# xingchensong/TouchNet

Measured on AMD Instinct MI355X. Metric: audio+text tokens/sec/node (packed seq, full train step) + step MFU, higher is better.
Workload: dtype bf16

## Files before the change

### include/touchnet_amd.h

```cpp
#ifndef TOUCHNET_AMD_H_
#define TOUCHNET_AMD_H_

#ifdef __cplusplus
extern "C" {
#endif

const char* tn_version(void);

int tn_norm_bwd_workspace_floats(int rows, int H);
int tn_rmsnorm_fwd(const void* x, const void* res_in, const void* w, void* y, void* res_out, float* rstd,
                   int rows, int H, float eps, int dtype, void* stream);
int tn_rmsnorm_bwd(const void* dy, const void* h, const void* w, const float* rstd, const void* dres, void* dh,
                   void* dw, float* workspace, int rows, int H, int dtype, void* stream);

int tn_layernorm_fwd(const void* x, const void* res_in, const void* w, const void* b, void* y, void* res_out,
                     float* mean, float* rstd, int rows, int H, float eps, int dtype, void* stream);
int tn_layernorm_bwd(const void* dy, const void* h, const void* w, const float* mean, const float* rstd,
                     const void* dres, void* dh, void* dw, void* db, float* workspace, int rows, int H, int dtype,
                     void* stream);

int tn_swiglu_fwd(const void* gate, const void* up, void* out, long long n, int dtype, void* stream);
int tn_swiglu_bwd(const void* dout, const void* gate, const void* up, void* dgate, void* dup, long long n,
                  int dtype, void* stream);
int tn_swiglu_fwd_t(const void* gate, const void* up, void* out, void* out_t, int rows, int cols, void* stream);
int tn_swiglu_bwd_t(const void* dout, const void* gate, const void* up, void* dgate, void* dup, void* dgu_t, int rows,
                    int cols, void* stream);
int tn_gelu_fwd(const void* x, void* out, long long n, int dtype, void* stream);
int tn_gelu_bwd(const void* dout, const void* x, void* dx, long long n, int dtype, void* stream);

int tn_rope_table(const long long* position_ids, const float* inv_freq, void* cos_t, void* sin_t, int n, int half,
                  float attention_scaling, int dtype, void* stream);
int tn_rope_apply(const void* q, const void* k, void* q_out, void* k_out, const void* cos_t, const void* sin_t,
                  int n, int hq, int hk, int D, int backward, int dtype, void* stream);

int tn_ce_forward(const void* logits, const long long* labels, const long long* sentence_lens,
                  const float* num_sentence, float* nll, float* lse, int* hit, float* out, int n, int V,
                  long long ignore_index, int dtype, void* stream);
int tn_ce_reduce(const float* nll, const int* hit, const long long* labels, const long long* sentence_lens,
                 const float* num_sentence, float* out, int n, long long ignore_index, void* stream);
int tn_ce_backward(const void* logits, void* dlogits, const long long* labels, const long long* sentence_lens,
                   const float* lse, const float* num_sentence, const float* grad_out, int n, int V,
                   long long ignore_index, int dtype, void* stream);

int tn_attn_meta_ints(int B, int T);
int tn_attn_build_meta(const int* doc, int* meta, int B, int T, void* stream);
int tn_attn_fwd(const void* q, const void* k, const void* v, void* o, float* lse2, const int* doc, const int* meta,
                int B, int T, int Nh, int Nkv, int D, float scale, void* stream);
int tn_attn_bwd(const void* q, const void* k, const void* v, const void* o, const void* dout, const float* lse2,
                float* delta, void* dq, void* dk, void* dv, const int* doc, const int* meta, int B, int T, int Nh,
                int Nkv, int D, float scale, void* stream);
int tn_attn_bwd_rope(const void* q, const void* k, const void* v, const void* o, const void* dout, const float* lse2,
                     float* delta, void* dq, void* dk, void* dv, const int* doc, const int* meta, int B, int T, int Nh,
                     int Nkv, int D, float scale, const void* cos_t, const void* sin_t, void* stream);
int tn_attn_fwd_bidir(const void* q, const void* k, const void* v, void* o, float* lse2, const int* doc, const int* meta,
                      int B, int T, int Nh, int Nkv, int D, float scale, void* stream);
int tn_attn_bwd_bidir(const void* q, const void* k, const void* v, const void* o, const void* dout, const float* lse2,
                      float* delta, void* dq, void* dk, void* dv, const int* doc, const int* meta, int B, int T, int Nh,
                      int Nkv, int D, float scale, void* stream);

int tn_attn_fwd_seg(const void* q, const void* k, const void* v, void* o, float* lse2, const int* doc,
                    const int* meta, int B, int T, int Nh, int Nkv, int D, float scale, int nseg,
                    const int* host_segs, int rows_per_batch, void* stream);
int tn_attn_fwd_seg_chunks(const void* q, const void* k, const void* v, void* o, float* lse2, const int* doc,
                           const int* meta, int B, int T, int Nh, int Nkv, int D, float scale, int nseg, const int* segs,
                           int rows_per_batch, int chunk_len, unsigned long long chunk_mask, void* stream);
int tn_attn_merge(const void* o_a, const float* lse2_a, const void* o_b, const float* lse2_b, void* o, float* lse2,
                  int B, int rows, int Nh, int D, void* stream);
int tn_attn_bwd_seg(const void* q, const void* k, const void* v, const void* o, const void* dout,
                    const float* lse2, float* delta, void* dq, void* dk, void* dv, const int* doc, const int* meta,
                    int B, int T, int Nh, int Nkv, int D, float scale, int nseg, const int* host_segs,
                    int rows_per_batch, void* stream);

int tn_fbank_frames(int n_samples);
int tn_kaldi_fbank(const float* wav, float* feat, int n_samples, int n_mels, void* stream);
int tn_log_mel(const float* wav, const float* mel_fb, float* feat, float* scratch_max, int n_samples, int n_mels,
               void* stream);
int tn_audiofeat_stack(const float* feat, float* out, int T, int F, int stack, int stride, int normalize,
                       void* stream);
int tn_feat_augment(const float* x, float* y, int T, int F, int out_rows, const int* t_masks, int n_t,
                    const int* f_masks, int n_f, const int* subs, int n_sub, void* stream);
int tn_resample_polyphase(const float* x, float* y, const float* tab, long long n_in, long long n_out, int p, int q,
                          int ntap, void* stream);
int tn_resample_sinc(const void* x, int x_is_pcm16, float* y, const float* tab, long long n_in, long long n_out,
                     int orig, int new_, int ntap, void* stream);

int tn_sumsq_scratch_floats(void);
int tn_sumsq(const void* g, float* scratch, float* norm_sq, long long n, int dtype, void* stream);
long long tn_sumsq_multi_chunk(void);
int tn_sumsq_multi(const void* const* ptrs, const long long* sizes, const long long* first_chunk, int ntensors,
                   long long nchunks, float* partial, float* norm_sq, int dtype, void* stream);
int tn_adamw_step(float* p, float* m, float* v, const void* g, void* p_shadow_bf16, const float* norm_sq,
                  long long n, float lr, float beta1, float beta2, float eps, float weight_decay, float max_norm,
                  float bias_corr1, float bias_corr2, int g_dtype, void* stream);

long long tn_adamw_multi_chunk(void);
int tn_adamw_prepare(const float* norm_sq, float* state, float beta1, float beta2, float max_norm, void* stream);
int tn_adamw_multi(void* const* ps, void* const* ms, void* const* vs, const void* const* gs, void* const* shadows,
                   const long long* sizes, const long long* first_chunk, int ntensors, long long nchunks,
                   const float* state, float lr, float beta1, float beta2, float eps, float weight_decay, int g_dtype,
                   void* stream);
int tn_adamw_multi_bounded(void* const* ps, void* const* ms, void* const* vs, const void* const* gs, void* const* shadows,
                           const long long* sizes, const long long* first_chunk, int ntensors, long long nchunks,
                           const float* state, float lr, float beta1, float beta2, float eps, float weight_decay,
                           int g_dtype, int max_workgroups, void* stream);

int tn_transpose_bf16(const void* src, void* dst, int rows, int cols, long long src_ld, long long dst_ld,
                      void* stream);

long long tn_colsum_workspace_floats(int rows, int cols);
int tn_colsum_bf16(const void* x, void* out, float* ws, int rows, int cols, long long ld, void* stream);

int tn_pcm16_to_f32(const void* pcm_int16, float* out, long long n, void* stream);

int tn_bestrq_tokenize(const float* feat, const float* quantizer, const float* codebook, long long* codes, int T,
                       int F, int E, int V, void* stream);

int tn_pack_plan(const int* lens, int n, int B, int T, int skip_too_long, int* row, int* col, int* sent, int* batch,
                 int* counts, void* stream);
int tn_pack_fill(const int* row, const int* col, const int* sent, const int* batch, int which_batch, int n,
                 const int* ntok, const long long* tok_off, const long long* tokens, const int* alen,
                 const long long* feat_off, const float* feat_src, int F, int B, int T, long long bos, long long eos,
                 long long pad, long long* input_ids, long long* labels, long long* position_ids, long long* doc,
                 long long* sentence_lens, float* feats, int* nsent, void* stream);

int tn_gemm_bf16(const void* const* A, const void* const* B, const long long* lda, const long long* ldb, const int* K,
                 int nseg, int a_kmaj, int b_kmaj, void* C, void* Ct, const void* bias, int M, int N, long long ldc,
                 long long ldct, int accumulate, void* stream);
int tn_gemm_bf16_addend(const void* A, const void* B, long long lda, long long ldb, int K, int a_kmaj, int b_kmaj, void* C,
                        const void* bias, const void* addend, long long ldadd, int M, int N, long long ldc, void* stream);
int tn_gemm_bf16_splitk(const void* A, const void* B, long long lda, long long ldb, int K, int a_kmaj, int b_kmaj,
                        void* C, const void* bias, int M, int N, long long ldc, int accumulate, int splitk, int tail_only,
                        void* workspace, long long workspace_bytes, void* stream);
int tn_gemm_bf16_wgrad_f32(const void* A, const void* B, long long lda, long long ldb, int K, float* C, int M, int N,
                           long long ldc, int accumulate, int splitk, void* workspace, long long workspace_bytes,
                           void* stream);
int tn_gemm_bf16_wgrad_bias(const void* A, const void* B, long long lda, long long ldb, int K, void* C, void* bias_grad,
                            int M, int N, long long ldc, int accumulate, int c_f32, int splitk, void* workspace,
                            long long workspace_bytes, void* stream);
long long tn_gemm_splitk_workspace_bytes(int M, int N, int splitk, int with_bias_grad, int tail_only);
long long tn_gemm_grouped_workspace_bytes(const int* M, const int* N, const int* K, int ngrp);
int tn_gemm_bf16_grouped(const void* const* A, const void* const* B, const long long* lda, const long long* ldb,
                         const int* K, void* const* C, const long long* ldc, const int* M, const int* N, int ngrp,
                         int a_kmaj, int b_kmaj, int accumulate, int c_f32, void* workspace, long long workspace_bytes,
                         void* stream);
long long tn_gemm_grouped_table_bytes(int n);
int tn_gemm_bf16_grouped_table(const void* const* A, const void* const* B, const long long* lda, const long long* ldb,
                               const int* K, void* const* C, const long long* ldc, const int* M, const int* N,
                               void* const* bias_grad, int n, int accumulate, int c_f32, void* table,
                               long long table_bytes, void* stream);
int tn_gemm_bf16_swiglu_fwd(const void* x, const void* wg, const void* wu, void* gate, void* up, void* act, int M, int I,
                            int K, long long ldx, long long ldw, long long ldc, void* stream);
int tn_gemm_bf16_swiglu_bwd(const void* dy, const void* wd, const void* gate, const void* up, void* dgate, void* dup,
                            int M, int I, int H, long long lddy, long long ldw, long long ld, void* stream);
int tn_gemm_bf16_gelu_fwd(const void* x, const void* w, const void* bias, void* pre, void* act, int M, int N, int K,
                          long long ldx, long long ldw, long long ldc, void* stream);
int tn_gemm_bf16_gelu_bwd(const void* dy, const void* w2, const void* pre, void* dpre, int M, int I, int H, long long lddy,
                          long long ldw, long long ld, void* stream);
int tn_gemm_bf16_rope(const void* x, const void* w, const void* bias, const void* cos_t, const void* sin_t, void* out, int M,
                      int N, int K, long long ldx, long long ldw, long long ldc, int head_dim, void* stream);
int tn_gemm_bf16_tn(const void* A, const void* B, void* C, void* Ct, const void* bias, int M, int N, int K,
                    long long lda, long long ldb, long long ldc, long long ldct, int accumulate, void* stream);

void tn_gemm_set_persistent(int on);
int tn_gemm_get_persistent(void);

long long tn_attn_decode_workspace_bytes(int B, int Nh, int Nkv, int D, int S_max);
int tn_attn_decode(const void* q, const void* k_new, const void* v_new, void* k_cache, void* v_cache, const int* cache_len,
                   void* o, void* workspace, int B, int Nh, int Nkv, int D, int S_max, float scale, void* stream);
int tn_greedy_step(const void* logits, int* hist, int* hist_len, int* cache_len, int* finished, int* n_unfinished, int B,
                   int V, int S_hist, float penalty, int ngram, int eos, int pad, int dtype, void* stream);
int tn_sample_step(const void* logits, int* hist, int* hist_len, int* cache_len, int* finished, int* n_unfinished,
                   const long long* row_key, const float* uniforms, int* n_kept, int B, int V, int S_hist, float penalty,
                   int do_sample, float temperature, int top_k, float top_p, unsigned long long seed, const int* eos_ids,
                   int n_eos, int pad, int dtype, void* stream);
int tn_kimi_text_step(const void* logits, int* hist, int* hist_len, int* cache_len, int* finished, int* n_unfinished,
                      const int* prompt_len, const void* embed, void* x_next, const long long* row_key,
                      const float* uniforms, int B, int V, int S_hist, int H, float penalty, int window, float temperature,
                      int top_k, unsigned long long seed, int eos, int blank, int audio_token, int dtype, void* stream);

int tn_attn_decode_beam(const void* q, const void* k_new, const void* v_new, void* k_cache, void* v_cache,
                        const int* cache_len, const int* src, void* o, void* workspace, int R, int Nh, int Nkv, int D,
                        int S_max, float scale, void* stream);
long long tn_beam_step_workspace_bytes(int B, int K);
int tn_beam_step(const void* logits, int* hist, int* hist_len, int* cache_len, int* src, float* run_score, int* fin_ids,
                 int* fin_len, float* fin_score, int* fin_flag, int* gen, int* unsat, int* done, int* n_unfinished,
                 int* out_ids, int* out_parent, void* workspace, int B, int K, int K_in, int V, int S_hist, float penalty,
                 int ngram, const int* eos_ids, int n_eos, int n_new, float length_penalty, int early_stopping, int dtype,
                 void* stream);

int tn_attn_block_causal_fwd(const void* q, const void* k, const void* v, void* o, const int* seg_start, const int* key_end,
                             int B, int T, int Nh, int D, int block, float scale, void* stream);
int tn_vq_nearest(const void* x, const void* codebook, const float* cnorm, long long* ids, int M, int V, int d, void* stream);

#ifdef __cplusplus
}
#endif
#endif
```

### touchnet_amd/_C.py

```python
from __future__ import annotations

import ctypes as C
import os

import torch

_HERE = os.path.dirname(os.path.abspath(__file__))
LIB_PATH = os.environ.get("TN_AMD_LIB") or os.path.join(_HERE, "_lib", "libtouchnet_amd.so")

_vp, _i, _f, _ll, _ull = C.c_void_p, C.c_int, C.c_float, C.c_longlong, C.c_ulonglong

PROTOTYPES = {
    "tn_version": [],
    "tn_norm_bwd_workspace_floats": [_i, _i],
    "tn_rmsnorm_fwd": [_vp, _vp, _vp, _vp, _vp, _vp, _i, _i, _f, _i, _vp],
    "tn_rmsnorm_bwd": [_vp, _vp, _vp, _vp, _vp, _vp, _vp, _vp, _i, _i, _i, _vp],
    "tn_layernorm_fwd": [_vp, _vp, _vp, _vp, _vp, _vp, _vp, _vp, _i, _i, _f, _i, _vp],
    "tn_layernorm_bwd": [_vp, _vp, _vp, _vp, _vp, _vp, _vp, _vp, _vp, _vp, _i, _i, _i, _vp],
    "tn_swiglu_fwd": [_vp, _vp, _vp, _ll, _i, _vp],
    "tn_swiglu_bwd": [_vp, _vp, _vp, _vp, _vp, _ll, _i, _vp],
    "tn_gelu_fwd": [_vp, _vp, _ll, _i, _vp],
    "tn_gelu_bwd": [_vp, _vp, _vp, _ll, _i, _vp],
    "tn_rope_table": [_vp, _vp, _vp, _vp, _i, _i, _f, _i, _vp],
    "tn_rope_apply": [_vp, _vp, _vp, _vp, _vp, _vp, _i, _i, _i, _i, _i, _i, _vp],
    "tn_ce_forward": [_vp, _vp, _vp, _vp, _vp, _vp, _vp, _vp, _i, _i, _ll, _i, _vp],
    "tn_ce_reduce": [_vp, _vp, _vp, _vp, _vp, _vp, _i, _ll, _vp],
    "tn_ce_backward": [_vp, _vp, _vp, _vp, _vp, _vp, _vp, _i, _i, _ll, _i, _vp],
    "tn_attn_meta_ints": [_i, _i],
    "tn_attn_build_meta": [_vp, _vp, _i, _i, _vp],
    "tn_attn_fwd": [_vp, _vp, _vp, _vp, _vp, _vp, _vp, _i, _i, _i, _i, _i, _f, _vp],
    "tn_attn_bwd": [_vp, _vp, _vp, _vp, _vp, _vp, _vp, _vp, _vp, _vp, _vp, _vp, _i, _i, _i, _i, _i, _f, _vp],
    "tn_attn_bwd_rope": [_vp, _vp, _vp, _vp, _vp, _vp, _vp, _vp, _vp, _vp, _vp, _vp, _i, _i, _i, _i, _i, _f, _vp, _vp, _vp],
    "tn_attn_fwd_bidir": [_vp, _vp, _vp, _vp, _vp, _vp, _vp, _i, _i, _i, _i, _i, _f, _vp],
    "tn_attn_bwd_bidir": [_vp, _vp, _vp, _vp, _vp, _vp, _vp, _vp, _vp, _vp, _vp, _vp, _i, _i, _i, _i, _i, _f, _vp],
    "tn_attn_fwd_seg": [_vp, _vp, _vp, _vp, _vp, _vp, _vp, _i, _i, _i, _i, _i, _f, _i, _vp, _i, _vp],
    "tn_attn_fwd_seg_chunks": [_vp, _vp, _vp, _vp, _vp, _vp, _vp, _i, _i, _i, _i, _i, _f, _i, _vp, _i, _i, C.c_ulonglong, _vp],
    "tn_attn_merge": [_vp, _vp, _vp, _vp, _vp, _vp, _i, _i, _i, _i, _vp],
    "tn_attn_bwd_seg": [_vp, _vp, _vp, _vp, _vp, _vp, _vp, _vp, _vp, _vp, _vp, _vp, _i, _i, _i, _i, _i, _f, _i, _vp,
                        _i, _vp],
    "tn_fbank_frames": [_i],
    "tn_kaldi_fbank": [_vp, _vp, _i, _i, _vp],
    "tn_log_mel": [_vp, _vp, _vp, _vp, _i, _i, _vp],
    "tn_audiofeat_stack": [_vp, _vp, _i, _i, _i, _i, _i, _vp],
    "tn_resample_polyphase": [_vp, _vp, _vp, _ll, _ll, _i, _i, _i, _vp],
    "tn_resample_sinc": [_vp, _i, _vp, _vp, _ll, _ll, _i, _i, _i, _vp],
    "tn_feat_augment": [_vp, _vp, _i, _i, _i, _vp, _i, _vp, _i, _vp, _i, _vp],
    "tn_sumsq_scratch_floats": [],
    "tn_sumsq": [_vp, _vp, _vp, _ll, _i, _vp],
    "tn_adamw_step": [_vp, _vp, _vp, _vp, _vp, _vp, _ll, _f, _f, _f, _f, _f, _f, _f, _f, _i, _vp],
    "tn_transpose_bf16": [_vp, _vp, _i, _i, _ll, _ll, _vp],
    "tn_swiglu_fwd_t": [_vp, _vp, _vp, _vp, _i, _i, _vp],
    "tn_swiglu_bwd_t": [_vp, _vp, _vp, _vp, _vp, _vp, _i, _i, _vp],
    "tn_colsum_workspace_floats": [_i, _i],
    "tn_colsum_bf16": [_vp, _vp, _vp, _i, _i, _ll, _vp],
    "tn_pcm16_to_f32": [_vp, _vp, _ll, _vp],
    "tn_bestrq_tokenize": [_vp, _vp, _vp, _vp, _i, _i, _i, _i, _vp],
    "tn_sumsq_multi_chunk": [],
    "tn_sumsq_multi": [_vp, _vp, _vp, _i, _ll, _vp, _vp, _i, _vp],
    "tn_adamw_multi_chunk": [],
    "tn_adamw_prepare": [_vp, _vp, _f, _f, _f, _vp],
    "tn_adamw_multi": [_vp, _vp, _vp, _vp, _vp, _vp, _vp, _i, _ll, _vp, _f, _f, _f, _f, _f, _i, _vp],
    "tn_adamw_multi_bounded": [_vp, _vp, _vp, _vp, _vp, _vp, _vp, _i, _ll, _vp, _f, _f, _f, _f, _f, _i, _i, _vp],
    "tn_pack_plan": [_vp, _i, _i, _i, _i, _vp, _vp, _vp, _vp, _vp, _vp],
    "tn_pack_fill": [_vp, _vp, _vp, _vp, _i, _i, _vp, _vp, _vp, _vp, _vp, _vp, _i, _i, _i, _ll, _ll, _ll, _vp, _vp, _vp,
                     _vp, _vp, _vp, _vp, _vp],
    "tn_gemm_bf16_tn": [_vp, _vp, _vp, _vp, _vp, _i, _i, _i, _ll, _ll, _ll, _ll, _i, _vp],
    "tn_gemm_bf16_addend": [_vp, _vp, _ll, _ll, _i, _i, _i, _vp, _vp, _vp, _ll, _i, _i, _ll, _vp],
    "tn_gemm_bf16_splitk": [_vp, _vp, _ll, _ll, _i, _i, _i, _vp, _vp, _i, _i, _ll, _i, _i, _i, _vp, _ll, _vp],
    "tn_gemm_bf16_wgrad_f32": [_vp, _vp, _ll, _ll, _i, _vp, _i, _i, _ll, _i, _i, _vp, _ll, _vp],
    "tn_gemm_bf16": [C.POINTER(_vp), C.POINTER(_vp), C.POINTER(_ll), C.POINTER(_ll), C.POINTER(_i), _i, _i, _i, _vp, _vp,
                     _vp, _i, _i, _ll, _ll, _i, _vp],
    "tn_gemm_splitk_workspace_bytes": [_i, _i, _i, _i, _i],
    "tn_gemm_grouped_workspace_bytes": [C.POINTER(_i), C.POINTER(_i), C.POINTER(_i), _i],
    "tn_gemm_bf16_grouped": [C.POINTER(_vp), C.POINTER(_vp), C.POINTER(_ll), C.POINTER(_ll), C.POINTER(_i), C.POINTER(_vp),
                             C.POINTER(_ll), C.POINTER(_i), C.POINTER(_i), _i, _i, _i, _i, _i, _vp, _ll, _vp],
    "tn_gemm_grouped_table_bytes": [_i],
    "tn_gemm_bf16_grouped_table": [C.POINTER(_vp), C.POINTER(_vp), C.POINTER(_ll), C.POINTER(_ll), C.POINTER(_i),
                                   C.POINTER(_vp), C.POINTER(_ll), C.POINTER(_i), C.POINTER(_i), C.POINTER(_vp), _i, _i, _i,
                                   _vp, _ll, _vp],
    "tn_gemm_bf16_wgrad_bias": [_vp, _vp, _ll, _ll, _i, _vp, _vp, _i, _i, _ll, _i, _i, _i, _vp, _ll, _vp],
    "tn_gemm_bf16_rope": [_vp, _vp, _vp, _vp, _vp, _vp, _i, _i, _i, _ll, _ll, _ll, _i, _vp],
    "tn_gemm_bf16_gelu_fwd": [_vp, _vp, _vp, _vp, _vp, _i, _i, _i, _ll, _ll, _ll, _vp],
    "tn_gemm_bf16_gelu_bwd": [_vp, _vp, _vp, _vp, _i, _i, _i, _ll, _ll, _ll, _vp],
    "tn_gemm_bf16_swiglu_fwd": [_vp, _vp, _vp, _vp, _vp, _vp, _i, _i, _i, _ll, _ll, _ll, _vp],
    "tn_gemm_bf16_swiglu_bwd": [_vp, _vp, _vp, _vp, _vp, _vp, _i, _i, _i, _ll, _ll, _ll, _vp],
    "tn_gemm_set_persistent": [_i],
    "tn_gemm_get_persistent": [],
    "tn_attn_decode_workspace_bytes": [_i, _i, _i, _i, _i],
    "tn_attn_decode": [_vp, _vp, _vp, _vp, _vp, _vp, _vp, _vp, _i, _i, _i, _i, _i, _f, _vp],
    "tn_greedy_step": [_vp, _vp, _vp, _vp, _vp, _vp, _i, _i, _i, _f, _i, _i, _i, _i, _vp],
    "tn_sample_step": [_vp, _vp, _vp, _vp, _vp, _vp, _vp, _vp, _vp, _i, _i, _i, _f, _i, _f, _i, _f, _ull, _vp, _i, _i, _i,
                       _vp],
    "tn_kimi_text_step": [_vp] * 11 + [_i, _i, _i, _i, _f, _i, _f, _i, _ull, _i, _i, _i, _i, _vp],
    "tn_attn_decode_beam": [_vp, _vp, _vp, _vp, _vp, _vp, _vp, _vp, _vp, _i, _i, _i, _i, _i, _f, _vp],
    "tn_beam_step_workspace_bytes": [_i, _i],
    "tn_beam_step": [_vp] * 17 + [_i, _i, _i, _i, _i, _f, _i, _vp, _i, _i, _f, _i, _i, _vp],
    "tn_attn_block_causal_fwd": [_vp, _vp, _vp, _vp, _vp, _vp, _i, _i, _i, _i, _i, _f, _vp],
    "tn_vq_nearest": [_vp, _vp, _vp, _vp, _i, _i, _i, _vp],
}
_RESTYPE = {"tn_gemm_set_persistent": None, "tn_version": C.c_char_p, "tn_sumsq_multi_chunk": C.c_longlong, "tn_adamw_multi_chunk": C.c_longlong,
            "tn_colsum_workspace_floats": C.c_longlong, "tn_gemm_splitk_workspace_bytes": C.c_longlong,
            "tn_gemm_grouped_workspace_bytes": C.c_longlong, "tn_gemm_grouped_table_bytes": C.c_longlong,
            "tn_attn_decode_workspace_bytes": C.c_longlong, "tn_beam_step_workspace_bytes": C.c_longlong,
            "tn_philox4x32_10": None}

DEV_PROTOTYPES = {
    "tn_philox4x32_10": [_vp, _ull],
}

_lib = None


class KernelError(RuntimeError):
    pass


def lib() -> C.CDLL:
    global _lib
    if _lib is None:
        if not os.path.exists(LIB_PATH):
            raise ImportError(
                f"{LIB_PATH} not found: build it with `python -m touchnet_amd.build` "
                "(touchnet_amd has no fallback path; the HIP extension is mandatory)")
        handle = C.CDLL(LIB_PATH)
        for name, argtypes in {**PROTOTYPES, **DEV_PROTOTYPES}.items():
            fn = getattr(handle, name)
            fn.argtypes = argtypes
            fn.restype = _RESTYPE.get(name, C.c_int)
        _lib = handle
    return _lib


def check(code: int, what: str) -> None:
    if code != 0:
        raise KernelError(f"{what} failed with code {code} "
                          f"({'EINVAL: unsupported shape/dtype' if code == -22 else 'hipError_t'})")


DTYPE_CODE = {torch.float32: 0, torch.bfloat16: 1}


def dcode(t: torch.Tensor) -> int:
    try:
        return DTYPE_CODE[t.dtype]
    except KeyError:
        raise KernelError(f"unsupported dtype {t.dtype} (float32 / bfloat16 only)") from None


def ptr(t):
    if t is None:
        return None
    if not t.is_cuda:
        raise KernelError("touchnet_amd kernels need device (HIP) tensors; got a CPU tensor")
    return C.c_void_p(t.data_ptr())


def stream():
    return C.c_void_p(torch.cuda.current_stream().cuda_stream)


def version() -> str:
    return lib().tn_version().decode()
```

### touchnet_amd/csrc/gemm.hip

```cpp
#include "gemm_host.h"

namespace tn {
namespace gemm {

typedef f32x4_t Acc16[8][4];

template <bool AK, bool BK, int EPI = EPI_PLAIN>
struct Kernel16 {
  static_assert(EPI == EPI_PLAIN || EPI == EPI_SWIGLU_FWD || EPI == EPI_SWIGLU_BWD || EPI == EPI_ROPE ||
                    EPI == EPI_GELU_FWD || EPI == EPI_GELU_BWD,
                "Kernel16: plain / SwiGLU / RoPE / GELU epilogues (the weight-gradient modes stay on Kernel)");
  static_assert(EPI != EPI_GELU_FWD || !BK, "GELU forward: x W^T layout");
  static_assert(EPI != EPI_GELU_BWD || BK, "GELU backward: dY W layout");
  static_assert(!AK, "Kernel16: row-stored A (forward and input-gradient products)");
  static_assert(EPI != EPI_SWIGLU_FWD || !BK, "SwiGLU forward: x W^T layout");
  static_assert(EPI != EPI_SWIGLU_BWD || BK, "SwiGLU backward: dY W layout");
  static_assert(EPI != EPI_ROPE || !BK, "RoPE epilogue: x W^T layout");
  static constexpr int BN_EFF = EPI == EPI_SWIGLU_FWD ? 128 : BN;
  static __device__ __forceinline__ float sigm(float x) { return sigmoid_fast(x); }
  static __device__ __forceinline__ float lo16(uint32_t w) { return __uint_as_float(w << 16); }
  static __device__ __forceinline__ float hi16(uint32_t w) { return __uint_as_float(w & 0xffff0000u); }
  static __device__ __forceinline__ float rbf(float v) { return __uint_as_float(((uint32_t)f2bf(v)) << 16); }
  template <bool KMAJ>
  struct F4 {
// ... 438 lines not shown
      for (int bi = 0; bi < 4; ++bi) {
        const int m = min(wm0 + (half * 4 + bi) * 16 + l15, p.M - 1);
#pragma unroll
        for (int bj = 0; bj < 2; ++bj) {
          const long long o = (long long)m * hd + c0 + 16 * bj + 4 * g4;
          cw[bi][bj] = *reinterpret_cast<const uint2*>(p.rope_cos + o);
          sw[bi][bj] = *reinterpret_cast<const uint2*>(p.rope_sin + o);
        }
      }
#pragma unroll
      for (int bi = 0; bi < 4; ++bi)
#pragma unroll
        for (int bj = 0; bj < 2; ++bj) {
          const float ba[4] = {lo16(bwa[bj].x), hi16(bwa[bj].x), lo16(bwa[bj].y), hi16(bwa[bj].y)};
          const float bb[4] = {lo16(bwb[bj].x), hi16(bwb[bj].x), lo16(bwb[bj].y), hi16(bwb[bj].y)};
          const float cf[4] = {lo16(cw[bi][bj].x), hi16(cw[bi][bj].x), lo16(cw[bi][bj].y), hi16(cw[bi][bj].y)};
          const float sf[4] = {lo16(sw[bi][bj].x), hi16(sw[bi][bj].x), lo16(sw[bi][bj].y), hi16(sw[bi][bj].y)};
          float ya[4], yb[4];
#pragma unroll
          for (int e = 0; e < 4; ++e)
            rope_rotate(rbf(acc[half * 4 + bi][bj][e] + ba[e]), rbf(acc[half * 4 + bi][bj + 2][e] + bb[e]), cf[e], sf[e],
                        ya[e], yb[e]);
          *reinterpret_cast<u32x2_t*>(park_at(park, bi, bj, l15, g4)) = u32x2_t{pack2bf(ya[0], ya[1]), pack2bf(ya[2], ya[3])};
          *reinterpret_cast<u32x2_t*>(park_at(park, bi, bj + 2, l15, g4)) = u32x2_t{pack2bf(yb[0], yb[1]), pack2bf(yb[2], yb[3])};
        }
      asm volatile("s_waitcnt lgkmcnt(0)" ::: "memory");
#pragma unroll 4
      for (int it = 0; it < 8; ++it) {
        const int row = it * 8 + (lane >> 3), c = lane & 7;
        const u32x4_t pv = *reinterpret_cast<const u32x4_t*>(park + row * 128 + ((c ^ (row & 7)) << 4));
        const int m = wm0 + half * 64 + row, n = (c < 4 ? col_a : col_b) + (c & 3) * 8;
        if (m < p.M && n < p.N)
          *reinterpret_cast<uint4*>(p.C + (long long)m * p.ldc + n) = make_uint4(pv.x, pv.y, pv.z, pv.w);
      }
    }
  }

  static __device__ __forceinline__ void epilogue16(const Params& p, Acc16& acc, char* park, int wm0, int wn0, int lane) {
    const int l15 = lane & 15, g4 = lane >> 4;
    float bias_v[4][4];
    if (p.bias != nullptr) {
#pragma unroll
      for (int bj = 0; bj < 4; ++bj) {
        const int n = min(wn0 + bj * 16 + 4 * g4, p.N - 4);
        const uint2 w = *reinterpret_cast<const uint2*>(p.bias + n);
        bias_v[bj][0] = __uint_as_float(w.x << 16);
        bias_v[bj][1] = __uint_as_float(w.x & 0xffff0000u);
        bias_v[bj][2] = __uint_as_float(w.y << 16);
        bias_v[bj][3] = __uint_as_float(w.y & 0xffff0000u);
      }
    }
    const bool acc_c = p.accumulate != 0 || p.addend != nullptr;
#pragma unroll
    for (int half = 0; half < 2; ++half) {
      uint4 xpre[8];
      if constexpr (EPI == EPI_GELU_BWD) {
#pragma unroll
        for (int it = 0; it < 8; ++it) {
          const int m = wm0 + half * 64 + it * 8 + (lane >> 3), n = wn0 + (lane & 7) * 8;
          xpre[it] = (m < p.M && n < p.N) ? *reinterpret_cast<const uint4*>(p.E1 + (long long)m * p.lde + n)
                                          : make_uint4(0, 0, 0, 0);
        }
      }
#pragma unroll
      for (int bi = 0; bi < 4; ++bi) {
        const int row = bi * 16 + l15;
#pragma unroll
        for (int bj = 0; bj < 4; ++bj) {
          float v[4];
#pragma unroll
          for (int e = 0; e < 4; ++e) v[e] = acc[half * 4 + bi][bj][e] + (p.bias != nullptr ? bias_v[bj][e] : 0.f);
          const int chunk = (bj * 2 + (g4 >> 1)) ^ (row & 7);
          const u32x2_t pk = {pack2bf(v[0], v[1]), pack2bf(v[2], v[3])};
          *reinterpret_cast<u32x2_t*>(park + row * 128 + chunk * 16 + (g4 & 1) * 8) = pk;
        }
      }
      asm volatile("s_waitcnt lgkmcnt(0)" ::: "memory");
      constexpr int kReadOutUnroll = EPI == EPI_GELU_BWD ? 8 : 4;
#pragma unroll kReadOutUnroll
      for (int it = 0; it < 8; ++it) {
        const int row = it * 8 + (lane >> 3), c = lane & 7;
        const u32x4_t pv = *reinterpret_cast<const u32x4_t*>(park + row * 128 + ((c ^ (row & 7)) << 4));
        uint4 v = make_uint4(pv.x, pv.y, pv.z, pv.w);
        const int m = wm0 + half * 64 + row, n = wn0 + c * 8;
        if (m < p.M && n < p.N) {
          bf16_t* dst = p.C + (long long)m * p.ldc + n;
          if constexpr (EPI == EPI_GELU_FWD) {
            *reinterpret_cast<uint4*>(dst) = v;
            Vec16<bf16_t> x;
            x.raw = v;
            float f[8];
            x.unpack(f);
#pragma unroll
            for (int e = 0; e < 8; e += 2) {
              const gelu_f32x2 r = gelu_f2(gelu_f32x2{f[e], f[e + 1]});
              f[e] = r.x;
              f[e + 1] = r.y;
            }
            x.pack(f);
            *reinterpret_cast<uint4*>(p.C2 + (long long)m * p.ldc + n) = x.raw;
            continue;
          }
          if constexpr (EPI == EPI_GELU_BWD) {
            Vec16<bf16_t> x, d;
            x.raw = xpre[it];
            d.raw = v;
            float f[8], df[8];
            x.unpack(f);
            d.unpack(df);
#pragma unroll
            for (int e = 0; e < 8; e += 2) {
              const gelu_f32x2 r = gelu_grad_f2(gelu_f32x2{f[e], f[e + 1]}, gelu_f32x2{df[e], df[e + 1]});
              df[e] = r.x;
              df[e + 1] = r.y;
            }
            d.pack(df);
            *reinterpret_cast<uint4*>(dst) = d.raw;
            continue;
          }
          if (acc_c) {
            Vec16<bf16_t> o, nw;
            o.load(p.addend != nullptr ? p.addend + (long long)m * p.ldadd + n : dst);
            nw.raw = v;
            float fo[8], fn[8];
            o.unpack(fo);
            nw.unpack(fn);
#pragma unroll
            for (int e = 0; e < 8; ++e) fn[e] += fo[e];
            nw.pack(fn);
            v = nw.raw;
          }
          *reinterpret_cast<uint4*>(dst) = v;
        }
      }
    }
  }
};

template <bool AK, bool BK, int EPI = EPI_PLAIN>
__global__ __launch_bounds__(NT, 2) void gemm16_kernel(const Params p) {
  __shared__ __attribute__((aligned(1024))) char smem[LDS_BYTES];
  Kernel16<AK, BK, EPI>::run(p, smem);
}

__global__ __launch_bounds__(256) void splitk_reduce_kernel(const float* __restrict__ ws, int S, int M, int N, int nbm,
                                                            int nbn, int tile0, int ntiles, bf16_t* __restrict__ C,
                                                            long long ldc, const bf16_t* __restrict__ bias,
                                                            int accumulate, int out_f32,
                                                            const float* __restrict__ bias_ws,
                                                            bf16_t* __restrict__ bias_out) {
  const int t = blockIdx.x >> 5, part = blockIdx.x & 31;
  int tm, tn;
  tile_of_block(tile0 + t, nbm, nbn, tm, tn);
  const int idx = part * 256 + threadIdx.x;
  const int lm = idx >> 5, ln = (idx & 31) * 8;
  const int m = tm * BM + lm, n = tn * BN + ln;
  if (m >= M || n >= N) return;
  if (bias_out != nullptr && tn == 0 && ln == 0) {
    float b = 0.f;
    for (int sp = 0; sp < S; ++sp) b += bias_ws[(long long)sp * (nbm * BM) + m];
    bias_out[m] = f2bf(b);
  }
  float a[8] = {0.f, 0.f, 0.f, 0.f, 0.f, 0.f, 0.f, 0.f};
  const float* src = ws + (long long)t * (BM * BN) + lm * BN + ln;
  const long long slab = (long long)ntiles * (BM * BN);
  for (int sp = 0; sp < S; ++sp) {
    const float4 x = *reinterpret_cast<const float4*>(src + sp * slab);
    const float4 y = *reinterpret_cast<const float4*>(src + sp * slab + 4);
    a[0] += x.x; a[1] += x.y; a[2] += x.z; a[3] += x.w;
    a[4] += y.x; a[5] += y.y; a[6] += y.z; a[7] += y.w;
  }
  if (out_f32) {
    float* d = reinterpret_cast<float*>(C) + (long long)m * ldc + n;
    float4 x = make_float4(a[0], a[1], a[2], a[3]), y = make_float4(a[4], a[5], a[6], a[7]);
    if (accumulate) {
      const float4 ox = *reinterpret_cast<const float4*>(d), oy = *reinterpret_cast<const float4*>(d + 4);
      x.x += ox.x; x.y += ox.y; x.z += ox.z; x.w += ox.w;
      y.x += oy.x; y.y += oy.y; y.z += oy.z; y.w += oy.w;
    }
    *reinterpret_cast<float4*>(d) = x;
    *reinterpret_cast<float4*>(d + 4) = y;
    return;
  }
  bf16_t* dst = C + (long long)m * ldc + n;
  if (bias != nullptr) {
    Vec16<bf16_t> b;
    float fb[8];
    b.load(bias + n);
    b.unpack(fb);
#pragma unroll
    for (int e = 0; e < 8; ++e) a[e] += fb[e];
  }
  if (accumulate) {
    Vec16<bf16_t> o;
    float fo[8];
    o.load(dst);
    o.unpack(fo);
#pragma unroll
    for (int e = 0; e < 8; ++e) a[e] += fo[e];
  }
  Vec16<bf16_t> out;
  out.pack(a);
  out.store(dst);
}

template <bool AK, bool BK, bool HAS_CT>
static int launch(dim3 grid, hipStream_t st, const Params& p) {
  constexpr bool WGRAD = AK && BK && !HAS_CT;
  auto reduce = [&](const float* bias_ws, bf16_t* bias_out) {
    hipLaunchKernelGGL(splitk_reduce_kernel, dim3((unsigned)p.ntiles * 32u), dim3(256), 0, st, p.ws, p.splitk, p.M, p.N,
                       p.nbm, p.nbn, p.tile0, p.ntiles, p.C, p.ldc, p.bias, p.accumulate, p.c_f32, bias_ws, bias_out);
  };
  if (p.bias_out != nullptr) {
    if constexpr (WGRAD) {
      if (p.splitk > 1) {
        hipLaunchKernelGGL((gemm_kernel<true, true, false, true, false, EPI_BIASG>), grid, dim3(NT), 0, st, p);
        reduce(p.bias_ws, p.bias_out);
      } else if (p.c_f32) {
        hipLaunchKernelGGL((gemm_kernel<true, true, false, false, true, EPI_BIASG>), grid, dim3(NT), 0, st, p);
      } else {
        hipLaunchKernelGGL((gemm_kernel<true, true, false, false, false, EPI_BIASG>), grid, dim3(NT), 0, st, p);
      }
    } else {
      return -1;
    }
  } else if (p.splitk > 1) {
    if constexpr (!HAS_CT) {
      hipLaunchKernelGGL((gemm_kernel<AK, BK, false, true>), grid, dim3(NT), 0, st, p);
      reduce(nullptr, nullptr);
    } else {
      return -1;
    }
  } else if (p.c_f32) {
    if constexpr (WGRAD) {
      hipLaunchKernelGGL((gemm_kernel<true, true, false, false, true>), grid, dim3(NT), 0, st, p);
    } else {
      return -1;
    }
  } else if constexpr (!AK && !HAS_CT) {
    hipLaunchKernelGGL((gemm16_kernel<AK, BK>), grid, dim3(NT), 0, st, p);
  } else {
    hipLaunchKernelGGL((gemm_kernel<AK, BK, HAS_CT>), grid, dim3(NT), 0, st, p);
  }
  return 0;
}

}
}


extern "C" long long tn_gemm_splitk_workspace_bytes(int M, int N, int splitk, int with_bias_grad, int tail_only);

namespace {

int g_persistent = 1;

long long slab_floats(int parts, long long tiles) { return parts * tiles * BM * BN; }

int grouped_split(long long total, int min_stages, int& r) {
  const int ncu = num_cus();
  r = (int)(total % ncu);
  if (total <= ncu || r == 0 || r * 2 > ncu || min_stages < 16) return 1;
  return min(ncu / r, min_stages / 8);
}

struct GemmCall {
  const void* const* A;
  const void* const* B;
  const long long* lda;
  const long long* ldb;
  const int* K;
  int nseg, a_kmaj, b_kmaj;
  void* C;
  long long ldc;
  int M, N;
  void* stream;
  const void* bias = nullptr;
  int accumulate = 0;
  void* Ct = nullptr;
  long long ldct = 0;
  int splitk = 1, tail_only = 0;
  void* workspace = nullptr;
  long long workspace_bytes = 0;
  int c_f32 = 0;
  void* bias_grad = nullptr;
  const void* addend = nullptr;
  long long ldadd = 0;
};

int launch_mode(bool a_kmaj, bool b_kmaj, bool ct, dim3 grid, hipStream_t st, const Params& p) {
  if (!a_kmaj && !b_kmaj) return ct ? launch<false, false, true>(grid, st, p) : launch<false, false, false>(grid, st, p);
  if (!a_kmaj) return ct ? launch<false, true, true>(grid, st, p) : launch<false, true, false>(grid, st, p);
  return ct ? launch<true, true, true>(grid, st, p) : launch<true, true, false>(grid, st, p);
}

int gemm_launch(const GemmCall& c) {
  const int M = c.M, N = c.N;
  const bool wgrad_mode = c.a_kmaj && c.b_kmaj && c.nseg == 1 && c.Ct == nullptr && c.bias == nullptr;
  if (c.a_kmaj && !c.b_kmaj) return TN_EINVAL;
  if (c.addend != nullptr && (c.accumulate || c.splitk > 1 || c.tail_only || c.Ct != nullptr || c.c_f32 ||
                              c.bias_grad != nullptr || !out_ok(c.addend, c.ldadd, N, 8)))
    return TN_EINVAL;
  if ((c.bias_grad != nullptr || c.c_f32) && (!wgrad_mode || c.tail_only)) return TN_EINVAL;
  if (!aligned(1, c.bias_grad)) return TN_EINVAL;
  if (M <= 0 || N <= 0 || c.nseg < 1 || c.nseg > MAXSEG || (N % 8) != 0 || (c.a_kmaj && (M % 8))) return TN_EINVAL;
  if (!out_ok(c.C, c.ldc, N, 8)) return TN_EINVAL;
  if (c.Ct != nullptr && ((M % 8) || c.accumulate || !out_ok(c.Ct, c.ldct, M, 8))) return TN_EINVAL;
  Params p;
  clear_params(p);
  for (int s = 0; s < c.nseg; ++s) {
    const int k = c.K[s];
    if (!(c.a_kmaj ? kmaj_operand_ok(c.A[s], c.lda[s], k, M, M) : row_operand_ok(c.A[s], c.lda[s], k, 1))) return TN_EINVAL;
    if (!(c.b_kmaj ? kmaj_operand_ok(c.B[s], c.ldb[s], k, N, 1) : row_operand_ok(c.B[s], c.ldb[s], k, 1))) return TN_EINVAL;
    set_seg(p.seg[s], c.A[s], c.B[s], c.lda[s], c.ldb[s], k);
    p.stages += (k + 63) / 64;
  }
  for (int s = c.nseg; s < MAXSEG; ++s) p.seg[s] = p.seg[0];
  p.nseg = c.nseg;
  p.M = M;
  p.N = N;
  p.C = (bf16_t*)c.C;
  p.Ct = (bf16_t*)c.Ct;
  p.bias = (const bf16_t*)c.bias;
  p.ldc = c.ldc;
  p.ldct = c.ldct;
  p.accumulate = c.accumulate;
  p.addend = (const bf16_t*)c.addend;
  p.ldadd = c.ldadd;
  p.nbm = (M + BM - 1) / BM;
  p.nbn = (N + BN - 1) / BN;
  p.ntiles = p.nbm * p.nbn;
  p.c_f32 = c.c_f32;
  p.bias_out = (bf16_t*)c.bias_grad;
  const int ncu = num_cus();
  int main_tiles = 0;
  if (c.splitk > 1) {
    if (c.nseg != 1 || c.Ct != nullptr) return TN_EINVAL;
    if (!(c.a_kmaj && c.b_kmaj) && (p.stages % c.splitk) != 0) return TN_EINVAL;
    const long long need = tn_gemm_splitk_workspace_bytes(M, N, c.splitk, c.bias_grad != nullptr, c.tail_only);
    if (need < 0 || c.workspace == nullptr || !aligned(15, c.workspace) || c.workspace_bytes < need) return TN_EINVAL;
    if (c.tail_only) main_tiles = p.ntiles / ncu * ncu;
    p.splitk = c.splitk;
    p.kchunk = (p.stages + c.splitk - 1) / c.splitk;
    p.ws = (float*)c.workspace;
    if (c.bias_grad != nullptr) p.bias_ws = p.ws + slab_floats(c.splitk, p.ntiles);
  }
  hipStream_t st = (hipStream_t)c.stream;
  int rc = 0;
  if (main_tiles > 0) {
    Params pm = p;
    pm.splitk = 1;
    pm.ntiles = main_tiles;
    rc |= launch_mode(c.a_kmaj, c.b_kmaj, c.Ct != nullptr, dim3(ncu), st, pm);
    p.tile0 = main_tiles;
    p.ntiles -= main_tiles;
  }
  rc |= launch_mode(c.a_kmaj, c.b_kmaj, c.Ct != nullptr, grid_for(p.ntiles * p.splitk), st, p);
  if (rc != 0) return TN_EINVAL;
  TN_LAUNCH_CHECK();
  return TN_OK;
}

template <int EPI, bool B_KMAJ>
int launch_fused(Params& p, int M, int N, long long ldc, int col_tile, void* stream) {
  for (int s = 1; s < MAXSEG; ++s)
    if (p.seg[s].K == 0) p.seg[s] = p.seg[0];
  p.stages = p.seg[0].K / 64;
  p.M = M;
  p.N = N;
  p.ldc = ldc;
  p.nbm = (M + BM - 1) / BM;
  p.nbn = (N + col_tile - 1) / col_tile;
  p.ntiles = p.nbm * p.nbn;
  hipLaunchKernelGGL((gemm16_kernel<false, B_KMAJ, EPI>), grid_for(p.ntiles), dim3(NT), 0, (hipStream_t)stream, p);
  TN_LAUNCH_CHECK();
  return TN_OK;
}

}

extern "C" {

void tn_gemm_set_persistent(int on) { g_persistent = on ? 1 : 0; }
int tn_gemm_get_persistent(void) { return g_persistent; }

long long tn_gemm_splitk_workspace_bytes(int M, int N, int splitk, int with_bias_grad, int tail_only) {
  if (splitk <= 1) return 0;
  if (M <= 0 || N <= 0) return -1;
  const long long nbm = (M + BM - 1) / BM;
  long long tiles = nbm * ((N + BN - 1) / BN);
  if (tail_only) {
    const int ncu = num_cus();
    if (tiles < ncu || tiles % ncu == 0) return -1;
    tiles %= ncu;
  }
  return (slab_floats(splitk, tiles) + (with_bias_grad ? splitk * nbm * BM : 0)) * (long long)sizeof(float);
}

int tn_gemm_bf16(const void* const* A, const void* const* B, const long long* lda, const long long* ldb, const int* K,
                 int nseg, int a_kmaj, int b_kmaj, void* C, void* Ct, const void* bias, int M, int N, long long ldc,
                 long long ldct, int accumulate, void* stream) {
  GemmCall c{A, B, lda, ldb, K, nseg, a_kmaj, b_kmaj, C, ldc, M, N, stream};
  c.bias = bias;
  c.accumulate = accumulate;
  c.Ct = Ct;
  c.ldct = ldct;
  return gemm_launch(c);
}

int tn_gemm_bf16_addend(const void* A, const void* B, long long lda, long long ldb, int K, int a_kmaj, int b_kmaj, void* C,
                        const void* bias, const void* addend, long long ldadd, int M, int N, long long ldc, void* stream) {
  if (addend == nullptr || addend == C) return TN_EINVAL;
  GemmCall c{&A, &B, &lda, &ldb, &K, 1, a_kmaj, b_kmaj, C, ldc, M, N, stream};
  c.bias = bias;
  c.addend = addend;
  c.ldadd = ldadd;
  return gemm_launch(c);
}

int tn_gemm_bf16_splitk(const void* A, const void* B, long long lda, long long ldb, int K, int a_kmaj, int b_kmaj,
                        void* C, const void* bias, int M, int N, long long ldc, int accumulate, int splitk, int tail_only,
                        void* workspace, long long workspace_bytes, void* stream) {
  if (splitk < 2) return TN_EINVAL;
  GemmCall c{&A, &B, &lda, &ldb, &K, 1, a_kmaj, b_kmaj, C, ldc, M, N, stream};
  c.bias = bias;
  c.accumulate = accumulate;
  c.splitk = splitk;
  c.tail_only = tail_only;
  c.workspace = workspace;
  c.workspace_bytes = workspace_bytes;
  return gemm_launch(c);
}

static int wgrad(const void* A, const void* B, long long lda, long long ldb, int K, void* C, void* bias_grad, int M, int N,
                 long long ldc, int accumulate, int c_f32, int splitk, void* workspace, long long workspace_bytes,
                 void* stream) {
  GemmCall c{&A, &B, &lda, &ldb, &K, 1, 1, 1, C, ldc, M, N, stream};
  c.accumulate = accumulate;
  c.c_f32 = c_f32;
  c.bias_grad = bias_grad;
  c.splitk = splitk > 1 ? splitk : 1;
  c.workspace = workspace;
  c.workspace_bytes = workspace_bytes;
  return gemm_launch(c);
}

int tn_gemm_bf16_wgrad_f32(const void* A, const void* B, long long lda, long long ldb, int K, float* C, int M, int N,
                           long long ldc, int accumulate, int splitk, void* workspace, long long workspace_bytes,
                           void* stream) {
  return wgrad(A, B, lda, ldb, K, C, nullptr, M, N, ldc, accumulate, 1, splitk, workspace, workspace_bytes, stream);
}

int tn_gemm_bf16_wgrad_bias(const void* A, const void* B, long long lda, long long ldb, int K, void* C, void* bias_grad,
                            int M, int N, long long ldc, int accumulate, int c_f32, int splitk, void* workspace,
                            long long workspace_bytes, void* stream) {
  if (bias_grad == nullptr) return TN_EINVAL;
  return wgrad(A, B, lda, ldb, K, C, bias_grad, M, N, ldc, accumulate, c_f32, splitk, workspace, workspace_bytes, stream);
}

long long tn_gemm_grouped_workspace_bytes(const int* M, const int* N, const int* K, int ngrp) {
  if (ngrp < 1 || ngrp > MAXSEG) return -1;
  long long tiles = 0;
  int min_stages = 0x7fffffff, r;
  for (int g = 0; g < ngrp; ++g) {
    tiles += (long long)((M[g] + BM - 1) / BM) * ((N[g] + BN - 1) / BN);
    min_stages = min(min_stages, (K[g] + 63) / 64);
  }
  const int S = grouped_split(tiles, min_stages, r);
  return S > 1 ? slab_floats(S, r) * (long long)sizeof(float) : 0;
}

int tn_gemm_bf16_grouped(const void* const* A, const void* const* B, const long long* lda, const long long* ldb,
                         const int* K, void* const* C, const long long* ldc, const int* M, const int* N, int ngrp,
                         int a_kmaj, int b_kmaj, int accumulate, int c_f32, void* workspace, long long workspace_bytes,
                         void* stream) {
  if (ngrp < 1 || ngrp > MAXSEG) return TN_EINVAL;
  if (!(a_kmaj && b_kmaj)) return TN_EINVAL;
  Params p;
  clear_params(p);
  int total = 0, min_stages = 0x7fffffff;
  for (int g = 0; g < ngrp; ++g) {
    if (!grouped_product(A[g], B[g], lda[g], ldb[g], K[g], C[g], ldc[g], M[g], N[g], c_f32, total, p.seg[g], p.grp[g]))
      return TN_EINVAL;
    min_stages = min(min_stages, p.grp[g].stages);
    total += p.grp[g].nbm * p.grp[g].nbn;
  }
  for (int g = ngrp; g < MAXSEG; ++g) {
    p.seg[g] = p.seg[0];
    p.grp[g] = p.grp[0];
    p.grp[g].start = 0x7fffffff;
  }
  p.ngrp = ngrp;
  p.accumulate = accumulate;
  p.c_f32 = c_f32;
  hipStream_t st = (hipStream_t)stream;
  int r, S = grouped_split(total, min_stages, r);
  if (S > 1 && (workspace == nullptr || !aligned(15, workspace) ||
                workspace_bytes < slab_floats(S, r) * (long long)sizeof(float)))
    S = 1;
  const int main_tiles = S > 1 ? total - r : total;
  p.tile0 = 0;
  p.ntiles = main_tiles;
  if (c_f32)
    hipLaunchKernelGGL((gemm_kernel<true, true, false, false, true, EPI_GROUPED>), grid_for(main_tiles), dim3(NT), 0, st, p);
  else
    hipLaunchKernelGGL((gemm_kernel<true, true, false, false, false, EPI_GROUPED>), grid_for(main_tiles), dim3(NT), 0, st, p);
  if (S > 1) {
    float* ws = (float*)workspace;
    for (int g = 0; g < ngrp; ++g) {
      const int end = p.grp[g].start + p.grp[g].nbm * p.grp[g].nbn;
      const int lo = max(main_tiles, p.grp[g].start), hi = end;
      if (lo >= hi) continue;
      Params q;
      clear_params(q);
      q.seg[0] = p.seg[g];
      q.seg[1] = q.seg[2] = q.seg[0];
      q.M = p.grp[g].M;
      q.N = p.grp[g].N;
      q.C = p.grp[g].C;
      q.ldc = p.grp[g].ldc;
      q.accumulate = accumulate;
      q.nbm = p.grp[g].nbm;
      q.nbn = p.grp[g].nbn;
      q.stages = p.grp[g].stages;
      q.splitk = S;
      q.kchunk = (q.stages + S - 1) / S;
      q.ws = ws;
      q.tile0 = lo - p.grp[g].start;
      q.ntiles = hi - lo;
      q.c_f32 = c_f32;
      hipLaunchKernelGGL((gemm_kernel<true, true, false, true>), grid_for(q.ntiles * S), dim3(NT), 0, st, q);
      hipLaunchKernelGGL(splitk_reduce_kernel, dim3((unsigned)q.ntiles * 32u), dim3(256), 0, st, q.ws, q.splitk, q.M, q.N,
                         q.nbm, q.nbn, q.tile0, q.ntiles, q.C, q.ldc, (const bf16_t*)nullptr, q.accumulate, q.c_f32,
                         (const float*)nullptr, (bf16_t*)nullptr);
      ws += slab_floats(S, q.ntiles);
    }
  }
  TN_LAUNCH_CHECK();
  return TN_OK;
}
int tn_gemm_bf16_swiglu_fwd(const void* x, const void* wg, const void* wu, void* gate, void* up, void* act, int M, int I,
                            int K, long long ldx, long long ldw, long long ldc, void* stream) {
  if (M <= 0 || I <= 0 || (I % 8) || !row_operand_ok(x, ldx, K, K) || !row_operand_ok(wg, ldw, K, K) ||
      !row_operand_ok(wu, ldw, K, K) || !out_ok(gate, ldc, I, 8) || !aligned(15, up, act))
    return TN_EINVAL;
  Params p;
  clear_params(p);
  set_seg(p.seg[0], x, wg, ldx, ldw, K);
  set_seg(p.seg[1], x, wu, ldx, ldw, K);
  p.C = (bf16_t*)gate;
  p.C2 = (bf16_t*)up;
  p.C3 = (bf16_t*)act;
  return launch_fused<EPI_SWIGLU_FWD, false>(p, M, I, ldc, 128, stream);
}

int tn_gemm_bf16_swiglu_bwd(const void* dy, const void* wd, const void* gate, const void* up, void* dgate, void* dup,
                            int M, int I, int H, long long lddy, long long ldw, long long ld, void* stream) {
  if (M <= 0 || I <= 0 || (I % 8) || !row_operand_ok(dy, lddy, H, H) || !kmaj_operand_ok(wd, ldw, H, I, I) ||
      !out_ok(dgate, ld, I, 8) || !aligned(15, dup, gate, up))
    return TN_EINVAL;
  Params p;
  clear_params(p);
  set_seg(p.seg[0], dy, wd, lddy, ldw, H);
  p.C = (bf16_t*)dgate;
  p.C2 = (bf16_t*)dup;
  p.E1 = (const bf16_t*)gate;
  p.E2 = (const bf16_t*)up;
  p.lde = ld;
  return launch_fused<EPI_SWIGLU_BWD, true>(p, M, I, ld, BN, stream);
}

int tn_gemm_bf16_rope(const void* x, const void* w, const void* bias, const void* cos_t, const void* sin_t, void* out, int M,
                      int N, int K, long long ldx, long long ldw, long long ldc, int head_dim, void* stream) {
  if (M <= 0 || N <= 0 || !row_operand_ok(x, ldx, K, K) || !row_operand_ok(w, ldw, K, K) || !out_ok(out, ldc, N, 8))
    return TN_EINVAL;
  if (!((head_dim == 128 && N % 256 == 0) || (head_dim == 64 && N % 64 == 0))) return TN_EINVAL;
  if (cos_t == nullptr || sin_t == nullptr || !aligned(7, cos_t, sin_t, bias)) return TN_EINVAL;
  Params p;
  clear_params(p);
  set_seg(p.seg[0], x, w, ldx, ldw, K);
  p.C = (bf16_t*)out;
  p.bias = (const bf16_t*)bias;
  p.rope_cos = (const bf16_t*)cos_t;
  p.rope_sin = (const bf16_t*)sin_t;
  p.rope_d = head_dim;
  return launch_fused<EPI_ROPE, false>(p, M, N, ldc, BN, stream);
}

int tn_gemm_bf16_gelu_fwd(const void* x, const void* w, const void* bias, void* pre, void* act, int M, int N, int K,
                          long long ldx, long long ldw, long long ldc, void* stream) {
  if (M <= 0 || N <= 0 || (N % 8) || !row_operand_ok(x, ldx, K, K) || !row_operand_ok(w, ldw, K, K) ||
      !out_ok(pre, ldc, N, 8) || !aligned(15, act) || !aligned(7, bias))
    return TN_EINVAL;
  if (pre == act) return TN_EINVAL;
  Params p;
  clear_params(p);
  set_seg(p.seg[0], x, w, ldx, ldw, K);
  p.C = (bf16_t*)pre;
  p.C2 = (bf16_t*)act;
  p.bias = (const bf16_t*)bias;
  return launch_fused<EPI_GELU_FWD, false>(p, M, N, ldc, BN, stream);
}

int tn_gemm_bf16_gelu_bwd(const void* dy, const void* w2, const void* pre, void* dpre, int M, int I, int H, long long lddy,
                          long long ldw, long long ld, void* stream) {
  if (M <= 0 || I <= 0 || (I % 8) || !row_operand_ok(dy, lddy, H, H) || !kmaj_operand_ok(w2, ldw, H, I, I) ||
      !out_ok(dpre, ld, I, 8) || !aligned(15, pre))
    return TN_EINVAL;
  Params p;
  clear_params(p);
  set_seg(p.seg[0], dy, w2, lddy, ldw, H);
  p.C = (bf16_t*)dpre;
  p.E1 = (const bf16_t*)pre;
  p.lde = ld;
  return launch_fused<EPI_GELU_BWD, true>(p, M, I, ld, BN, stream);
}

int tn_gemm_bf16_tn(const void* A, const void* B, void* C, void* Ct, const void* bias, int M, int N, int K,
                    long long lda, long long ldb, long long ldc, long long ldct, int accumulate, void* stream) {
  return tn_gemm_bf16(&A, &B, &lda, &ldb, &K, 1, 0, 0, C, Ct, bias, M, N, ldc, ldct, accumulate, stream);
}

}
```

### touchnet_amd/csrc/gemm_host.h

```cpp
#pragma once

#include "gemm_kernel.h"

using namespace tn::gemm;
using tn::bf16_t;

extern "C" int tn_gemm_get_persistent(void);

namespace {

int num_cus() {
  static const int ncu = [] {
    int dev = 0, n = 256;
    if (hipGetDevice(&dev) == hipSuccess) (void)hipDeviceGetAttribute(&n, hipDeviceAttributeMultiprocessorCount, dev);
    return n >= 8 ? n / 8 * 8 : 8;
  }();
  return ncu;
}

bool persistent_now() {
  const char* pe = getenv("TN_GEMM_PERSIST");
  return pe ? atoi(pe) != 0 : tn_gemm_get_persistent() != 0;
}

dim3 grid_for(int units) {
  const int ncu = num_cus();
  return dim3(persistent_now() && units > ncu ? ncu : units);
}

void clear_params(Params& p) {
  p = Params{};
  p.splitk = 1;
  p.nseg = 1;
}

void set_seg(Seg& s, const void* A, const void* B, long long lda, long long ldb, int K) {
  s.A = (const bf16_t*)A;
  s.B = (const bf16_t*)B;
  s.lda = lda;
  s.ldb = ldb;
  s.K = K;
  s.pad_ = 0;
}

template <typename... P>
bool aligned(uintptr_t mask, P... ps) {
  return ((... | (uintptr_t)ps) & mask) == 0;
}

constexpr long long DMA_SPAN = 0x7fffffffLL;

bool row_operand_ok(const void* X, long long ld, int K, long long min_ld) {
  return K > 0 && (K % 64) == 0 && aligned(15, X) && (ld % 8) == 0 && ld >= min_ld && 288 * ld * 2 < DMA_SPAN;
}

bool kmaj_operand_ok(const void* X, long long ld, int K, int rows, long long min_ld) {
  return K > 0 && aligned(15, X) && (ld % 8) == 0 && ld >= min_ld && ((long long)(K - 1) * ld + rows) * 2 < DMA_SPAN;
}

bool out_ok(const void* C, long long ld, int cols, int ld_mult) { return aligned(15, C) && (ld % ld_mult) == 0 && ld >= cols; }

bool grouped_product(const void* A, const void* B, long long lda, long long ldb, int k, void* C, long long ldc, int m, int n,
                     int c_f32, int start, Seg& s, Grp& g) {
  if (m <= 0 || n <= 0 || (m % 8) || (n % 8) || !kmaj_operand_ok(A, lda, k, m, m) || !kmaj_operand_ok(B, ldb, k, n, 1) ||
      !out_ok(C, ldc, n, c_f32 ? 4 : 8))
    return false;
  set_seg(s, A, B, lda, ldb, k);
  g.C = (bf16_t*)C;
  g.ldc = ldc;
  g.M = m;
  g.N = n;
  g.nbm = (m + BM - 1) / BM;
  g.nbn = (n + BN - 1) / BN;
  g.start = start;
  g.stages = (k + 63) / 64;
  return true;
}

}
```

### touchnet_amd/csrc/gemm_kernel.h

```cpp
#pragma once

#include <stdlib.h>

#include <type_traits>
#include <utility>
#include <vector>

#include "common.h"

namespace tn {
namespace gemm {

constexpr int BM = 256, BN = 256;
constexpr int SLOT = 32768;
constexpr int LDS_BYTES = 5 * SLOT;
constexpr int NT = 512;
constexpr int MAXSEG = 3;

typedef __attribute__((address_space(3))) void* lds_ptr_t;
typedef __attribute__((ext_vector_type(2))) uint32_t u32x2_t;
typedef __attribute__((ext_vector_type(4))) uint32_t u32x4_t;

struct Seg {
  const bf16_t* A;
  const bf16_t* B;
  long long lda, ldb;
  int K;
  int pad_;
};

struct Grp {
  bf16_t* C;
  long long ldc;
  int M, N, nbm, nbn;
  int start;
  int stages;
};

struct Rec {
  Seg seg;
  Grp grp;
  bf16_t* bias_out;
};
typedef const __attribute__((address_space(4))) Rec* rec_ptr_t;
constexpr int MAXTAB = 1024;
constexpr int TABCHUNK = 32;

constexpr int EPI_PLAIN = 0, EPI_GROUPED = 1, EPI_SWIGLU_FWD = 2, EPI_SWIGLU_BWD = 3, EPI_BIASG = 4, EPI_ROPE = 5;
constexpr int EPI_GELU_FWD = 6, EPI_GELU_BWD = 7, EPI_TABLE = 8;

struct Params {
  Seg seg[MAXSEG];
  int nseg;
  int M, N;
  bf16_t* C;
  bf16_t* Ct;
  const bf16_t* bias;
  long long ldc, ldct;
  int accumulate;
  const bf16_t* addend;
  long long ldadd;
  int nbm, nbn;
  int stages;
  int splitk, kchunk;
  float* ws;
  int tile0, ntiles;
  int c_f32;
  Grp grp[MAXSEG];
  int ngrp;
  bf16_t* C2;
  bf16_t* C3;
  const bf16_t* E1;
  const bf16_t* E2;
  long long lde;
  bf16_t* bias_out;
  float* bias_ws;
  const bf16_t* rope_cos;
  const bf16_t* rope_sin;
  int rope_d;
  const Rec* table;
};

__device__ __forceinline__ int xcd_chunk(int bid, int total) {
  const int xcd = bid & 7, local = bid >> 3;
  const int q = total >> 3, r = total & 7;
  return (xcd < r ? xcd * (q + 1) : r * (q + 1) + (xcd - r) * q) + local;
}

__device__ __forceinline__ void panel_group(int vid, int nbm, int nbn, int& tm, int& tn) {
  constexpr int GM = 8;
  const int per_group = GM * nbn;
  const int g = vid / per_group, w = vid - g * per_group;
  const int gm = min(GM, nbm - g * GM);
  tm = g * GM + w % gm;
  tn = w / gm;
}

__device__ __forceinline__ void tile_of_block(int bid, int nbm, int nbn, int& tm, int& tn) {
  panel_group(xcd_chunk(bid, nbm * nbn), nbm, nbn, tm, tn);
}

typedef f32x16_t Acc[4][2];

constexpr int kPieceB[4] = {0, 2, 4, 6}, kPieceA[4] = {14, 18, 22, 26};
static_assert(kPieceB[3] < kPieceA[0], "every B piece is issued before the first A piece");

template <bool IS_A> constexpr int piece_at(int pos) {
  for (int i = 0; i < 4; ++i)
    if ((IS_A ? kPieceA[i] : kPieceB[i]) == pos) return i;
  return -1;
}
constexpr int early_piece_count() {
  int n = 0;
  for (int i = 0; i < 4; ++i) n += (kPieceB[i] < 8) + (kPieceA[i] < 8);
  return n;
}

template <bool KMAJ, bool M16 = false>
struct Stream {
  __amdgpu_buffer_rsrc_t rs;
  int soff;
  int step;
  int left;
  int seg;
  int ld2;
  int voff[4];

  __device__ __forceinline__ void set_voff(int wave, int lane) {
    if constexpr (!KMAJ) {
#pragma unroll
      for (int q = 0; q < 4; ++q) {
        const int row = wave * 32 + q * 8 + (lane >> 3);
        voff[q] = row * ld2 + (((lane & 7) ^ ((row >> 1) & 7)) << 4);
      }
    } else {
#pragma unroll
      for (int q = 0; q < 4; ++q) {
        const int k = wave * 8 + q * 2 + (lane >> 5);
        const int u = lane & 31;
        const int ch = M16 ? ((u & 3) ^ (((k >> 3) & 1) << 1)) : (u & 3);
        voff[q] = k * ld2 + ((((u >> 2) ^ (k & 3)) << 6) | (ch << 4));
      }
    }
  }

  __device__ __forceinline__ void open(const bf16_t* X, long long ld, int K, int R, int origin, int wave, int lane) {
    ld2 = (int)(ld * 2);
    if constexpr (!KMAJ) {
      const long long bytes = max((long long)(R - origin) * ld2, 0LL);
      rs = __builtin_amdgcn_make_buffer_rsrc((void*)(X + (long long)origin * ld), 0, (int)min(bytes, 0x7fffffffLL),
                                             0x00020000);
      step = 128;
    } else {
      const long long bytes = ((long long)(K - 1) * ld + (R - origin)) * 2;
      rs = __builtin_amdgcn_make_buffer_rsrc((void*)(X + origin), 0, (int)min(bytes, 0x7fffffffLL), 0x00020000);
      step = 64 * ld2;
    }
    set_voff(wave, lane);
    soff = 0;
    left = (K + 63) >> 6;
  }
  __device__ __forceinline__ void kill(const void* any) {
    rs = __builtin_amdgcn_make_buffer_rsrc((void*)any, 0, 0, 0x00020000);
    soff = 0;
    step = 0;
    left = 0x7fffffff;
  }
};

template <bool KMAJ, int NB>
struct Frags {
  bf16x8_t v[NB];
  u32x2_t h[KMAJ ? NB : 1][2];
};

template <int OFF>
__device__ __forceinline__ u32x2_t ds_tr16(uint32_t addr) {
  u32x2_t r;
  asm volatile("ds_read_b64_tr_b16 %0, %1 offset:%2" : "=v"(r) : "v"(addr), "n"(OFF));
  return r;
}

template <bool AK, bool BK, bool HAS_CT, bool SPLITK = false, bool OUT_F32 = false, int EPI = EPI_PLAIN>
struct Kernel {
  static_assert(EPI == EPI_PLAIN || EPI == EPI_GROUPED || EPI == EPI_BIASG || EPI == EPI_TABLE,
                "Kernel: plain / grouped / bias-gradient epilogues (the fused ones are Kernel16's)");
  static constexpr bool MULTI = EPI == EPI_GROUPED || EPI == EPI_TABLE;
  static constexpr bool BIASG = EPI == EPI_BIASG || EPI == EPI_TABLE;
  static_assert(!MULTI || (!HAS_CT && !SPLITK), "grouped launch: whole tiles, no transposed copy");
  static_assert(!BIASG || (AK && BK && !HAS_CT), "bias gradient: weight-gradient mode");
  struct Out {
    bf16_t* C;
    long long ldc;
    int M, N;
  };
  template <bool KMAJ, int NB>
  struct Reader {
    int x[4];
    __device__ __forceinline__ Reader(int lane, int row0 ) {
      const int l31 = lane & 31, hi = lane >> 5;
      if constexpr (!KMAJ) {
        const int f = (l31 >> 1) & 7;
#pragma unroll
        for (int q = 0; q < 4; ++q) x[q] = (row0 + l31) * 128 + (((2 * q + hi) ^ f) << 4);
      } else {
        const int s4 = lane & 15, j = s4 >> 2, w = s4 & 3, half = (lane >> 4) & 1;
#pragma unroll
        for (int b = 0; b < 4; ++b)
          x[b] = (8 * hi + j) * 512 + half * 32 + w * 8 + ((((row0 >> 5) + (b < NB ? b : 0)) ^ j) << 6);
      }
    }
    template <int Q, int B>
    __device__ __forceinline__ void read(const char* smem, int sbase, Frags<KMAJ, NB>& f) const {
      if constexpr (!KMAJ) {
        f.v[B] = __builtin_bit_cast(bf16x8_t, *reinterpret_cast<const u32x4_t*>(smem + sbase + x[Q] + B * 4096));
      } else {
        const uint32_t a = (uint32_t)(size_t)(lds_ptr_t)smem + (uint32_t)(sbase + x[B]);
        f.h[B][0] = ds_tr16<(16 * Q) * 512>(a);
        f.h[B][1] = ds_tr16<(16 * Q + 4) * 512>(a);
      }
    }
  };

  static __device__ __forceinline__ void wait_frags(Frags<AK, 4>& a, Frags<BK, 2>& b) {
    if constexpr (AK && BK) {
      asm volatile("s_waitcnt lgkmcnt(0)"
                   : "+v"(a.h[0][0]), "+v"(a.h[0][1]), "+v"(a.h[1][0]), "+v"(a.h[1][1]), "+v"(a.h[2][0]), "+v"(a.h[2][1]),
                     "+v"(a.h[3][0]), "+v"(a.h[3][1]), "+v"(b.h[0][0]), "+v"(b.h[0][1]), "+v"(b.h[1][0]), "+v"(b.h[1][1]));
    } else if constexpr (AK) {
      asm volatile("s_waitcnt lgkmcnt(0)"
                   : "+v"(a.h[0][0]), "+v"(a.h[0][1]), "+v"(a.h[1][0]), "+v"(a.h[1][1]), "+v"(a.h[2][0]), "+v"(a.h[2][1]),
                     "+v"(a.h[3][0]), "+v"(a.h[3][1]));
    } else if constexpr (BK) {
      asm volatile("s_waitcnt lgkmcnt(0)" : "+v"(b.h[0][0]), "+v"(b.h[0][1]), "+v"(b.h[1][0]), "+v"(b.h[1][1]));
    }
    if constexpr (AK) {
#pragma unroll
      for (int i = 0; i < 4; ++i) {
        const u32x4_t t = {a.h[i][0].x, a.h[i][0].y, a.h[i][1].x, a.h[i][1].y};
        a.v[i] = __builtin_bit_cast(bf16x8_t, t);
      }
    }
    if constexpr (BK) {
#pragma unroll
      for (int j = 0; j < 2; ++j) {
        const u32x4_t t = {b.h[j][0].x, b.h[j][0].y, b.h[j][1].x, b.h[j][1].y};
        b.v[j] = __builtin_bit_cast(bf16x8_t, t);
      }
    }
  }

  static __device__ __forceinline__ void run(const Params& p, char* smem) { body(p, smem); }

  static __device__ __forceinline__ void body(const Params& p, char* smem) {
    const int tid = threadIdx.x;
    int lane = tid & 63;
    const int wave = __builtin_amdgcn_readfirstlane(tid >> 6);
    const int wr = wave >> 2, wc = wave & 3;

    const int bid = blockIdx.x, G = gridDim.x;
    const int tiles = p.ntiles;
    const int mine = ((SPLITK ? tiles * p.splitk : tiles) - bid + G - 1) / G;
    const rec_ptr_t tab = (rec_ptr_t)p.table;
    auto seg_of = [&](int g) {
      if constexpr (EPI == EPI_TABLE) {
        Seg s;
        s.A = tab[g].seg.A;
        s.B = tab[g].seg.B;
        s.lda = tab[g].seg.lda;
        s.ldb = tab[g].seg.ldb;
        s.K = tab[g].seg.K;
        s.pad_ = 0;
        return s;
      } else {
        return p.seg[g];
      }
    };
    auto grp_of = [&](int g) {
      if constexpr (EPI == EPI_TABLE) {
        Grp r;
        r.C = tab[g].grp.C;
        r.ldc = tab[g].grp.ldc;
        r.M = tab[g].grp.M;
        r.N = tab[g].grp.N;
        r.nbm = tab[g].grp.nbm;
        r.nbn = tab[g].grp.nbn;
        r.start = tab[g].grp.start;
        r.stages = tab[g].grp.stages;
        return r;
      } else {
        return p.grp[g];
      }
    };
    auto origin_g = [&](int k, int& m0, int& n0, int& g) {
      int tm, tn, u = bid + k * G;
      if constexpr (SPLITK) u -= (u / tiles) * tiles;
      u += p.tile0;
      g = 0;
      if constexpr (EPI == EPI_TABLE) {
        u = xcd_chunk(u, tiles);
        int hi = p.ngrp - 1;
        while (g < hi) {
          const int mid = (g + hi + 1) >> 1;
          if (tab[mid].grp.start <= u) g = mid;
          else hi = mid - 1;
        }
      } else if constexpr (EPI == EPI_GROUPED) {
        if (p.ngrp > 1 && u >= p.grp[1].start) g = 1;
        if (p.ngrp > 2 && u >= p.grp[2].start) g = 2;
      }
      if constexpr (EPI == EPI_TABLE) {
        const Grp r = grp_of(g);
        panel_group(u - r.start, r.nbm, r.nbn, tm, tn);
      } else if constexpr (EPI == EPI_GROUPED) {
        const Grp r = grp_of(g);
        tile_of_block(u - r.start, r.nbm, r.nbn, tm, tn);
      } else {
        tile_of_block(u, p.nbm, p.nbn, tm, tn);
      }
      m0 = tm * BM;
      n0 = tn * BN;
    };
    auto origin = [&](int k, int& m0, int& n0) {
      int g;
      origin_g(k, m0, n0, g);
    };
    auto split_of = [&](int k) { return (bid + k * G) / tiles; };

    Stream<AK> sA;
    Stream<BK> sB;
    int ka = 0, kb = 0;
    auto open_a = [&](int s) {
      int m0, n0;
      origin(ka, m0, n0);
      if constexpr (SPLITK) {
        const int k0 = split_of(ka) * p.kchunk * 64, klen = min(p.seg[0].K - k0, p.kchunk * 64);
        if (klen > 0) sA.open(p.seg[0].A + (AK ? (long long)k0 * p.seg[0].lda : (long long)k0), p.seg[0].lda, klen, p.M,
                              m0, wave, lane);
        else sA.kill(p.C);
        sA.left = p.kchunk;
      } else if constexpr (MULTI) {
        int g;
        origin_g(ka, m0, n0, g);
// ... 120 lines not shown
        constexpr int pa = P0 < 0 ? -1 : piece_at<true>(P0 + m);
        if constexpr (pb >= 0) {
          piece_b(dst_b, pb);
          if constexpr (pb == 3) adv_b();
          TN_PIN();
        }
        if constexpr (pa >= 0) {
          piece_a(dst_a, pa);
          if constexpr (pa == 3) adv_a();
          TN_PIN();
        }
      };
      step(std::integral_constant<int, 0>{});
      step(std::integral_constant<int, 1>{});
      step(std::integral_constant<int, 2>{});
      step(std::integral_constant<int, 3>{});
      step(std::integral_constant<int, 4>{});
      step(std::integral_constant<int, 5>{});
      step(std::integral_constant<int, 6>{});
      step(std::integral_constant<int, 7>{});
    };
    auto early_pieces = [&](int dst_b, int dst_a) {
      auto one = [&](auto MC) {
        constexpr int m = decltype(MC)::value;
        constexpr int pb = piece_at<false>(m), pa = piece_at<true>(m);
        if constexpr (pb >= 0) {
          piece_b(dst_b, pb);
          if constexpr (pb == 3) adv_b();
        }
        if constexpr (pa >= 0) {
          piece_a(dst_a, pa);
          if constexpr (pa == 3) adv_a();
        }
      };
      one(std::integral_constant<int, 0>{});
      one(std::integral_constant<int, 1>{});
      one(std::integral_constant<int, 2>{});
      one(std::integral_constant<int, 3>{});
      one(std::integral_constant<int, 4>{});
      one(std::integral_constant<int, 5>{});
      one(std::integral_constant<int, 6>{});
      one(std::integral_constant<int, 7>{});
    };
    auto next = [](int s, int d) { s += d; return s >= 5 ? s - 5 : s; };
    using I0 = std::integral_constant<int, 0>;
    using I1 = std::integral_constant<int, 1>;
    using I2 = std::integral_constant<int, 2>;
    using I3 = std::integral_constant<int, 3>;
    using NONE = std::integral_constant<int, -1>;

#pragma unroll
    for (int q = 0; q < 4; ++q) piece_a(0, q);
    adv_a();
#pragma unroll
    for (int q = 0; q < 4; ++q) piece_b(1, q);
    adv_b();
#pragma unroll
    for (int q = 0; q < 4; ++q) piece_a(2, q);
    adv_a();
    early_pieces(3, 4);
    asm volatile("s_waitcnt vmcnt(%0)" ::"n"(4 + early_piece_count()) : "memory");
    __builtin_amdgcn_s_barrier();
    int sa = 0, sb = 1;
    int pa = 4, pb = 3;

    auto trip = [&](auto LASTC) {
      constexpr bool LAST = decltype(LASTC)::value;
      const int sa1 = next(sa, 2), sb1 = next(sb, 2);
      __builtin_amdgcn_s_setprio(1);
      quarter(I1{}, std::integral_constant<int, 8>{}, ae, be, ao, bo, sa, sb, pb, pa);
      wait_frags(ao, bo);
      TN_PIN();
      quarter(I2{}, std::integral_constant<int, 16>{}, ao, bo, ae, be, sa, sb, pb, pa);
      wait_frags(ae, be);
      TN_PIN();
      quarter(I3{}, std::integral_constant<int, 24>{}, ae, be, ao, bo, sa, sb, pb, pa);
      __builtin_amdgcn_s_setprio(0);
      wait_frags(ao, bo);
      __builtin_amdgcn_s_waitcnt(0xc07f);
      asm volatile("s_waitcnt vmcnt(4)" ::: "memory");
      __builtin_amdgcn_s_barrier();
      __builtin_amdgcn_s_setprio(1);
      if constexpr (!LAST) {
        quarter(I0{}, I0{}, ao, bo, ae, be, sa1, sb1, sa, sb);
        __builtin_amdgcn_s_setprio(0);
        wait_frags(ae, be);
        TN_PIN();
      } else {
        if constexpr (BIASG) {
          if (bias_on) bias_accum(ao);
        }
#pragma unroll
        for (int m = 0; m < 8; ++m) mma(ao, bo, m >> 1, m & 1);
        __builtin_amdgcn_s_setprio(0);
      }
      pb = sa;
      pa = sb;
      sa = sa1;
      sb = sb1;
    };

    const int np_all = SPLITK ? p.kchunk : p.stages;
    for (int kc = 0; kc < mine; ++kc) {
      int np = np_all;
      if constexpr (BIASG) {
        int m0_, n0_, g_;
        origin_g(kc, m0_, n0_, g_);
        bias_on = n0_ == 0;
        if constexpr (EPI == EPI_TABLE) bias_on = bias_on && tab[g_].bias_out != nullptr;
        bsum = 0.f;
      }
      if constexpr (MULTI) {
        int m0_, n0_, g_;
        origin_g(kc, m0_, n0_, g_);
        np = grp_of(g_).stages;
      }
      read_all(I0{}, sa, sb, ae, be);
      wait_frags(ae, be);
      TN_PIN();
      for (int t = 1; t < np; ++t) trip(std::false_type{});
      trip(std::true_type{});
      int m0, n0, grp;
      origin_g(kc, m0, n0, grp);
      if constexpr (BIASG) {
        if (bias_on) {
          const float tot = bsum + __shfl_xor(bsum, 32, 64);
          const int m = m0 + wr * 128 + wc * 32 + (lane & 31);
          if (lane < 32) {
            if constexpr (SPLITK) {
              p.bias_ws[(long long)split_of(kc) * (p.nbm * BM) + m] = tot;
            } else if constexpr (EPI == EPI_TABLE) {
              if (m < tab[grp].grp.M) tab[grp].bias_out[m] = f2bf(tot);
            } else if (m < p.M) {
              p.bias_out[m] = f2bf(tot);
            }
          }
        }
      }
      if constexpr (SPLITK) {
        const int u = bid + kc * G, sp = u / tiles;
        epilogue_ws(p, acc, sp * tiles + (u - sp * tiles), wr * 128, wc * 64, lane);
      } else if constexpr (OUT_F32) {
        if constexpr (MULTI) {
          const Grp r = grp_of(grp);
          const Out o = {r.C, r.ldc, r.M, r.N};
          epilogue_f32(p, o, acc, m0 + wr * 128, n0 + wc * 64, lane);
        } else {
          const Out o = {p.C, p.ldc, p.M, p.N};
          epilogue_f32(p, o, acc, m0 + wr * 128, n0 + wc * 64, lane);
        }
      } else if constexpr (MULTI) {
        const Grp r = grp_of(grp);
        const Out o = {r.C, r.ldc, r.M, r.N};
        epilogue(p, o, acc, smem + (wave < 4 ? pb : pa) * SLOT + (wave & 3) * 8192, m0 + wr * 128, n0 + wc * 64, lane);
      } else {
        const Out o = {p.C, p.ldc, p.M, p.N};
        epilogue(p, o, acc, smem + (wave < 4 ? pb : pa) * SLOT + (wave & 3) * 8192, m0 + wr * 128, n0 + wc * 64, lane);
      }
      zero_acc();
      __builtin_amdgcn_s_waitcnt(0xc07f);
      __builtin_amdgcn_s_barrier();
      asm volatile("" : "+v"(lane));
      ra = Reader<AK, 4>(lane, wr * 128);
      rb = Reader<BK, 2>(lane, wc * 64);
      sA.set_voff(wave, lane);
      sB.set_voff(wave, lane);
      early_pieces(pb, pa);
    }
  }

  static __device__ __forceinline__ void epilogue_f32(const Params& p, const Out& o, Acc& acc, int wm0, int wn0, int lane) {
    const int l31 = lane & 31, hi = lane >> 5;
    float* C = reinterpret_cast<float*>(o.C);
    const bool add = p.accumulate != 0;
#pragma unroll
    for (int i = 0; i < 4; ++i) {
      const int m = wm0 + i * 32 + l31;
#pragma unroll
      for (int j = 0; j < 2; ++j)
#pragma unroll
        for (int g = 0; g < 4; ++g) {
          const int n = wn0 + j * 32 + 8 * g + 4 * hi;
          if (m < o.M && n < o.N) {
            f32x4_t* dst = reinterpret_cast<f32x4_t*>(C + (long long)m * o.ldc + n);
            f32x4_t v = {acc[i][j][4 * g], acc[i][j][4 * g + 1], acc[i][j][4 * g + 2], acc[i][j][4 * g + 3]};
            if (add) v += *dst;
            *dst = v;
          }
        }
    }
  }

  static __device__ __forceinline__ void epilogue_ws(const Params& p, Acc& acc, int slab, int lm0, int ln0, int lane) {
    const int l31 = lane & 31, hi = lane >> 5;
    float* base = p.ws + (long long)slab * (BM * BN);
#pragma unroll
    for (int i = 0; i < 4; ++i) {
      const int m = lm0 + i * 32 + l31;
#pragma unroll
      for (int j = 0; j < 2; ++j)
#pragma unroll
        for (int g = 0; g < 4; ++g) {
          const int n = ln0 + j * 32 + 8 * g + 4 * hi;
          const f32x4_t v = {acc[i][j][4 * g], acc[i][j][4 * g + 1], acc[i][j][4 * g + 2], acc[i][j][4 * g + 3]};
          *reinterpret_cast<f32x4_t*>(base + m * BN + n) = v;
        }
    }
  }

  static __device__ __forceinline__ void epilogue(const Params& p, const Out& o, Acc& acc, char* park, int wm0, int wn0,
                                                  int lane) {
    const int l31 = lane & 31, hi = lane >> 5;
    float bias_v[2][4][4];
    if (p.bias != nullptr) {
#pragma unroll
      for (int j = 0; j < 2; ++j)
#pragma unroll
        for (int g = 0; g < 4; ++g) {
          const int n = min(wn0 + j * 32 + 8 * g + 4 * hi, o.N - 4);
          const uint2 w = *reinterpret_cast<const uint2*>(p.bias + n);
          bias_v[j][g][0] = __uint_as_float(w.x << 16);
          bias_v[j][g][1] = __uint_as_float(w.x & 0xffff0000u);
          bias_v[j][g][2] = __uint_as_float(w.y << 16);
          bias_v[j][g][3] = __uint_as_float(w.y & 0xffff0000u);
        }
    }
    const bool acc_c = p.accumulate != 0 || p.addend != nullptr;
#pragma unroll
    for (int half = 0; half < 2; ++half) {
#pragma unroll
      for (int ii = 0; ii < 2; ++ii) {
        const int i = half * 2 + ii;
        const int row = ii * 32 + l31;
#pragma unroll
        for (int j = 0; j < 2; ++j)
#pragma unroll
          for (int g = 0; g < 4; ++g) {
            float v[4];
#pragma unroll
            for (int e = 0; e < 4; ++e) v[e] = acc[i][j][4 * g + e] + (p.bias != nullptr ? bias_v[j][g][e] : 0.f);
            const int chunk = (j * 4 + g) ^ (row & 7);
            const u32x2_t pk = {pack2bf(v[0], v[1]), pack2bf(v[2], v[3])};
            *reinterpret_cast<u32x2_t*>(park + row * 128 + chunk * 16 + hi * 8) = pk;
          }
      }
      asm volatile("s_waitcnt lgkmcnt(0)" ::: "memory");
#pragma unroll 4
      for (int it = 0; it < 8; ++it) {
        const int row = it * 8 + (lane >> 3), c = lane & 7;
        const u32x4_t pv = *reinterpret_cast<const u32x4_t*>(park + row * 128 + ((c ^ (row & 7)) << 4));
        uint4 v = make_uint4(pv.x, pv.y, pv.z, pv.w);
        const int m = wm0 + half * 64 + row, n = wn0 + c * 8;
        if (m < o.M && n < o.N) {
          bf16_t* dst = o.C + (long long)m * o.ldc + n;
          if (acc_c) {
            Vec16<bf16_t> o, nw;
            o.load(p.addend != nullptr ? p.addend + (long long)m * p.ldadd + n : dst);
            nw.raw = v;
            float fo[8], fn[8];
            o.unpack(fo);
            nw.unpack(fn);
#pragma unroll
            for (int e = 0; e < 8; ++e) fn[e] += fo[e];
            nw.pack(fn);
            v = nw.raw;
          }
          *reinterpret_cast<uint4*>(dst) = v;
        }
      }
      if constexpr (HAS_CT) {
#pragma unroll 2
        for (int it = 0; it < 8; ++it) {
          const int n_l = it * 8 + (lane >> 3), mg = lane & 7;
          uint32_t w[4];
#pragma unroll
          for (int e2 = 0; e2 < 4; ++e2) {
            uint32_t lo, hi16;
            {
              const int row = mg * 8 + 2 * e2;
              lo = *reinterpret_cast<const uint16_t*>(park + row * 128 + ((((n_l >> 3) ^ (row & 7))) << 4) + (n_l & 7) * 2);
            }
            {
              const int row = mg * 8 + 2 * e2 + 1;
              hi16 = *reinterpret_cast<const uint16_t*>(park + row * 128 + ((((n_l >> 3) ^ (row & 7))) << 4) + (n_l & 7) * 2);
            }
            w[e2] = lo | (hi16 << 16);
          }
          const int n = wn0 + n_l, m = wm0 + half * 64 + mg * 8;
          if (n < o.N && m < o.M)
            *reinterpret_cast<uint4*>(p.Ct + (long long)n * p.ldct + m) = make_uint4(w[0], w[1], w[2], w[3]);
        }
      }
    }
  }
};

template <bool AK, bool BK, bool HAS_CT, bool SPLITK = false, bool OUT_F32 = false, int EPI = EPI_PLAIN>
__global__ __launch_bounds__(NT, 2) void gemm_kernel(const Params p) {
  __shared__ __attribute__((aligned(1024))) char smem[LDS_BYTES];
  Kernel<AK, BK, HAS_CT, SPLITK, OUT_F32, EPI>::run(p, smem);
}

}
}
```

### touchnet_amd/csrc/gemm_table.hip

```cpp
#include "gemm_host.h"

namespace tn {
namespace gemm {

struct RecChunk {
  Rec r[TABCHUNK];
};
static_assert(sizeof(Rec) % 8 == 0 && sizeof(RecChunk) <= 3072, "a chunk of records fits the kernel-argument segment");
constexpr int REC_WORDS = (int)(sizeof(Rec) / 8);

__global__ __launch_bounds__(TABCHUNK * REC_WORDS) void table_upload_kernel(const RecChunk c, Rec* dst, int n) {
  const int t = threadIdx.x;
  if (t < n * REC_WORDS)
    reinterpret_cast<unsigned long long*>(dst)[t] = reinterpret_cast<const unsigned long long*>(&c)[t];
}

}
}

extern "C" {

long long tn_gemm_grouped_table_bytes(int n) { return n < 1 || n > MAXTAB ? -1 : (long long)n * (long long)sizeof(Rec); }

int tn_gemm_bf16_grouped_table(const void* const* A, const void* const* B, const long long* lda, const long long* ldb,
                               const int* K, void* const* C, const long long* ldc, const int* M, const int* N,
                               void* const* bias_grad, int n, int accumulate, int c_f32, void* table, long long table_bytes,
                               void* stream) {
  if (n < 1 || n > MAXTAB) return TN_EINVAL;
  if (table == nullptr || !aligned(15, table) || table_bytes < tn_gemm_grouped_table_bytes(n)) return TN_EINVAL;
  std::vector<RecChunk> chunks((n + TABCHUNK - 1) / TABCHUNK);
  long long total = 0;
  for (int g = 0; g < n; ++g) {
    Rec& r = chunks[g / TABCHUNK].r[g % TABCHUNK];
    if (total > 0x7fffffff) return TN_EINVAL;
    if (!grouped_product(A[g], B[g], lda[g], ldb[g], K[g], C[g], ldc[g], M[g], N[g], c_f32, (int)total, r.seg, r.grp))
      return TN_EINVAL;
    r.bias_out = bias_grad != nullptr ? (bf16_t*)bias_grad[g] : nullptr;
    if (!aligned(1, r.bias_out)) return TN_EINVAL;
    total += (long long)r.grp.nbm * r.grp.nbn;
  }
  if (total > 0x7fffffff) return TN_EINVAL;
  hipStream_t st = (hipStream_t)stream;
  for (int c = 0; c * TABCHUNK < n; ++c)
    hipLaunchKernelGGL(table_upload_kernel, dim3(1), dim3(TABCHUNK * REC_WORDS), 0, st, chunks[c],
                       (Rec*)table + c * TABCHUNK, min(TABCHUNK, n - c * TABCHUNK));
  Params p;
  clear_params(p);
  p.table = (const Rec*)table;
  p.ngrp = n;
  p.accumulate = accumulate;
  p.c_f32 = c_f32;
  p.ntiles = (int)total;
  if (c_f32)
    hipLaunchKernelGGL((gemm_kernel<true, true, false, false, true, EPI_TABLE>), grid_for(p.ntiles), dim3(NT), 0, st, p);
  else
    hipLaunchKernelGGL((gemm_kernel<true, true, false, false, false, EPI_TABLE>), grid_for(p.ntiles), dim3(NT), 0, st, p);
  TN_LAUNCH_CHECK();
  return TN_OK;
}

}
```

### touchnet_amd/csrc/optim.hip

```cpp
#include "common.h"

namespace tn {

constexpr int kSumsqBlocks = 1024;

template <typename T>
__global__ __launch_bounds__(256) void sumsq_partial_kernel(const T* __restrict__ g, float* __restrict__ partial,
                                                            size_t n) {
  constexpr int N = Vec16<T>::N;
  __shared__ float sm[4];
  float acc = 0.f;
  const size_t nvec = n / N;
  for (size_t v = (size_t)blockIdx.x * blockDim.x + threadIdx.x; v < nvec; v += (size_t)gridDim.x * blockDim.x) {
    Vec16<T> a;
    float f[N];
    a.load(g + v * N);
    a.unpack(f);
#pragma unroll
    for (int j = 0; j < N; ++j) acc += f[j] * f[j];
  }
  if (blockIdx.x == 0)
    for (size_t i = nvec * N + threadIdx.x; i < n; i += blockDim.x) {
      const float f = Elem<T>::ld(g + i);
      acc += f * f;
    }
  acc = block_sum(acc, sm);
  if (threadIdx.x == 0) partial[blockIdx.x] = acc;
}

__global__ __launch_bounds__(1024) void sumsq_final_kernel(const float* __restrict__ partial,
                                                           float* __restrict__ norm_sq, int nb) {
  __shared__ float sm[16];
  float acc = 0.f;
  for (int i = threadIdx.x; i < nb; i += blockDim.x) acc += partial[i];
  acc = block_sum(acc, sm);
  if (threadIdx.x == 0) norm_sq[0] += acc;
}

constexpr long long kSumsqChunk = 32768;

template <typename T>
__global__ __launch_bounds__(256) void sumsq_multi_kernel(const void* const* __restrict__ ptrs,
                                                          const long long* __restrict__ sizes,
                                                          const long long* __restrict__ first_chunk, int ntensors,
                                                          float* __restrict__ partial) {
  constexpr int N = Vec16<T>::N;
  __shared__ float sm[4];
  const long long c = blockIdx.x;
  int lo = 0, hi = ntensors - 1;
  while (lo < hi) {
    const int mid = (lo + hi + 1) >> 1;
    if (first_chunk[mid] <= c) lo = mid; else hi = mid - 1;
  }
  const T* g = static_cast<const T*>(ptrs[lo]);
  const long long beg = (c - first_chunk[lo]) * kSumsqChunk;
  const long long end = min(beg + kSumsqChunk, sizes[lo]);
  float acc = 0.f;
  if ((reinterpret_cast<uintptr_t>(g) & 15) == 0) {
    const long long nvec = (end - beg) / N;
    for (long long v = threadIdx.x; v < nvec; v += 256) {
      Vec16<T> a;
      float f[N];
      a.load(g + beg + v * N);
      a.unpack(f);
#pragma unroll
      for (int j = 0; j < N; ++j) acc += f[j] * f[j];
    }
    for (long long i = beg + nvec * N + threadIdx.x; i < end; i += 256) {
      const float f = Elem<T>::ld(g + i);
      acc += f * f;
    }
  } else {
    for (long long i = beg + threadIdx.x; i < end; i += 256) {
      const float f = Elem<T>::ld(g + i);
      acc += f * f;
    }
  }
  acc = block_sum(acc, sm);
  if (threadIdx.x == 0) partial[c] = acc;
}

template <typename G> __device__ __forceinline__ void load4(const G* g, size_t i, float (&f)[4]);
template <> __device__ __forceinline__ void load4<float>(const float* g, size_t i, float (&f)[4]) {
  const float4 t = reinterpret_cast<const float4*>(g)[i];
  f[0] = t.x; f[1] = t.y; f[2] = t.z; f[3] = t.w;
}
template <> __device__ __forceinline__ void load4<bf16_t>(const bf16_t* g, size_t i, float (&f)[4]) {
  const uint2 t = reinterpret_cast<const uint2*>(g)[i];
  f[0] = __uint_as_float(t.x << 16); f[1] = __uint_as_float(t.x & 0xffff0000u);
  f[2] = __uint_as_float(t.y << 16); f[3] = __uint_as_float(t.y & 0xffff0000u);
}

template <typename G>
__global__ __launch_bounds__(256) void adamw_kernel(float* __restrict__ p, float* __restrict__ m,
                                                    float* __restrict__ v, const G* __restrict__ g,
                                                    bf16_t* __restrict__ shadow, const float* __restrict__ norm_sq,
                                                    size_t n, float lr, float b1, float b2, float eps, float wd,
                                                    float max_norm, float bc1, float bc2) {
  const float nsq = norm_sq ? norm_sq[0] : 0.f;
  if (!(nsq == nsq) || nsq > 3.0e38f) return;
  float clip = 1.f;
  if (norm_sq && max_norm > 0.f) clip = fminf(1.f, max_norm / (sqrtf(nsq) + 1e-6f));
  const float step = lr / bc1, rs_bc2 = rsqrtf(bc2), decay = 1.f - lr * wd;
  const size_t n4 = n / 4;
  for (size_t i = (size_t)blockIdx.x * blockDim.x + threadIdx.x; i < n4; i += (size_t)gridDim.x * blockDim.x) {
    float4 pv = reinterpret_cast<float4*>(p)[i];
    float4 mv = reinterpret_cast<float4*>(m)[i];
    float4 vv = reinterpret_cast<float4*>(v)[i];
    float gf[4];
    load4<G>(g, i, gf);
#pragma unroll
    for (int j = 0; j < 4; ++j) gf[j] *= clip;
    float* pp = &pv.x;
    float* mp = &mv.x;
    float* vp = &vv.x;
#pragma unroll
    for (int j = 0; j < 4; ++j) {
      pp[j] *= decay;
      mp[j] = b1 * mp[j] + (1.f - b1) * gf[j];
      vp[j] = b2 * vp[j] + (1.f - b2) * gf[j] * gf[j];
      pp[j] -= step * mp[j] / (sqrtf(vp[j]) * rs_bc2 + eps);
    }
    reinterpret_cast<float4*>(p)[i] = pv;
    reinterpret_cast<float4*>(m)[i] = mv;
    reinterpret_cast<float4*>(v)[i] = vv;
    if (shadow) {
      uint2 s;
      s.x = pack2bf(pp[0], pp[1]);
      s.y = pack2bf(pp[2], pp[3]);
      reinterpret_cast<uint2*>(shadow)[i] = s;
    }
  }
  if (blockIdx.x == 0)
    for (size_t i = n4 * 4 + threadIdx.x; i < n; i += blockDim.x) {
      const float gi = Elem<G>::ld(g + i) * clip;
      float pi = p[i] * decay;
      const float mi = b1 * m[i] + (1.f - b1) * gi;
      const float vi = b2 * v[i] + (1.f - b2) * gi * gi;
      pi -= step * mi / (sqrtf(vi) * rs_bc2 + eps);
      p[i] = pi;
      m[i] = mi;
      v[i] = vi;
      if (shadow) shadow[i] = f2bf(pi);
    }
}

constexpr long long kAdamChunk = 16384;

__global__ void adamw_prepare_kernel(const float* __restrict__ norm_sq, float* __restrict__ state, float b1, float b2,
                                     float max_norm) {
  const float nsq = norm_sq ? norm_sq[0] : 0.f;
  const bool bad = !(nsq == nsq) || nsq > 3.0e38f;
  int step = __float_as_int(state[0]);
  if (!bad) ++step;
  state[0] = __int_as_float(step);
  const float fs = (float)(step < 1 ? 1 : step);
  state[1] = 1.f - powf(b1, fs);
  state[2] = 1.f - powf(b2, fs);
  state[3] = (norm_sq && max_norm > 0.f && !bad) ? fminf(1.f, max_norm / (sqrtf(nsq) + 1e-6f)) : 1.f;
  state[4] = bad ? 1.f : 0.f;
}

__device__ __forceinline__ void adamw_element(float& p, float& m, float& v, float g, float clip, float decay, float step,
                                              float rs_bc2, float b1, float b2, float omb1, float omb2, float eps) {
#pragma clang fp contract(off)
  const float gj = g * clip;
  m = __builtin_fmaf(omb1, gj, b1 * m);
  v = __builtin_fmaf(gj, omb2 * gj, b2 * v);
  const float upd = (step * m) / __builtin_fmaf(sqrtf(v), rs_bc2, eps);
  p = __builtin_fmaf(decay, p, -upd);
}

template <typename G>
__global__ __launch_bounds__(256) void adamw_multi_kernel(float* const* __restrict__ ps, float* const* __restrict__ ms,
                                                          float* const* __restrict__ vs,
                                                          const void* const* __restrict__ gs,
                                                          bf16_t* const* __restrict__ shadows,
                                                          const long long* __restrict__ sizes,
                                                          const long long* __restrict__ first_chunk, int ntensors,
                                                          long long nchunks,
                                                          const float* __restrict__ state, float lr, float b1, float b2,
                                                          float eps, float wd) {
  if (state[4] != 0.f) return;
  for (long long c = blockIdx.x; c < nchunks; c += gridDim.x) {
  int lo = 0, hi = ntensors - 1;
  while (lo < hi) {
    const int mid = (lo + hi + 1) >> 1;
    if (first_chunk[mid] <= c) lo = mid; else hi = mid - 1;
  }
  float* p = ps[lo];
  float* m = ms[lo];
  float* v = vs[lo];
  const G* g = static_cast<const G*>(gs[lo]);
  bf16_t* shadow = shadows[lo];
  const long long beg = (c - first_chunk[lo]) * kAdamChunk;
  const long long end = min(beg + kAdamChunk, sizes[lo]);
  const float clip = state[3];
  const float step = lr / state[1], rs_bc2 = rsqrtf(state[2]), decay = 1.f - lr * wd;
  const float omb1 = 1.f - b1, omb2 = 1.f - b2;
  const bool aligned = ((reinterpret_cast<uintptr_t>(p) | reinterpret_cast<uintptr_t>(m) |
                         reinterpret_cast<uintptr_t>(v) | reinterpret_cast<uintptr_t>(g) |
                         reinterpret_cast<uintptr_t>(shadow)) & 15) == 0;
  long long done = beg;
  if (aligned) {
    const long long n4 = (end - beg) / 4;
    const size_t base4 = (size_t)(beg / 4);
    for (long long i = threadIdx.x; i < n4; i += 256) {
      float4 pv = reinterpret_cast<float4*>(p)[base4 + i];
      float4 mv = reinterpret_cast<float4*>(m)[base4 + i];
      float4 vv = reinterpret_cast<float4*>(v)[base4 + i];
      float gf[4];
      load4<G>(g, base4 + i, gf);
      float* pp = &pv.x;
      float* mp = &mv.x;
      float* vp = &vv.x;
#pragma unroll
      for (int j = 0; j < 4; ++j)
        adamw_element(pp[j], mp[j], vp[j], gf[j], clip, decay, step, rs_bc2, b1, b2, omb1, omb2, eps);
      reinterpret_cast<float4*>(p)[base4 + i] = pv;
      reinterpret_cast<float4*>(m)[base4 + i] = mv;
      reinterpret_cast<float4*>(v)[base4 + i] = vv;
      if (shadow) reinterpret_cast<uint2*>(shadow)[base4 + i] = make_uint2(pack2bf(pp[0], pp[1]), pack2bf(pp[2], pp[3]));
    }
    done = beg + n4 * 4;
  }
  for (long long i = done + threadIdx.x; i < end; i += 256) {
    float pi = p[i], mi = m[i], vi = v[i];
    adamw_element(pi, mi, vi, Elem<G>::ld(g + i), clip, decay, step, rs_bc2, b1, b2, omb1, omb2, eps);
    p[i] = pi;
    m[i] = mi;
    v[i] = vi;
    if (shadow) shadow[i] = f2bf(pi);
  }
  }
}

}

using namespace tn;

extern "C" {

int tn_sumsq_scratch_floats(void) { return kSumsqBlocks; }

int tn_sumsq(const void* g, float* scratch, float* norm_sq, long long n, int dtype, void* stream) {
  if (n <= 0) return TN_EINVAL;
  hipStream_t st = (hipStream_t)stream;
  int nb = (int)((n / 8 + 255) / 256);
  nb = nb < 1 ? 1 : (nb > kSumsqBlocks ? kSumsqBlocks : nb);
  if (dtype == 0)
    hipLaunchKernelGGL((sumsq_partial_kernel<float>), dim3(nb), dim3(256), 0, st, (const float*)g, scratch,
                       (size_t)n);
  else if (dtype == 1)
    hipLaunchKernelGGL((sumsq_partial_kernel<bf16_t>), dim3(nb), dim3(256), 0, st, (const bf16_t*)g, scratch,
                       (size_t)n);
  else
    return TN_EINVAL;
  TN_LAUNCH_CHECK();
  hipLaunchKernelGGL(sumsq_final_kernel, dim3(1), dim3(1024), 0, st, scratch, norm_sq, nb);
  TN_LAUNCH_CHECK();
  return TN_OK;
}

long long tn_sumsq_multi_chunk(void) { return kSumsqChunk; }

int tn_sumsq_multi(const void* const* ptrs, const long long* sizes, const long long* first_chunk, int ntensors,
                   long long nchunks, float* partial, float* norm_sq, int dtype, void* stream) {
  if (ntensors <= 0 || nchunks <= 0 || nchunks > 0x7fffffffLL) return TN_EINVAL;
  hipStream_t st = (hipStream_t)stream;
  if (dtype == 0)
    hipLaunchKernelGGL((sumsq_multi_kernel<float>), dim3((unsigned)nchunks), dim3(256), 0, st, ptrs, sizes, first_chunk,
                       ntensors, partial);
  else if (dtype == 1)
    hipLaunchKernelGGL((sumsq_multi_kernel<bf16_t>), dim3((unsigned)nchunks), dim3(256), 0, st, ptrs, sizes,
                       first_chunk, ntensors, partial);
  else
    return TN_EINVAL;
  TN_LAUNCH_CHECK();
  hipLaunchKernelGGL(sumsq_final_kernel, dim3(1), dim3(1024), 0, st, partial, norm_sq, (int)nchunks);
  TN_LAUNCH_CHECK();
  return TN_OK;
}

int tn_adamw_step(float* p, float* m, float* v, const void* g, void* p_shadow_bf16, const float* norm_sq,
                  long long n, float lr, float beta1, float beta2, float eps, float weight_decay, float max_norm,
                  float bias_corr1, float bias_corr2, int g_dtype, void* stream) {
  if (n <= 0) return TN_EINVAL;
  hipStream_t st = (hipStream_t)stream;
  size_t nb = ((size_t)n / 4 + 255) / 256;
  nb = nb < 1 ? 1 : (nb > 8192 ? 8192 : nb);
  if (g_dtype == 0)
    hipLaunchKernelGGL((adamw_kernel<float>), dim3((int)nb), dim3(256), 0, st, p, m, v, (const float*)g,
                       (bf16_t*)p_shadow_bf16, norm_sq, (size_t)n, lr, beta1, beta2, eps, weight_decay, max_norm,
                       bias_corr1, bias_corr2);
  else if (g_dtype == 1)
    hipLaunchKernelGGL((adamw_kernel<bf16_t>), dim3((int)nb), dim3(256), 0, st, p, m, v, (const bf16_t*)g,
                       (bf16_t*)p_shadow_bf16, norm_sq, (size_t)n, lr, beta1, beta2, eps, weight_decay, max_norm,
                       bias_corr1, bias_corr2);
  else
    return TN_EINVAL;
  TN_LAUNCH_CHECK();
  return TN_OK;
}

long long tn_adamw_multi_chunk(void) { return kAdamChunk; }

int tn_adamw_prepare(const float* norm_sq, float* state, float beta1, float beta2, float max_norm, void* stream) {
  if (state == nullptr) return TN_EINVAL;
  hipLaunchKernelGGL(adamw_prepare_kernel, dim3(1), dim3(1), 0, (hipStream_t)stream, norm_sq, state, beta1, beta2,
                     max_norm);
  TN_LAUNCH_CHECK();
  return TN_OK;
}

int tn_adamw_multi_bounded(void* const* ps, void* const* ms, void* const* vs, const void* const* gs,
                           void* const* shadows, const long long* sizes, const long long* first_chunk, int ntensors,
                           long long nchunks, const float* state, float lr, float beta1, float beta2, float eps,
                           float weight_decay, int g_dtype, int max_workgroups, void* stream) {
  if (ntensors <= 0 || nchunks <= 0 || nchunks > 0x7fffffffLL || state == nullptr || max_workgroups < 0) return TN_EINVAL;
  hipStream_t st = (hipStream_t)stream;
  const unsigned grid = (unsigned)((max_workgroups > 0 && max_workgroups < nchunks) ? max_workgroups : nchunks);
  if (g_dtype == 0)
    hipLaunchKernelGGL((adamw_multi_kernel<float>), dim3(grid), dim3(256), 0, st, (float* const*)ps,
                       (float* const*)ms, (float* const*)vs, gs, (bf16_t* const*)shadows, sizes, first_chunk, ntensors,
                       nchunks, state, lr, beta1, beta2, eps, weight_decay);
  else if (g_dtype == 1)
    hipLaunchKernelGGL((adamw_multi_kernel<bf16_t>), dim3(grid), dim3(256), 0, st, (float* const*)ps,
                       (float* const*)ms, (float* const*)vs, gs, (bf16_t* const*)shadows, sizes, first_chunk, ntensors,
                       nchunks, state, lr, beta1, beta2, eps, weight_decay);
  else
    return TN_EINVAL;
  TN_LAUNCH_CHECK();
  return TN_OK;
}

int tn_adamw_multi(void* const* ps, void* const* ms, void* const* vs, const void* const* gs, void* const* shadows,
                   const long long* sizes, const long long* first_chunk, int ntensors, long long nchunks,
                   const float* state, float lr, float beta1, float beta2, float eps, float weight_decay, int g_dtype,
                   void* stream) {
  return tn_adamw_multi_bounded(ps, ms, vs, gs, shadows, sizes, first_chunk, ntensors, nchunks, state, lr, beta1, beta2,
                                eps, weight_decay, g_dtype, 0, stream);
}

}
```

### touchnet_amd/functional.py

```python
from __future__ import annotations

import ctypes
import math
import os
import weakref
from dataclasses import dataclass
from typing import Optional

import torch

from . import _C
from . import library as L

_cur = _C.stream
_p = _C.ptr


def _c(t: torch.Tensor) -> torch.Tensor:
    return t if t.is_contiguous() else t.contiguous()


def rms_norm(x, weight, eps, residual=None):
    y, h, _ = L.rmsnorm_fwd(x, residual, weight, float(eps))
    return (y, h) if residual is not None else y
# ... 181 lines not shown
    loss, stats, _ = L.ce_fwd(logits, lab, sl, ns, int(ignore_index))
    return loss, stats.detach()


class _FusedLinearCE(torch.autograd.Function):

    @staticmethod
    def forward(ctx, hidden, weight, labels, sentence_lens, num_sentence, ignore_index, chunk, compact=False, tp=None):
        H = hidden.shape[-1]
        h2 = hidden.reshape(-1, H)
        lab = labels.reshape(-1).to(torch.int64).contiguous()
        sl = sentence_lens.reshape(-1).to(torch.int64).contiguous()
        rows = None
        overflow = None
        if compact is not False and compact is not None:
            n_all = h2.shape[0]
            labelled = lab != ignore_index
            if compact is True:
                rows = torch.nonzero(labelled).squeeze(1)
            else:
                n_max = min(int(compact), n_all)
                rows = torch.nonzero_static(labelled, size=max(n_max, 1), fill_value=0).squeeze(1)
                count = labelled.sum()
                valid = torch.arange(rows.numel(), device=lab.device) < count
                overflow = count > n_max
            if rows.numel() == 0:
                rows = None
            else:
                h2, lab, sl = h2.index_select(0, rows), lab.index_select(0, rows), sl.index_select(0, rows)
                if compact is not True:
                    lab = torch.where(valid, lab, torch.full_like(lab, ignore_index))
        n, V = h2.shape[0], weight.shape[0]
        ns = _num_sentence_dev(num_sentence, hidden.device)
        one = torch.ones(1, dtype=torch.float32, device=hidden.device)
        dh = torch.empty_like(h2)
        dw = None
        parts = []
        lab_k = lab
        if tp is not None:
            from touchnet_amd.models.tensor_parallel import tp_all_reduce
            group, tp_rank, _ = tp
            v0 = tp_rank * V
            mine = (lab >= v0) & (lab < v0 + V)
            lab_k = torch.where(lab == ignore_index, lab, torch.where(mine, lab - v0, torch.full_like(lab, V)))
        for s in range(0, n, chunk):
            e = min(s + chunk, n)
            logits = _mm_tn(h2[s:e], weight)
            nll_c, lse_c, hit_c = L.ce_fwd_rows(logits, lab_k[s:e], sl[s:e], ns, int(ignore_index))
            if tp is not None:
                valid = lab[s:e] != ignore_index
                target = lse_c - nll_c
                top_v, top_i = logits.float().max(dim=1)
                mx = torch.where(valid, lse_c, torch.full_like(lse_c, float("-inf")))
                tp_all_reduce(mx, group, torch.distributed.ReduceOp.MAX)
                se = torch.where(valid, torch.exp(lse_c - mx), torch.zeros_like(lse_c))
                tp_all_reduce(se, group)
                tp_all_reduce(target, group)
                lse_c = torch.where(valid, mx + torch.log(se), torch.zeros_like(lse_c))
                nll_c = torch.where(valid, lse_c - target, torch.zeros_like(lse_c))
                best = torch.stack([top_v, (top_i + v0).float()], dim=1)
                if not getattr(group, "emulated", False):
                    size = torch.distributed.get_world_size(group)
                    every = torch.empty((size * best.shape[0], 2), dtype=best.dtype, device=best.device)
                    torch.distributed.all_gather_into_tensor(every, best.contiguous(), group=group)
                    every = every.view(size, best.shape[0], 2)
                    win = every[..., 0].argmax(dim=0)
                    best = every.gather(0, win[None, :, None].expand(1, -1, 2))[0]
                hit_c = ((best[:, 1].to(torch.int64) == lab[s:e]) & valid).to(hit_c.dtype)
            L.ce_bwd_(logits, lab_k[s:e], sl[s:e], lse_c, ns, one, int(ignore_index))
            parts.append((nll_c, hit_c))
            _dgrad([logits], [weight], out=dh[s:e], dgrad_tn=False)
            if dw is None and n > chunk and logits.dtype == torch.bfloat16:
                dw = torch.zeros(V, H, dtype=torch.float32, device=h2.device)
            dw = _wgrad_unowned(logits, h2[s:e], out=dw, accumulate=dw is not None)
            del logits
        if dw.dtype != h2.dtype:
            dw = dw.to(h2.dtype)
        nll = torch.cat([a for a, _ in parts]) if len(parts) > 1 else parts[0][0]
        hit = torch.cat([b for _, b in parts]) if len(parts) > 1 else parts[0][1]
        out = L.ce_reduce(nll, hit, lab, sl, ns, int(ignore_index))
        if rows is not None:
            dh = torch.zeros(n_all, H, dtype=dh.dtype, device=dh.device).index_add_(0, rows, dh)
        if overflow is not None:
            poison = torch.where(overflow, float("nan"), 1.0)
            out = out * poison.to(out.dtype)
            dh = dh * poison.to(dh.dtype)
            dw = dw * poison.to(dw.dtype) if dw is not None else dw
        ctx.save_for_backward(dh, dw)
        ctx.hshape, ctx.wdtype = hidden.shape, weight.dtype
        ctx.mark_non_differentiable(out)
        return out[0].clone(), out

    @staticmethod
    def backward(ctx, g_loss, _g):
        dh, dw = ctx.saved_tensors
        g = g_loss.to(torch.float32)
        return ((dh * g.to(dh.dtype)).view(ctx.hshape), (dw * g.to(dw.dtype)).to(ctx.wdtype), None, None, None, None, None,
                None, None)


def fused_linear_cross_entropy(hidden, weight, labels, sentence_lens, num_sentence, ignore_index=-100,
                               chunk_tokens=4096, compact=False, tp=None):
    return _FusedLinearCE.apply(hidden, weight, labels, sentence_lens, num_sentence, ignore_index, chunk_tokens,
                                compact, tp)


def transpose_2d(x: torch.Tensor, out: Optional[torch.Tensor] = None) -> torch.Tensor:
    if x.dim() != 2 or x.dtype != torch.bfloat16 or not (x.is_cuda or x.is_meta) or x.stride(1) != 1:
        raise RuntimeError("transpose_2d: expects a 2-D bf16 device tensor with contiguous rows")
    R, Cn = x.shape
    if out is None:
        out = torch.empty(Cn, R, dtype=x.dtype, device=x.device)
    L.transpose_bf16_(x, out)
    return out


def column_sum(x: torch.Tensor) -> torch.Tensor:
    R, Cn = x.shape
    if x.dtype != torch.bfloat16 or not (x.is_cuda or x.is_meta) or x.stride(1) != 1 or Cn % 8 or x.stride(0) % 8:
        return x.sum(0)
    return L.colsum_bf16(x)


def _out_or_new(name, out, accumulate, M, N, device):
    if out is not None:
        return out
    if accumulate:
        raise _C.KernelError(f"{name}: accumulate needs an output to add to")
    return torch.empty(M, N, dtype=torch.bfloat16, device=device)


def gemm_tn(a: torch.Tensor, b: torch.Tensor, bias: Optional[torch.Tensor] = None, out: Optional[torch.Tensor] = None,
            accumulate: bool = False, out_t: Optional[torch.Tensor] = None) -> torch.Tensor:
    if a.dim() != 2 or b.dim() != 2 or a.dtype != torch.bfloat16 or b.dtype != torch.bfloat16:
        raise _C.KernelError("gemm_tn: 2-D bf16 operands only")
    if a.stride(1) != 1 or b.stride(1) != 1 or a.shape[1] != b.shape[1]:
        raise _C.KernelError("gemm_tn: operands must be contraction-contiguous [M, K] / [N, K]")
    M, K = a.shape
    N = b.shape[0]
    out = _out_or_new("gemm_tn", out, accumulate, M, N, a.device)
    if out.stride(1) != 1 or tuple(out.shape) != (M, N):
        raise _C.KernelError("gemm_tn: bad `out`")
    if bias is not None:
        bias = _c(bias).to(a.dtype)
    _C.check(_C.lib().tn_gemm_bf16_tn(_p(a), _p(b), _p(out), _p(out_t), _p(bias), M, N, K, a.stride(0), b.stride(0),
                                      out.stride(0), out_t.stride(0) if out_t is not None else 0, int(accumulate),
                                      _cur()), "tn_gemm_bf16_tn")
    return out


def gemm(segs, a_kmaj: bool = False, b_kmaj: bool = False, bias: Optional[torch.Tensor] = None,
         out: Optional[torch.Tensor] = None, accumulate: bool = False,
         out_t: Optional[torch.Tensor] = None, bias_grad: Optional[torch.Tensor] = None,
         addend: Optional[torch.Tensor] = None) -> torch.Tensor:
    if not 1 <= len(segs) <= 3:
        raise _C.KernelError("gemm: 1..3 segments")
    for a, b in segs:
        if a.dim() != 2 or b.dim() != 2 or a.dtype != torch.bfloat16 or b.dtype != torch.bfloat16:
            raise _C.KernelError("gemm: 2-D bf16 operands only")
        if a.stride(1) != 1 or b.stride(1) != 1:
            raise _C.KernelError("gemm: operands need contiguous rows")
    a0, b0 = segs[0]
    M = a0.shape[1] if a_kmaj else a0.shape[0]
    N = b0.shape[1] if b_kmaj else b0.shape[0]
    Ks = []
    for a, b in segs:
        Ka, Ma = (a.shape[0], a.shape[1]) if a_kmaj else (a.shape[1], a.shape[0])
        Kb, Nb = (b.shape[0], b.shape[1]) if b_kmaj else (b.shape[1], b.shape[0])
        if Ka != Kb or Ma != M or Nb != N:
            raise _C.KernelError(f"gemm: segment shapes disagree: a {tuple(a.shape)} b {tuple(b.shape)}")
        Ks.append(Ka)
    out = _out_or_new("gemm", out, accumulate, M, N, a0.device)
    n = len(segs)
    f32 = out.dtype == torch.float32
    wgrad_mode = a_kmaj and b_kmaj and n == 1 and bias is None and out_t is None
    if f32:
        if not wgrad_mode:
            raise _C.KernelError("gemm: fp32 output exists for the single-segment weight-gradient mode only")
        if out.stride(1) != 1 or tuple(out.shape) != (M, N) or not a0.is_cuda:
            raise _C.KernelError("gemm: bad fp32 `out`")
    else:
        if out.stride(1) != 1 or tuple(out.shape) != (M, N) or out.dtype != torch.bfloat16:
            raise _C.KernelError("gemm: bad `out`")
        if bias is not None:
            bias = _c(bias).to(torch.bfloat16)
        if not a0.is_cuda:
            raise _C.KernelError("touchnet_amd kernels need device (HIP) tensors; got a CPU tensor")
        if addend is not None:
            if (n != 1 or accumulate or out_t is not None or bias_grad is not None or addend.dtype != torch.bfloat16
                    or tuple(addend.shape) != (M, N) or addend.stride(1) != 1 or addend.data_ptr() == out.data_ptr()):
                raise _C.KernelError("gemm: addend needs one segment, a bf16 [M, N] matrix with contiguous rows that is not `out`")
            _C.check(_C.lib().tn_gemm_bf16_addend(_p(a0), _p(b0), a0.stride(0), b0.stride(0), Ks[0], int(a_kmaj), int(b_kmaj),
                                                  _p(out), _p(bias), _p(addend), addend.stride(0), M, N, out.stride(0), _cur()),
                     "tn_gemm_bf16_addend")
            return out
    lib = _C.lib()
    if f32 or bias_grad is not None:
        if not wgrad_mode:
            raise _C.KernelError("gemm: bias_grad exists for the single-segment weight-gradient mode only")
        split = split_k(M, N, Ks[0], True, True) if SPLIT_K else 1
        ws, ws_bytes = _splitk_workspace(M, N, split, bias_grad is not None, a0.device)
        if bias_grad is None:
            _C.check(lib.tn_gemm_bf16_wgrad_f32(_p(a0), _p(b0), a0.stride(0), b0.stride(0), Ks[0], _p(out), M, N, out.stride(0),
                                                int(accumulate), split, _p(ws), ws_bytes, _cur()), "tn_gemm_bf16_wgrad_f32")
        else:
            _check_bias_grad(bias_grad, M, a0)
            _C.check(lib.tn_gemm_bf16_wgrad_bias(_p(a0), _p(b0), a0.stride(0), b0.stride(0), Ks[0], _p(out), _p(bias_grad), M, N,
                                                 out.stride(0), int(accumulate), int(f32), split, _p(ws), ws_bytes, _cur()),
                     "tn_gemm_bf16_wgrad_bias")
        return out
    split = split_k(M, N, Ks[0], a_kmaj, b_kmaj) if n == 1 and out_t is None and SPLIT_K else 1
    if split > 1:
        ws, ws_bytes = _splitk_workspace(M, N, split, False, a0.device)
        _C.check(lib.tn_gemm_bf16_splitk(_p(a0), _p(b0), a0.stride(0), b0.stride(0), Ks[0], int(a_kmaj), int(b_kmaj), _p(out),
                                         _p(bias), M, N, out.stride(0), int(accumulate), split, 0, _p(ws), ws_bytes, _cur()),
                 "tn_gemm_bf16_splitk")
        return out
    _C.check(lib.tn_gemm_bf16(*_operand_arrays(segs), _carr(ctypes.c_int, Ks), n, int(a_kmaj), int(b_kmaj), _p(out), _p(out_t),
                              _p(bias), M, N, out.stride(0), out_t.stride(0) if out_t is not None else 0, int(accumulate),
                              _cur()), "tn_gemm_bf16")
    return out


def _splitk_workspace(M, N, split, with_bias_grad, device):
    if split <= 1:
        return None, 0
    need = int(_C.lib().tn_gemm_splitk_workspace_bytes(M, N, split, int(with_bias_grad), 0))
    return torch.empty(need // 4, dtype=torch.float32, device=device), need


def _carr(ctype, values):
    return (ctype * len(values))(*values)


def _operand_arrays(pairs):
    return (_carr(ctypes.c_void_p, [a.data_ptr() for a, _ in pairs]), _carr(ctypes.c_void_p, [b.data_ptr() for _, b in pairs]),
            _carr(ctypes.c_longlong, [a.stride(0) for a, _ in pairs]), _carr(ctypes.c_longlong, [b.stride(0) for _, b in pairs]))


def _check_bias_grad(bias_grad, M, like):
    if (bias_grad.dtype != torch.bfloat16 or bias_grad.dim() != 1 or bias_grad.numel() != M or not bias_grad.is_contiguous()
            or bias_grad.device != like.device):
        raise _C.KernelError("gemm: bias_grad must be a contiguous bf16 [M] device vector")


def _check_grouped(name, pairs, outs, accumulate):
    for a, b in pairs:
        if (a.dim() != 2 or b.dim() != 2 or a.dtype != torch.bfloat16 or b.dtype != torch.bfloat16 or a.stride(1) != 1
                or b.stride(1) != 1 or a.shape[0] != b.shape[0] or not a.is_cuda):
            raise _C.KernelError(f"{name}: pairs of 2-D bf16 device matrices [K, M] / [K, N] with contiguous rows")
    if outs is None:
        outs = [_out_or_new(name, None, accumulate, a.shape[1], b.shape[1], a.device) for a, b in pairs]
    for o, (a, b) in zip(outs, pairs):
        if (o.dtype != outs[0].dtype or o.dtype not in (torch.float32, torch.bfloat16) or o.stride(1) != 1
                or tuple(o.shape) != (a.shape[1], b.shape[1])):
            raise _C.KernelError(f"{name}: bad `outs`")
    return outs


def gemm_grouped_wgrad(pairs, outs=None, accumulate: bool = False):
    n = len(pairs)
    if not 1 <= n <= 3:
        raise _C.KernelError("gemm_grouped_wgrad: 1..3 products")
    outs = _check_grouped("gemm_grouped_wgrad", pairs, outs, accumulate)
    f32 = outs[0].dtype == torch.float32
    Ms = _carr(ctypes.c_int, [a.shape[1] for a, _ in pairs])
    Ns = _carr(ctypes.c_int, [b.shape[1] for _, b in pairs])
    Ks = _carr(ctypes.c_int, [a.shape[0] for a, _ in pairs])
    need = int(_C.lib().tn_gemm_grouped_workspace_bytes(Ms, Ns, Ks, n))
    ws = torch.empty(need // 4, dtype=torch.float32, device=outs[0].device) if need > 0 else None
    Ap, Bp, la, lb = _operand_arrays(pairs)
    _C.check(_C.lib().tn_gemm_bf16_grouped(Ap, Bp, la, lb, Ks, _carr(ctypes.c_void_p, [o.data_ptr() for o in outs]),
                                           _carr(ctypes.c_longlong, [o.stride(0) for o in outs]), Ms, Ns, n, 1, 1,
                                           int(accumulate), int(f32), _p(ws), need, _cur()), "tn_gemm_bf16_grouped")
    return list(outs)


GROUPED_TABLE_MAX = 1024


def gemm_grouped_table_wgrad(pairs, outs=None, accumulate: bool = False, bias_grads=None):
    n = len(pairs)
    if not 1 <= n <= GROUPED_TABLE_MAX:
        raise _C.KernelError(f"gemm_grouped_table_wgrad: 1..{GROUPED_TABLE_MAX} products")
    outs = _check_grouped("gemm_grouped_table_wgrad", pairs, outs, accumulate)
    if bias_grads is None:
        bias_grads = [None] * n
    for bg, (a, _) in zip(bias_grads, pairs):
        if bg is not None:
            _check_bias_grad(bg, a.shape[1], a)
    lib = _C.lib()
    need = int(lib.tn_gemm_grouped_table_bytes(n))
    table = torch.empty(need, dtype=torch.uint8, device=outs[0].device)
    Ap, Bp, la, lb = _operand_arrays(pairs)
    _C.check(lib.tn_gemm_bf16_grouped_table(
        Ap, Bp, la, lb, _carr(ctypes.c_int, [a.shape[0] for a, _ in pairs]),
        _carr(ctypes.c_void_p, [o.data_ptr() for o in outs]), _carr(ctypes.c_longlong, [o.stride(0) for o in outs]),
        _carr(ctypes.c_int, [a.shape[1] for a, _ in pairs]), _carr(ctypes.c_int, [b.shape[1] for _, b in pairs]),
        _carr(ctypes.c_void_p, [bg.data_ptr() if bg is not None else None for bg in bias_grads]), n, int(accumulate),
        int(outs[0].dtype == torch.float32), _p(table), need, _cur()), "tn_gemm_bf16_grouped_table")
    return list(outs)


def gemm_swiglu_fwd(x2: torch.Tensor, w_gate: torch.Tensor, w_up: torch.Tensor):
    M, K = x2.shape
    I = w_gate.shape[0]
    if not _bf16_rows(x2, w_gate, w_up) or w_up.shape != w_gate.shape or w_gate.shape[1] != K or w_gate.stride(0) != w_up.stride(0):
        raise _C.KernelError("gemm_swiglu_fwd: bf16 device matrices x [M, K], w_gate / w_up [I, K] of one row pitch")
    gate, up, act = (torch.empty(M, I, dtype=torch.bfloat16, device=x2.device) for _ in range(3))
    _C.check(_C.lib().tn_gemm_bf16_swiglu_fwd(_p(x2), _p(w_gate), _p(w_up), _p(gate), _p(up), _p(act), M, I, K, x2.stride(0),
                                              w_gate.stride(0), I, _cur()), "tn_gemm_bf16_swiglu_fwd")
    return gate, up, act


def gemm_gelu_fwd(x2: torch.Tensor, w: torch.Tensor, bias: Optional[torch.Tensor]):
    M, K = x2.shape
    N = w.shape[0]
    if not _bf16_rows(x2, w) or w.shape[1] != K or (bias is not None and (bias.dtype != torch.bfloat16 or bias.numel() != N)):
        raise _C.KernelError("gemm_gelu_fwd: bf16 device matrices x [M, K], w [N, K], bias [N]")
    pre, act = (torch.empty(M, N, dtype=torch.bfloat16, device=x2.device) for _ in range(2))
    _C.check(_C.lib().tn_gemm_bf16_gelu_fwd(_p(x2), _p(w), _p(_c(bias)) if bias is not None else None, _p(pre), _p(act), M, N,
                                            K, x2.stride(0), w.stride(0), N, _cur()), "tn_gemm_bf16_gelu_fwd")
    return pre, act


def gemm_gelu_bwd(dy2: torch.Tensor, w2: torch.Tensor, pre: torch.Tensor):
    M, H = dy2.shape
    I = w2.shape[1]
    if not _bf16_rows(dy2, w2, pre) or w2.shape[0] != H or tuple(pre.shape) != (M, I) or pre.stride(0) != I:
        raise _C.KernelError("gemm_gelu_bwd: bf16 device matrices dy [M, H], w2 [H, I], dense pre [M, I]")
    dpre = torch.empty(M, I, dtype=torch.bfloat16, device=dy2.device)
    _C.check(_C.lib().tn_gemm_bf16_gelu_bwd(_p(dy2), _p(w2), _p(pre), _p(dpre), M, I, H, dy2.stride(0), w2.stride(0), I,
                                            _cur()), "tn_gemm_bf16_gelu_bwd")
    return dpre


def gemm_swiglu_bwd(dy2: torch.Tensor, w_down: torch.Tensor, gate: torch.Tensor, up: torch.Tensor):
    M, H = dy2.shape
    I = w_down.shape[1]
    if (not _bf16_rows(dy2, w_down, gate, up) or w_down.shape[0] != H or tuple(gate.shape) != (M, I) or gate.shape != up.shape
            or gate.stride(0) != up.stride(0)):
        raise _C.KernelError("gemm_swiglu_bwd: bf16 device matrices dy [M, H], w_down [H, I], gate / up [M, I]")
    dgate = torch.empty(M, I, dtype=torch.bfloat16, device=dy2.device)
    dup = torch.empty(M, I, dtype=torch.bfloat16, device=dy2.device)
    if gate.stride(0) != I:
        raise _C.KernelError("gemm_swiglu_bwd: gate / up must be dense [M, I]")
    _C.check(_C.lib().tn_gemm_bf16_swiglu_bwd(_p(dy2), _p(w_down), _p(gate), _p(up), _p(dgate), _p(dup), M, I, H,
                                              dy2.stride(0), w_down.stride(0), I, _cur()), "tn_gemm_bf16_swiglu_bwd")
    return dgate, dup


def gemm_rope(x2: torch.Tensor, weight: torch.Tensor, bias: Optional[torch.Tensor], cos: torch.Tensor, sin: torch.Tensor,
              head_dim: int) -> torch.Tensor:
    M, K = x2.shape
    N = weight.shape[0]
    if (not _bf16_rows(x2, weight) or weight.shape[1] != K or cos.dtype != torch.bfloat16 or sin.dtype != torch.bfloat16
            or tuple(cos.shape) != (M, head_dim // 2) or tuple(sin.shape) != (M, head_dim // 2)
            or not cos.is_contiguous() or not sin.is_contiguous()):
        raise _C.KernelError("gemm_rope: bf16 x [M, K], weight [N, K], cos / sin [M, head_dim / 2]")
    if bias is not None:
        bias = _c(bias).to(torch.bfloat16)
    out = torch.empty(M, N, dtype=torch.bfloat16, device=x2.device)
    _C.check(_C.lib().tn_gemm_bf16_rope(_p(x2), _p(weight), _p(bias), _p(cos), _p(sin), _p(out), M, N, K, x2.stride(0),
                                        weight.stride(0), N, int(head_dim), _cur()), "tn_gemm_bf16_rope")
    return out


def rope_epilogue_ok(M: int, N: int, K: int, head_dim: int) -> bool:
    return (ROPE_EPILOGUE and _own(M, N, (K,)) and _whole_unsplit(M, N, K)
            and ((head_dim == 128 and N % 256 == 0) or (head_dim == 64 and N % 64 == 0)))


def _rope_epilogue_own(x2, w, rope) -> bool:
    (M, K), cos, D = x2.shape, rope[0], rope[2]
    return (rope_epilogue_ok(M, w.shape[0], K, D) and _bf16_rows(x2, w) and cos.dtype == torch.bfloat16
            and tuple(cos.shape) == (M, D // 2))


def _rotated(y2, rope):
    cos, sin, D = rope[:3]
    M = y2.shape[0]
    y4 = y2.view(1, M, -1, D)
    return L.rope_apply(y4, y4.new_empty(1, M, 0, D), cos, sin, False)[0].view(M, -1)


def _whole_unsplit(M: int, N: int, K: int) -> bool:
    return K % 64 == 0 and (not SPLIT_K or split_k(M, N, K, False, False) == 1)


ROPE_EPILOGUE = True
MLP_EPILOGUE = True
GROUPED_WGRAD = True
SPLIT_K = True
_NUM_CU = 256


def split_k(M: int, N: int, K: int, a_kmaj: bool, b_kmaj: bool) -> int:
    tiles = ((M + 255) // 256) * ((N + 255) // 256)
    stages = (K + 63) // 64
    if tiles * 2 > _NUM_CU or stages < 16:
        return 1
    s = min(_NUM_CU // tiles, stages // 8)
    if not (a_kmaj and b_kmaj):
        while s > 1 and stages % s:
            s -= 1
    return max(s, 1)


def gemm_supported(M: int, N: int, Ks, a_kmaj: bool = False, b_kmaj: bool = False) -> bool:
    k_ok = all(k > 0 and (k % 64 == 0 or (a_kmaj and b_kmaj)) for k in Ks)
    return k_ok and N % 8 == 0 and M > 0 and (not a_kmaj or M % 8 == 0)


LINEAR_GEMM = os.environ.get("TN_LINEAR_GEMM", "own")
_OWN_MIN_TILES = 96


def _own_configured() -> bool:
    return LINEAR_GEMM == "own"


def _own(M: int, N: int, Ks, a_kmaj: bool = False, b_kmaj: bool = False) -> bool:
    if not (_own_configured() and gemm_supported(M, N, Ks, a_kmaj, b_kmaj)):
        return False
    tiles = ((M + 255) // 256) * ((N + 255) // 256)
    if tiles >= _OWN_MIN_TILES:
        return True
    return SPLIT_K and len(Ks) == 1 and tiles * split_k(M, N, Ks[0], a_kmaj, b_kmaj) >= _OWN_MIN_TILES


def _bf16_rows(*ts, meta_ok: bool = False) -> bool:
    return all((t.is_cuda or (meta_ok and t.is_meta)) and t.dtype == torch.bfloat16 and t.dim() == 2 and t.stride(1) == 1
               and t.stride(0) % 8 == 0 and (t.is_meta or t.data_ptr() % 16 == 0) for t in ts)


def _transposable(*ts) -> bool:
    return all(t.dtype == torch.bfloat16 and (t.is_cuda or t.is_meta) and t.shape[0] % 8 == 0 and t.shape[1] % 8 == 0
               for t in ts)


def _fwd_own(a, b, bias=None) -> bool:
    return (_own(a.shape[0], b.shape[0], (a.shape[1],)) and _bf16_rows(a, b)
            and (bias is None or bias.dtype == torch.bfloat16))


def _mm_tn(a: torch.Tensor, b: torch.Tensor, bias: Optional[torch.Tensor] = None, out: Optional[torch.Tensor] = None,
           accumulate: bool = False) -> torch.Tensor:
    if _fwd_own(a, b, bias):
        return gemm([(a, b)], bias=bias, out=out, accumulate=accumulate)
    if accumulate:
        return out.addmm_(a, b.t())
    if out is not None:
        return torch.mm(a, b.t(), out=out) if bias is None else torch.addmm(bias, a, b.t(), out=out)
    return torch.nn.functional.linear(a, b, bias)


def _dgrad_own(dys, ws, out=None) -> bool:
    return (_own(dys[0].shape[0], ws[0].shape[1], [w.shape[0] for w in ws])
            and _bf16_rows(*dys, *ws, *(() if out is None else (out,))))


def _dgrad(dys, ws, out: Optional[torch.Tensor] = None, dgrad_tn: bool = True) -> torch.Tensor:
    if _dgrad_own(dys, ws, out):
        for i in range(0, len(ws), 3):
            out = gemm(list(zip(dys[i:i + 3], ws[i:i + 3])), b_kmaj=True, out=out, accumulate=i > 0)
        return out
    if dgrad_tn and _transposable(*dys, *ws):
        wts = [transpose_2d(w) for w in ws]
        out = _mm_tn(dys[0], wts[0], out=out)
        for d, wt in zip(dys[1:], wts[1:]):
            _mm_tn(d, wt, out=out, accumulate=True)
        return out
    out = torch.mm(dys[0], ws[0]) if out is None else torch.mm(dys[0], ws[0], out=out)
    for d, w in zip(dys[1:], ws[1:]):
        out.addmm_(d, w)
    return out


BIAS_IN_WGRAD = True


def _wgrad_own(dy, x2, queued: bool = False) -> bool:
    shape = (dy.shape[1], x2.shape[1], (dy.shape[0],), True, True)
    return (dy.shape[0] == x2.shape[0] and _bf16_rows(dy, x2, meta_ok=queued)
            and (_own_configured() and gemm_supported(*shape) if queued else _own(*shape)))


WGRAD_STREAM = None
WGRAD_MAIN = None
WGRAD_RETURNS_NEED_SYNC = False


def enable_wgrad_stream(on: bool = True) -> None:
    global WGRAD_STREAM
    WGRAD_STREAM = torch.cuda.Stream(priority=int(os.environ.get("TN_WGRAD_STREAM_PRIORITY", "-1"))) if on else None


def wgrad_streams():
    out = [torch.cuda.current_stream()]
    for st in (WGRAD_STREAM, WGRAD_MAIN if WGRAD_STREAM is not None else None):
        if st is not None and all(st != o for o in out):
            out.append(st)
    return out


def sync_wgrad_stream() -> None:
    if WGRAD_STREAM is not None:
        torch.cuda.current_stream().wait_stream(WGRAD_STREAM)


def _beside(inputs, fn, written=()):
    side = WGRAD_STREAM
    if side is None:
        return fn()
    global WGRAD_MAIN
    main = torch.cuda.current_stream()
    WGRAD_MAIN = main
    side.wait_stream(main)
    with torch.cuda.stream(side):
        out = fn()
    for t in inputs:
        t.record_stream(side)
    wait = False
    for t in written:
        if t is not None:
            t.record_stream(side)
            wait = True
    outs = out if isinstance(out, (list, tuple)) else (out,)
    for t in outs:
        if isinstance(t, torch.Tensor):
            t.record_stream(main)
            wait = wait or WGRAD_RETURNS_NEED_SYNC
    if wait:
        main.wait_stream(side)
    return out


GRAD_SINKS = {}


def _live(table, w):
    ref = table.get(id(w))
    return ref() if ref is not None else None


def _sink_of(w):
    sink = _live(GRAD_SINKS, w)
    return sink if sink is not None and sink.owns(w) else None


DEFERRED_WGRAD = True
DEFERRED_WGRAD_FLUSH_LAYERS = 11
WGRAD_QUEUES = {}


def _queue_of(w):
    return _live(WGRAD_QUEUES, w)


class DeferredWgrad:

    def __init__(self, layers, flush_layers: int = DEFERRED_WGRAD_FLUSH_LAYERS):
        if flush_layers < 1:
            raise ValueError("DeferredWgrad: flush_layers >= 1")
        self.flush_layers = flush_layers
        self.launch = gemm_grouped_table_wgrad
        self.enabled = True
        self._owned = {}
        self._items = []
        self._waiting = set()
        self._layers = set()
        self.flushes = 0
        for li, layer in enumerate(layers):
            for w, b in layer:
                self._owned[id(w)] = (w, b, li)
                WGRAD_QUEUES[id(w)] = weakref.ref(self)

    def __len__(self):
        return len(self._items)

    def close(self):
        if self._items:
            raise _C.KernelError("DeferredWgrad.close: the queue is not empty")
        for k in self._owned:
            ref = WGRAD_QUEUES.get(k)
            if ref is not None and ref() is self:
                del WGRAD_QUEUES[k]
        self._owned = {}

    def push(self, w, dy, x2, with_bias: bool) -> bool:
        own = self._owned.get(id(w))
        if not self.enabled or own is None or own[0] is not w:
            return False
        _, bias, layer = own
        if id(w) in self._waiting:
            raise _C.KernelError("DeferredWgrad: a weight was queued twice without a flush in between "
                                 "(two backward passes through one layer: flush between them)")
        ok = (_wgrad_own(dy, x2, queued=True) and w.dtype == torch.bfloat16 and tuple(w.shape) == (dy.shape[1], x2.shape[1])
              and (not with_bias or (bias is not None and bias.dtype == torch.bfloat16))
              and (w.grad is None or (w.grad.dtype == torch.bfloat16 and w.grad.is_contiguous()
                                      and (w.grad.is_meta or w.grad.data_ptr() % 16 == 0))))
        if not ok:
            return False
        if layer not in self._layers and len(self._layers) >= self.flush_layers:
            self.flush()
        self._items.append((w, dy, x2, bias if with_bias else None, torch.cuda.current_stream() if dy.is_cuda else None))
        self._waiting.add(id(w))
        self._layers.add(layer)
        return True

    def flush(self) -> None:
        items, self._items = self._items, []
        self._waiting.clear()
        self._layers.clear()
        if not items:
            return
        self.flushes += 1
        cur = torch.cuda.current_stream() if items[0][1].is_cuda else None
        for w, dy, x2, _, st in items:
            if st is not None and st != cur:
                cur.wait_stream(st)
                dy.record_stream(cur)
                x2.record_stream(cur)
        parts = {acc: [it for it in items if (it[0].grad is not None) == acc] for acc in (False, True)}
        for acc, part in parts.items():
            for i in range(0, len(part), GROUPED_TABLE_MAX):
                chunk = part[i:i + GROUPED_TABLE_MAX]
                outs = [w.grad if acc else torch.empty(w.shape, dtype=torch.bfloat16, device=dy.device)
                        for w, dy, _, _, _ in chunk]
                bgs = [torch.empty(dy.shape[1], dtype=torch.bfloat16, device=dy.device) if b is not None else None
                       for _, dy, _, b, _ in chunk]
                self.launch([(dy, x2) for _, dy, x2, _, _ in chunk], outs=outs, accumulate=acc, bias_grads=bgs)
                for (w, _, _, b, _), o, bg in zip(chunk, outs, bgs):
                    if not acc:
                        w.grad = o
                    if b is not None:
                        if b.grad is None:
                            b.grad = bg
                        else:
                            b.grad.add_(bg)


def _queue_wgrad(w, dy, x2, with_bias: bool) -> bool:
    if not DEFERRED_WGRAD or WGRAD_STREAM is not None:
        return False
    q = _queue_of(w)
    return q is not None and _sink_of(w) is None and q.push(w, dy, x2, with_bias)


def _route_wgrad(w, dy, x2, want_bias: bool = False):
    ride = bool(want_bias and BIAS_IN_WGRAD)
    if _queue_wgrad(w, dy, x2, ride):
        return None, None, True
    if not _wgrad_own(dy, x2):
        return None, None, False
    sink = _sink_of(w)
    db = torch.empty(dy.shape[1], dtype=torch.bfloat16, device=dy.device) if ride else None

    def launch():
        if sink is None:
            return gemm([(dy, x2)], True, True, bias_grad=db)
        view, acc = sink.take(w)
        gemm([(dy, x2)], True, True, out=view, accumulate=acc, bias_grad=db)
        sink.done(w)
    return _beside((dy, x2), launch, written=(db,)), db, True


def _bias_left(want_bias, taken) -> bool:
    return bool(want_bias and not (taken and BIAS_IN_WGRAD))


def _wgrad_lib(dys, x2, layout: str = "nt", out: Optional[torch.Tensor] = None, accumulate: bool = False):
    n, (M, K), Ns = len(dys), x2.shape, [d.shape[1] for d in dys]
    if layout == "nt_fused" and n > 1:
        st = _stacked_view(dys)
        if st is not None:
            return list(torch.bmm(st.transpose(1, 2), x2.unsqueeze(0).expand(n, M, K)).unbind(0))
        return list(torch.split(torch.mm(torch.cat(dys, dim=1).t(), x2), Ns, dim=0))
    if layout == "tn" and _transposable(x2, *dys):
        xt = transpose_2d(_c(x2))
        dyt = torch.empty(sum(Ns), M, dtype=x2.dtype, device=x2.device)
        o = 0
        for d, N in zip(dys, Ns):
            transpose_2d(d, out=dyt[o:o + N])
            o += N
        return list(torch.split(_mm_tn(dyt, xt), Ns, dim=0))
    if out is None:
        return [torch.mm(d.t(), x2) for d in dys]
    (d,) = dys
    if out.dtype != d.dtype:
        d, x2 = d.float(), x2.float()
    return [out.addmm_(d.t(), x2) if accumulate else torch.mm(d.t(), x2, out=out)]


def _wgrad_unowned(dy, x2, out: Optional[torch.Tensor] = None, accumulate: bool = False) -> torch.Tensor:
    if _wgrad_own(dy, x2):
        return gemm([(dy, x2)], True, True, out=out, accumulate=accumulate)
    return _wgrad_lib([dy], x2, out=out, accumulate=accumulate)[0]


def _wgrads(ws, dys, x2, want_w, want_b, layout: str = "nt"):
    n = len(ws)
    dws, dbs, want_b = [None] * n, [None] * n, list(want_b)
    left = [i for i in range(n) if want_w[i]]
    for i in [i for i in left if dys[i].is_cuda]:
        dws[i], dbs[i], taken = _route_wgrad(ws[i], dys[i], x2, want_b[i])
        want_b[i] = _bias_left(want_b[i], taken)
        if taken:
            left.remove(i)
    if left:
        for i, dw in zip(left, _wgrad_lib([dys[i] for i in left], x2, layout if len(left) == n else "nt")):
            dws[i] = dw
    return dws, [column_sum(d) if nb else b for b, nb, d in zip(dbs, want_b, dys)]


def _wgrad_one(w, dy, x2):
    return _wgrads([w], [dy], x2, [True], [False])[0][0]


def _wgrad_group(items):
    sinks = [_sink_of(w) for w, _, _ in items]
    owned = sum(sk is not None for sk in sinks)
    if not all(_wgrad_own(dy, x2) for _, dy, x2 in items) or 0 < owned < len(items):
        return [_wgrad_one(*it) for it in items]
    pairs = [(dy, x2) for _, dy, x2 in items]

    def launch():
        if not owned:
            return gemm_grouped_wgrad(pairs)
        taken = [sk.take(w) for sk, (w, _, _) in zip(sinks, items)]
        if len({(v.dtype, bool(acc)) for v, acc in taken}) == 1:
            gemm_grouped_wgrad(pairs, outs=[v for v, _ in taken], accumulate=bool(taken[0][1]))
        else:
            for (view, acc), pair in zip(taken, pairs):
                gemm([pair], True, True, out=view, accumulate=acc)
        for sk, (w, _, _) in zip(sinks, items):
            sk.done(w)
        return [None] * len(items)
    return _beside([t for pair in pairs for t in pair], launch)


def _stacked_view(ts):
    t0 = ts[0]
    if t0.dim() != 2 or not all(t.shape == t0.shape and t.dtype == t0.dtype and t.is_contiguous() for t in ts):
        return None
    step = t0.numel()
    try:
        base = t0.untyped_storage().data_ptr()
        if not all(t.untyped_storage().data_ptr() == base and t.storage_offset() == t0.storage_offset() + i * step
                   for i, t in enumerate(ts)):
            return None
    except (RuntimeError, NotImplementedError):
        return None
    return t0.as_strided((len(ts), t0.shape[0], t0.shape[1]), (step, t0.shape[1], 1))


class _LinearGroup(torch.autograd.Function):

    @staticmethod
    def forward(ctx, x, n, wgrad, dgrad_tn, extra, *wb):
        ws, bs = wb[:n], wb[n:]
        src, rope = extra
        ctx.rope = rope
        if src is not None:
            ctx.save_for_backward(src[0], *ws, src[1])
            ctx.src_eps, ctx.xshape = float(src[2]), x.shape
        else:
            ctx.save_for_backward(x, *ws)
            ctx.src_eps = None
        ctx.has_bias = [b is not None for b in bs]
        ctx.wgrad, ctx.dgrad_tn = wgrad, dgrad_tn
        x2 = _c(x.reshape(-1, x.shape[-1]))
        at_once = _own_configured() and x.is_cuda
        outs = []
        for i, (w, b) in enumerate(zip(ws, bs)):
            w = _c(w)
            if rope is None or i not in rope[3]:
                y = _mm_tn(x2, w, b)
            elif _rope_epilogue_own(x2, w, rope):
                y = gemm_rope(x2, w, b, *rope[:3])
            else:
                y = _mm_tn(x2, w, b)
                if at_once:
                    y = _rotated(y, rope)
            outs.append(y)
        if rope is not None and not at_once:
            for i in rope[3]:
                outs[i] = _rotated(outs[i], rope)
        return tuple(y.view(*x.shape[:-1], y.shape[-1]) for y in outs)

    @staticmethod
    def backward(ctx, *dys):
        x, *ws = ctx.saved_tensors
        if ctx.src_eps is not None:
            norm_w = ws.pop()
            x = L.rmsnorm_fwd(x, None, norm_w, ctx.src_eps)[0].view(ctx.xshape)
        n = len(ws)
        x2 = _c(x.reshape(-1, x.shape[-1]))
        M = x2.shape[0]
        dys = [torch.zeros(M, w.shape[0], dtype=x.dtype, device=x.device) if d is None else _c(d).reshape(M, -1)
               for d, w in zip(dys, ws)]
        if ctx.rope is not None and not ctx.rope[4]:
            cos, sin, D, which = ctx.rope[:4]
            which = sorted(which)
            for a in range(0, len(which), 2):
                i, j = which[a], which[a + 1] if a + 1 < len(which) else None
                gi = dys[i].view(1, M, -1, D)
                gj = dys[j].view(1, M, -1, D) if j is not None else gi.new_empty(1, M, 0, D)
                ri, rj = L.rope_apply(gi, gj, cos, sin, True)
                dys[i] = ri.view(M, -1)
                if j is not None:
                    dys[j] = rj.view(M, -1)
        need = ctx.needs_input_grad
        dx = _dgrad(dys, [_c(w) for w in ws], dgrad_tn=ctx.dgrad_tn).view(x.shape) if need[0] else None
        dws, dbs = _wgrads(ws, dys, x2, need[5:5 + n], [hb and nb for hb, nb in zip(ctx.has_bias, need[5 + n:])], ctx.wgrad)
        return (dx, None, None, None, None, *dws, *dbs)


def norm_source(h, norm_weight, eps):
    return (h.detach(), norm_weight.detach(), float(eps))


def _norm_src_describes(norm_src, x) -> bool:
    return (norm_src is not None and tuple(norm_src[0].shape) == tuple(x.shape) and norm_src[0].dtype == x.dtype
            and norm_src[1].shape[-1] == x.shape[-1])


def linear_group(x, layers, wgrad: str = "tn", dgrad_tn: bool = True, norm_src=None, rope=None,
                 rope_grad_in_attention: bool = False):
    if wgrad not in ("tn", "nt", "nt_fused"):
        raise ValueError(f"linear_group: wgrad={wgrad!r}")
    if not (x.is_cuda or x.is_meta):
        raise _C.KernelError("linear_group: device tensors only (the product path has no CPU fallback)")
    ws = [w for w, _ in layers]
    bs = [b for _, b in layers]
    if not _norm_src_describes(norm_src, x):
        norm_src = None
    if rope is not None:
        rope = (rope[0].detach(), rope[1].detach(), int(rope[2]), tuple(int(i) for i in rope[3]),
                bool(rope_grad_in_attention))
    return list(_LinearGroup.apply(x, len(ws), wgrad, dgrad_tn, (norm_src, rope), *ws, *bs))


class _SwiGLUMLP(torch.autograd.Function):

    @staticmethod
    def forward(ctx, x, wg, wu, wd, src=None):
        K, I = x.shape[-1], wg.shape[0]
        x2 = _c(x.reshape(-1, K))
        M = x2.shape[0]
        own = _own(M, I, (K,)) and _own(M, K, (I,)) and _own(I, K, (M,), True, True) and _own(K, I, (M,), True, True)
        fused = own and MLP_EPILOGUE and _bf16_rows(x2, wg, wu, wd) and wg.stride(0) == wu.stride(0)
        if fused:
            gate, up, act = gemm_swiglu_fwd(x2, wg, wu)
            kept = act
        else:
            gate, up = _mm_tn(x2, _c(wg)), _mm_tn(x2, _c(wu))
            if own:
                act = L.swiglu_fwd(gate, up)
                kept = act
            else:
                act, kept = L.swiglu_fwd_t(gate, up)
        y = _mm_tn(act, _c(wd))
        if src is not None and own:
            ctx.save_for_backward(src[0].reshape(-1, K), gate, up, src[1], wg, wu, wd)
            ctx.src_eps = float(src[2])
        else:
            ctx.save_for_backward(x2, gate, up, kept, wg, wu, wd)
            ctx.src_eps = None
        ctx.xshape, ctx.own, ctx.fused = x.shape, own, fused
        return y.view(*x.shape[:-1], wd.shape[0])

    @staticmethod
    def backward(ctx, dy):
        x2, gate, up, kept, wg, wu, wd = ctx.saved_tensors
        if ctx.src_eps is not None:
            x2 = L.rmsnorm_fwd(x2, None, kept, ctx.src_eps)[0]
            kept = L.swiglu_fwd(gate, up)
        M, K = x2.shape
        I, H = wg.shape[0], wd.shape[0]
        dy2 = _c(dy).reshape(M, H)
        nx, ng, nu, nd = ctx.needs_input_grad[:4]
# ... 374 lines not shown
```

### touchnet_amd/utils/optimizer.py

```python
from __future__ import annotations

import os
from typing import Any, Dict, Iterable, List, Optional

import torch

from touchnet_amd import _C


def _local(t: torch.Tensor) -> torch.Tensor:
    return t._local_tensor if hasattr(t, "_local_tensor") else t


def _shard_groups(params) -> List[Any]:
    groups, seen = [], set()
    for p in params:
        mesh = getattr(p, "device_mesh", None)
        if mesh is None:
            continue
        for d, pl in enumerate(p.placements):
            if pl.is_shard() and mesh.size(d) > 1 and (id(mesh), d) not in seen:
                seen.add((id(mesh), d))
                groups.append(mesh.get_group(d))
    return groups


class FusedAdamW:
    def __init__(self, params: Iterable, lr=8e-4, betas=(0.9, 0.95), eps=1e-8,
                 weight_decay=0.1, max_norm: float = 1.0, process_group=None, tp_group=None, tp_param_ids=()):
        items = list(params)
        if items and isinstance(items[0], (tuple, list)):
            items = [(n, p) for n, p in items if p.requires_grad]
            self.names = [n.replace("_checkpoint_wrapped_module.", "") for n, _ in items]
            self.params = [p for _, p in items]
        else:
            self.params = [p for p in items if p.requires_grad]
            self.names = [f"param.{i}" for i in range(len(self.params))]
        if len(set(self.names)) != len(self.names):
            raise ValueError("FusedAdamW: parameter names must be unique")
        self.tp_group = tp_group
        self._tp_index = {i for i, p in enumerate(self.params) if id(p) in set(tp_param_ids)}
        self.lr, self.betas, self.eps, self.weight_decay, self.max_norm = lr, betas, eps, weight_decay, max_norm
        self.groups = [process_group] if process_group is not None else _shard_groups(self.params)
        dev = _local(self.params[0]).device
        self.state = []
        for p in self.params:
            lp = _local(p.data)
            master = lp if lp.dtype == torch.float32 else lp.detach().float().clone()
            self.state.append(dict(master=master, m=torch.zeros_like(master), v=torch.zeros_like(master)))
        self.norm_sq = torch.zeros(1, dtype=torch.float32, device=dev)
        self.step_state = torch.zeros(8, dtype=torch.float32, device=dev)
        self._partial, self._keep = None, None
        self._pipe = None
        self._pipe_delay_cycles = 0
        self.side_workgroups = int(os.environ.get("TN_ADAMW_SIDE_WORKGROUPS", "128"))

    def pipeline_updates(self, groups: List[List[int]]) -> None:
        if any(hasattr(p, "_local_tensor") for p in self.params):
            raise ValueError("pipeline_updates: sharded parameters are updated by their data-parallel engine's schedule")
        seen = sorted(i for g in groups for i in g)
        if seen != list(range(len(self.params))):
            raise ValueError("pipeline_updates: the groups must cover every parameter exactly once")
        of = {i: gi for gi, g in enumerate(groups) for i in g}
        self._pipe = ([list(g) for g in groups], of, torch.cuda.Stream(),
                      [torch.cuda.Event() for _ in groups], list(range(len(groups))))

    def set_launch_order(self, order: List[int]) -> None:
        if sorted(order) != list(range(len(self._pipe[0]))):
            raise ValueError("set_launch_order: a permutation of the group indices")
        self._pipe[4][:] = list(order)

    def wait_group(self, gi: int) -> None:
        if self._pipe is not None:
            torch.cuda.current_stream().wait_event(self._pipe[3][gi])

    def wait_updates(self) -> None:
        if self._pipe is not None:
            torch.cuda.current_stream().wait_stream(self._pipe[2])

    @staticmethod
    def _table(rows, device):
        t = torch.tensor(rows, dtype=torch.int64).pin_memory()
        return t.to(device, non_blocking=True)

    def _sumsq(self, by_dtype):
        lib, p_, st = _C.lib(), _C.ptr, _C.stream
        chunk = int(lib.tn_sumsq_multi_chunk())
        keep = []
        for dt, items in by_dtype.items():
            gs = [g for _, g in items]
            sizes = [g.numel() for g in gs]
            first, tot = [], 0
            for n in sizes:
                first.append(tot)
                tot += (n + chunk - 1) // chunk
            table = self._table([[g.data_ptr() for g in gs], sizes, first], gs[0].device)
            if self._partial is None or self._partial.numel() < tot:
                self._partial = torch.empty(tot, dtype=torch.float32, device=gs[0].device)
            _C.check(lib.tn_sumsq_multi(p_(table[0]), p_(table[1]), p_(table[2]), len(gs), tot, p_(self._partial),
                                        p_(self.norm_sq), _C.dcode(gs[0]), st()), "tn_sumsq_multi")
            keep.append((table, gs))
        return keep

    def zero_grad(self, set_to_none: bool = True):
        for p in self.params:
            if set_to_none:
                p.grad = None
            elif p.grad is not None:
                p.grad.zero_()

    @torch.no_grad()
    def step(self, lr: Optional[float] = None) -> torch.Tensor:
        lib, p_, st = _C.lib(), _C.ptr, _C.stream
        lr = self.lr if lr is None else lr
        b1, b2 = self.betas
        self.wait_updates()
        self.norm_sq.zero_()
        by_dtype: Dict[torch.dtype, list] = {}
        for i, p in enumerate(self.params):
            if p.grad is None:
                continue
            g = _local(p.grad).contiguous()
            if g.numel():
                by_dtype.setdefault(g.dtype, []).append((i, g))
        if self.tp_group is not None and self._tp_index:
            pick = lambda inside: {dt: [it for it in items if (it[0] in self._tp_index) == inside]
                                   for dt, items in by_dtype.items()}
            drop_empty = lambda d: {dt: v for dt, v in d.items() if v}
            keep = self._sumsq(drop_empty(pick(True)))
            from touchnet_amd.models.tensor_parallel import tp_all_reduce
            tp_all_reduce(self.norm_sq, self.tp_group)
            keep += self._sumsq(drop_empty(pick(False)))
        else:
            keep = self._sumsq(by_dtype)
        for grp in self.groups:
            torch.distributed.all_reduce(self.norm_sq, group=grp)
        _C.check(lib.tn_adamw_prepare(p_(self.norm_sq), p_(self.step_state), b1, b2, float(self.max_norm), st()),
                 "tn_adamw_prepare")
        chunk = int(lib.tn_adamw_multi_chunk())
        if self._pipe is None:
            launches = [(None, items) for items in by_dtype.values()]
        else:
            groups, of = self._pipe[0], self._pipe[1]
            launches = []
            for gi in self._pipe[4]:
                for items in by_dtype.values():
                    sub = [it for it in items if of[it[0]] == gi]
                    launches.append((gi, sub))
        rows = [[], [], [], [], [], [], []]
        spans = []
        for gi, items in launches:
            tot, a = 0, len(rows[0])
            for i, g in items:
                s = self.state[i]
                lp = _local(self.params[i].data)
                rows[0].append(s["master"].data_ptr())
                rows[1].append(s["m"].data_ptr())
                rows[2].append(s["v"].data_ptr())
                rows[3].append(g.data_ptr())
                rows[4].append(lp.data_ptr() if lp.dtype == torch.bfloat16 else 0)
                rows[5].append(g.numel())
                rows[6].append(tot)
                tot += (g.numel() + chunk - 1) // chunk
            spans.append((gi, a, len(rows[0]), tot, _C.dcode(items[0][1]) if items else 0))
        if rows[0]:
            t = self._table(rows, _local(self.params[0]).device)
            keep.append(t)

            bound = 0 if self._pipe is None else self.side_workgroups

            def launch(a, b, tot, code):
                _C.check(lib.tn_adamw_multi_bounded(p_(t[0][a:b]), p_(t[1][a:b]), p_(t[2][a:b]), p_(t[3][a:b]),
                                                    p_(t[4][a:b]), p_(t[5][a:b]), p_(t[6][a:b]), b - a, tot,
                                                    p_(self.step_state), float(lr), b1, b2, self.eps, self.weight_decay,
                                                    code, bound, st()), "tn_adamw_multi_bounded")
            if self._pipe is None:
                for _, a, b, tot, code in spans:
                    launch(a, b, tot, code)
            else:
                side, events = self._pipe[2], self._pipe[3]
                side.wait_stream(torch.cuda.current_stream())
                with torch.cuda.stream(side):
                    if self._pipe_delay_cycles:
                        torch.cuda._sleep(int(self._pipe_delay_cycles))
                    for k, (gi, a, b, tot, code) in enumerate(spans):
                        if b > a:
                            launch(a, b, tot, code)
                        if k + 1 == len(spans) or spans[k + 1][0] != gi:
                            events[gi].record(side)
        self._keep = keep
        return self.norm_sq.sqrt().squeeze(0)

    @property
    def step_count(self) -> int:
        return int(self.step_state[:1].view(torch.int32).item())

    def _as_saved(self, i: int, t: torch.Tensor) -> torch.Tensor:
        p = self.params[i]
        mesh = getattr(p, "device_mesh", None)
        if mesh is None:
            return t
        from torch.distributed.tensor import DTensor
        return DTensor.from_local(t, mesh, p.placements, run_check=False, shape=p.shape, stride=p.stride())

    def state_dict(self) -> Dict[str, Any]:
        self.wait_updates()
        return {"step_state": self.step_state.clone(),
                "state": {n: {"master": self._as_saved(i, s["master"]), "exp_avg": self._as_saved(i, s["m"]),
                              "exp_avg_sq": self._as_saved(i, s["v"])}
                          for i, (n, s) in enumerate(zip(self.names, self.state))},
                "hyper": {"lr": self.lr, "betas": tuple(self.betas), "eps": self.eps,
                          "weight_decay": self.weight_decay, "max_norm": self.max_norm}}

    @torch.no_grad()
    def load_state_dict(self, sd: Dict[str, Any]) -> None:
        st = sd["state"]
        self.wait_updates()
        if len(st) != len(self.state):
            raise ValueError(f"optimizer state has {len(st)} tensors, this optimizer {len(self.state)}")
        self.step_state.copy_(sd["step_state"])
        for i, (n, s) in enumerate(zip(self.names, self.state)):
            src = st[n] if n in st else st[i] if i in st else st[str(i)]
            for key, dst in (("master", s["master"]), ("exp_avg", s["m"]), ("exp_avg_sq", s["v"])):
                t = _local(src[key])
                if t.shape != dst.shape:
                    raise ValueError(f"optimizer state {n}.{key}: shard shape {tuple(t.shape)} != {tuple(dst.shape)}")
                if t.data_ptr() != dst.data_ptr():
                    dst.copy_(t)
            lp = _local(self.params[i].data)
            if lp.dtype == torch.bfloat16:
                lp.copy_(s["master"])
        h = sd.get("hyper", {})
        self.lr = h.get("lr", self.lr)


def update_groups(model: torch.nn.Module, names: List[str]):
    strip = lambda n: n.replace("_checkpoint_wrapped_module.", "")
    blocks = []
    for name, mod in model.named_modules():
        if isinstance(mod, torch.nn.ModuleList) and not any(strip(name).startswith(p + ".") for p, _ in blocks):
            for cname, child in mod.named_children():
                if any(True for _ in child.parameters()):
                    blocks.append((strip(f"{name}.{cname}" if name else cname), child))
    owner = []
    for n in names:
        hit = [bi for bi, (p, _) in enumerate(blocks) if n.startswith(p + ".")]
        owner.append(hit[0] if hit else None)
    inside = [i for i, o in enumerate(owner) if o is not None]
    last = max(inside) if inside else -1
    early = [i for i, o in enumerate(owner) if o is None and i < last]
    late = [i for i, o in enumerate(owner) if o is None and i > last]
    groups, out = [early], []
    for bi, (_, mod) in enumerate(blocks):
        mine = [i for i, o in enumerate(owner) if o == bi]
        if mine:
            out.append((mod, len(groups)))
            groups.append(mine)
    groups.append(late)
    return groups, out


def pipeline_updates_under_forward(model: torch.nn.Module, optimizer: "FusedAdamW"):
    groups, blocks = update_groups(model, optimizer.names)
    optimizer.pipeline_updates(groups)
    late, last_block = len(groups) - 1, (blocks[-1][1] if blocks else None)
    at_entry = [0] if blocks else [0, late]
    fired, learning = [], [True]

    def entry(m, a):
        if learning[0]:
            optimizer.wait_updates()
        for gi in at_entry:
            optimizer.wait_group(gi)

    def block(gi):
        def hook(m, a):
            if learning[0] and gi not in fired:
                fired.append(gi)
            optimizer.wait_group(gi)
        return hook

    def first_forward_done(m, a, o):
        if not learning[0]:
            return
        learning[0] = False
        silent = [gi for _, gi in blocks if gi not in fired]
        at_entry.extend(silent)
# ... 53 lines not shown
```

Before: 23000.

## Fuse gradient sum-of-squares into wgrad GEMM epilogues for clip-norm

Wgrad GEMM epilogues (plain, grouped, split-k reduce) now also write per-tile partial sums of squares of the bf16 gradient into a per-weight slot arena held by a ledger. At optimizer step, gradients the ledger confirms were written unchanged skip the separate sumsq_multi pass over gradient memory, and only a small range-sum kernel over the slot arena runs. This removes a full read of most weight gradients per step, in exchange for extra epilogue work and register pressure in the GEMM, plus bookkeeping based on data_ptr and version checks. It applies only when there are no shard groups, no TP group and no DTensor parameters.

```diff
diff --git a/include/touchnet_amd.h b/include/touchnet_amd.h
--- a/include/touchnet_amd.h
+++ b/include/touchnet_amd.h
@@ -89,6 +89,9 @@
 long long tn_sumsq_multi_chunk(void);
 int tn_sumsq_multi(const void* const* ptrs, const long long* sizes, const long long* first_chunk, int ntensors,
                    long long nchunks, float* partial, float* norm_sq, int dtype, void* stream);
+long long tn_sum_ranges_chunk(void);
+int tn_sum_ranges(const void* const* ptrs, const long long* sizes, const long long* first_chunk, int nranges,
+                  long long nchunks, float* partial, float* norm_sq, void* stream);
 int tn_adamw_step(float* p, float* m, float* v, const void* g, void* p_shadow_bf16, const float* norm_sq,
                   long long n, float lr, float beta1, float beta2, float eps, float weight_decay, float max_norm,
                   float bias_corr1, float bias_corr2, int g_dtype, void* stream);
@@ -148,6 +151,18 @@
                                const int* K, void* const* C, const long long* ldc, const int* M, const int* N,
                                void* const* bias_grad, int n, int accumulate, int c_f32, void* table,
                                long long table_bytes, void* stream);
+long long tn_gemm_wgrad_sumsq_floats(int M, int N);
+int tn_gemm_bf16_wgrad_sumsq(const void* A, const void* B, long long lda, long long ldb, int K, void* C, void* bias_grad,
+                             int M, int N, long long ldc, int accumulate, int splitk, void* workspace,
+                             long long workspace_bytes, float* sumsq, void* stream);
+int tn_gemm_bf16_grouped_sumsq(const void* const* A, const void* const* B, const long long* lda, const long long* ldb,
+                               const int* K, void* const* C, const long long* ldc, const int* M, const int* N, int ngrp,
+                               int accumulate, void* workspace, long long workspace_bytes, float* const* sumsq,
+                               void* stream);
+int tn_gemm_bf16_grouped_table_sumsq(const void* const* A, const void* const* B, const long long* lda,
+                                     const long long* ldb, const int* K, void* const* C, const long long* ldc, const int* M,
+                                     const int* N, void* const* bias_grad, int n, int accumulate, void* table,
+                                     long long table_bytes, float* const* sumsq, void* stream);
 int tn_gemm_bf16_swiglu_fwd(const void* x, const void* wg, const void* wu, void* gate, void* up, void* act, int M, int I,
                             int K, long long ldx, long long ldw, long long ldc, void* stream);
 int tn_gemm_bf16_swiglu_bwd(const void* dy, const void* wd, const void* gate, const void* up, void* dgate, void* dup,
diff --git a/touchnet_amd/_C.py b/touchnet_amd/_C.py
--- a/touchnet_amd/_C.py
+++ b/touchnet_amd/_C.py
@@ -57,6 +57,8 @@
     "tn_bestrq_tokenize": [_vp, _vp, _vp, _vp, _i, _i, _i, _i, _vp],
     "tn_sumsq_multi_chunk": [],
     "tn_sumsq_multi": [_vp, _vp, _vp, _i, _ll, _vp, _vp, _i, _vp],
+    "tn_sum_ranges_chunk": [],
+    "tn_sum_ranges": [_vp, _vp, _vp, _i, _ll, _vp, _vp, _vp],
     "tn_adamw_multi_chunk": [],
     "tn_adamw_prepare": [_vp, _vp, _f, _f, _f, _vp],
     "tn_adamw_multi": [_vp, _vp, _vp, _vp, _vp, _vp, _vp, _i, _ll, _vp, _f, _f, _f, _f, _f, _i, _vp],
@@ -79,6 +81,14 @@
                                    C.POINTER(_vp), C.POINTER(_ll), C.POINTER(_i), C.POINTER(_i), C.POINTER(_vp), _i, _i, _i,
                                    _vp, _ll, _vp],
     "tn_gemm_bf16_wgrad_bias": [_vp, _vp, _ll, _ll, _i, _vp, _vp, _i, _i, _ll, _i, _i, _i, _vp, _ll, _vp],
+    "tn_gemm_wgrad_sumsq_floats": [_i, _i],
+    "tn_gemm_bf16_wgrad_sumsq": [_vp, _vp, _ll, _ll, _i, _vp, _vp, _i, _i, _ll, _i, _i, _vp, _ll, _vp, _vp],
+    "tn_gemm_bf16_grouped_sumsq": [C.POINTER(_vp), C.POINTER(_vp), C.POINTER(_ll), C.POINTER(_ll), C.POINTER(_i),
+                                   C.POINTER(_vp), C.POINTER(_ll), C.POINTER(_i), C.POINTER(_i), _i, _i, _vp, _ll,
+                                   C.POINTER(_vp), _vp],
+    "tn_gemm_bf16_grouped_table_sumsq": [C.POINTER(_vp), C.POINTER(_vp), C.POINTER(_ll), C.POINTER(_ll), C.POINTER(_i),
+                                         C.POINTER(_vp), C.POINTER(_ll), C.POINTER(_i), C.POINTER(_i), C.POINTER(_vp), _i,
+                                         _i, _vp, _ll, C.POINTER(_vp), _vp],
     "tn_gemm_bf16_rope": [_vp, _vp, _vp, _vp, _vp, _vp, _i, _i, _i, _ll, _ll, _ll, _i, _vp],
     "tn_gemm_bf16_gelu_fwd": [_vp, _vp, _vp, _vp, _vp, _i, _i, _i, _ll, _ll, _ll, _vp],
     "tn_gemm_bf16_gelu_bwd": [_vp, _vp, _vp, _vp, _i, _i, _i, _ll, _ll, _ll, _vp],
@@ -98,7 +108,8 @@
     "tn_attn_block_causal_fwd": [_vp, _vp, _vp, _vp, _vp, _vp, _i, _i, _i, _i, _i, _f, _vp],
     "tn_vq_nearest": [_vp, _vp, _vp, _vp, _i, _i, _i, _vp],
 }
-_RESTYPE = {"tn_gemm_set_persistent": None, "tn_version": C.c_char_p, "tn_sumsq_multi_chunk": C.c_longlong, "tn_adamw_multi_chunk": C.c_longlong,
+_RESTYPE = {"tn_gemm_set_persistent": None, "tn_version": C.c_char_p, "tn_sumsq_multi_chunk": C.c_longlong, "tn_sum_ranges_chunk": C.c_longlong,
+            "tn_gemm_wgrad_sumsq_floats": C.c_longlong, "tn_adamw_multi_chunk": C.c_longlong,
             "tn_colsum_workspace_floats": C.c_longlong, "tn_gemm_splitk_workspace_bytes": C.c_longlong,
             "tn_gemm_grouped_workspace_bytes": C.c_longlong, "tn_gemm_grouped_table_bytes": C.c_longlong,
             "tn_attn_decode_workspace_bytes": C.c_longlong, "tn_beam_step_workspace_bytes": C.c_longlong,
diff --git a/touchnet_amd/csrc/gemm.hip b/touchnet_amd/csrc/gemm.hip
--- a/touchnet_amd/csrc/gemm.hip
+++ b/touchnet_amd/csrc/gemm.hip
@@ -614,66 +614,26 @@
   const int t = blockIdx.x >> 5, part = blockIdx.x & 31;
   int tm, tn;
   tile_of_block(tile0 + t, nbm, nbn, tm, tn);
-  const int idx = part * 256 + threadIdx.x;
-  const int lm = idx >> 5, ln = (idx & 31) * 8;
-  const int m = tm * BM + lm, n = tn * BN + ln;
-  if (m >= M || n >= N) return;
-  if (bias_out != nullptr && tn == 0 && ln == 0) {
-    float b = 0.f;
-    for (int sp = 0; sp < S; ++sp) b += bias_ws[(long long)sp * (nbm * BM) + m];
-    bias_out[m] = f2bf(b);
-  }
-  float a[8] = {0.f, 0.f, 0.f, 0.f, 0.f, 0.f, 0.f, 0.f};
-  const float* src = ws + (long long)t * (BM * BN) + lm * BN + ln;
-  const long long slab = (long long)ntiles * (BM * BN);
-  for (int sp = 0; sp < S; ++sp) {
-    const float4 x = *reinterpret_cast<const float4*>(src + sp * slab);
-    const float4 y = *reinterpret_cast<const float4*>(src + sp * slab + 4);
-    a[0] += x.x; a[1] += x.y; a[2] += x.z; a[3] += x.w;
-    a[4] += y.x; a[5] += y.y; a[6] += y.z; a[7] += y.w;
-  }
-  if (out_f32) {
-    float* d = reinterpret_cast<float*>(C) + (long long)m * ldc + n;
-    float4 x = make_float4(a[0], a[1], a[2], a[3]), y = make_float4(a[4], a[5], a[6], a[7]);
-    if (accumulate) {
-      const float4 ox = *reinterpret_cast<const float4*>(d), oy = *reinterpret_cast<const float4*>(d + 4);
-      x.x += ox.x; x.y += ox.y; x.z += ox.z; x.w += ox.w;
-      y.x += oy.x; y.y += oy.y; y.z += oy.z; y.w += oy.w;
-    }
-    *reinterpret_cast<float4*>(d) = x;
-    *reinterpret_cast<float4*>(d + 4) = y;
-    return;
-  }
-  bf16_t* dst = C + (long long)m * ldc + n;
-  if (bias != nullptr) {
-    Vec16<bf16_t> b;
-    float fb[8];
-    b.load(bias + n);
-    b.unpack(fb);
-#pragma unroll
-    for (int e = 0; e < 8; ++e) a[e] += fb[e];
-  }
-  if (accumulate) {
-    Vec16<bf16_t> o;
-    float fo[8];
-    o.load(dst);
-    o.unpack(fo);
-#pragma unroll
-    for (int e = 0; e < 8; ++e) a[e] += fo[e];
-  }
-  Vec16<bf16_t> out;
-  out.pack(a);
-  out.store(dst);
+  (void)splitk_reduce_thread(ws, S, M, N, nbm, tm, tn, t, part, ntiles, C, ldc, bias, accumulate, out_f32, bias_ws, bias_out);
 }
 
 template <bool AK, bool BK, bool HAS_CT>
 static int launch(dim3 grid, hipStream_t st, const Params& p) {
   constexpr bool WGRAD = AK && BK && !HAS_CT;
   auto reduce = [&](const float* bias_ws, bf16_t* bias_out) {
-    hipLaunchKernelGGL(splitk_reduce_kernel, dim3((unsigned)p.ntiles * 32u), dim3(256), 0, st, p.ws, p.splitk, p.M, p.N,
-                       p.nbm, p.nbn, p.tile0, p.ntiles, p.C, p.ldc, p.bias, p.accumulate, p.c_f32, bias_ws, bias_out);
+    if (p.sumsq != nullptr)
+      launch_splitk_reduce_sumsq(st, p, bias_ws, bias_out, p.sumsq);
+    else
+      hipLaunchKernelGGL(splitk_reduce_kernel, dim3((unsigned)p.ntiles * 32u), dim3(256), 0, st, p.ws, p.splitk, p.M, p.N,
+                         p.nbm, p.nbn, p.tile0, p.ntiles, p.C, p.ldc, p.bias, p.accumulate, p.c_f32, bias_ws, bias_out);
   };
-  if (p.bias_out != nullptr) {
+  if (p.sumsq != nullptr && p.splitk <= 1) {
+    if constexpr (WGRAD) {
+      launch_sumsq(p.bias_out != nullptr ? EPI_BIASG : EPI_PLAIN, grid, st, p);
+    } else {
+      return -1;
+    }
+  } else if (p.bias_out != nullptr) {
     if constexpr (WGRAD) {
       if (p.splitk > 1) {
         hipLaunchKernelGGL((gemm_kernel<true, true, false, true, false, EPI_BIASG>), grid, dim3(NT), 0, st, p);
@@ -748,6 +708,7 @@
   void* bias_grad = nullptr;
   const void* addend = nullptr;
   long long ldadd = 0;
+  float* sumsq = nullptr;
 };
 
 int launch_mode(bool a_kmaj, bool b_kmaj, bool ct, dim3 grid, hipStream_t st, const Params& p) {
@@ -765,6 +726,7 @@
     return TN_EINVAL;
   if ((c.bias_grad != nullptr || c.c_f32) && (!wgrad_mode || c.tail_only)) return TN_EINVAL;
   if (!aligned(1, c.bias_grad)) return TN_EINVAL;
+  if (c.sumsq != nullptr && (!wgrad_mode || c.c_f32 || c.tail_only || !aligned(15, c.sumsq))) return TN_EINVAL;
   if (M <= 0 || N <= 0 || c.nseg < 1 || c.nseg > MAXSEG || (N % 8) != 0 || (c.a_kmaj && (M % 8))) return TN_EINVAL;
   if (!out_ok(c.C, c.ldc, N, 8)) return TN_EINVAL;
   if (c.Ct != nullptr && ((M % 8) || c.accumulate || !out_ok(c.Ct, c.ldct, M, 8))) return TN_EINVAL;
@@ -794,6 +756,7 @@
   p.ntiles = p.nbm * p.nbn;
   p.c_f32 = c.c_f32;
   p.bias_out = (bf16_t*)c.bias_grad;
+  p.sumsq = c.sumsq;
   const int ncu = num_cus();
   int main_tiles = 0;
   if (c.splitk > 1) {
@@ -896,11 +859,12 @@
 
 static int wgrad(const void* A, const void* B, long long lda, long long ldb, int K, void* C, void* bias_grad, int M, int N,
                  long long ldc, int accumulate, int c_f32, int splitk, void* workspace, long long workspace_bytes,
-                 void* stream) {
+                 void* stream, float* sumsq = nullptr) {
   GemmCall c{&A, &B, &lda, &ldb, &K, 1, 1, 1, C, ldc, M, N, stream};
   c.accumulate = accumulate;
   c.c_f32 = c_f32;
   c.bias_grad = bias_grad;
+  c.sumsq = sumsq;
   c.splitk = splitk > 1 ? splitk : 1;
   c.workspace = workspace;
   c.workspace_bytes = workspace_bytes;
@@ -918,6 +882,18 @@
                             long long workspace_bytes, void* stream) {
   if (bias_grad == nullptr) return TN_EINVAL;
   return wgrad(A, B, lda, ldb, K, C, bias_grad, M, N, ldc, accumulate, c_f32, splitk, workspace, workspace_bytes, stream);
+}
+
+long long tn_gemm_wgrad_sumsq_floats(int M, int N) {
+  if (M <= 0 || N <= 0) return -1;
+  return (long long)((M + BM - 1) / BM) * ((N + BN - 1) / BN) * SUMSQ_SLOTS;
+}
+
+int tn_gemm_bf16_wgrad_sumsq(const void* A, const void* B, long long lda, long long ldb, int K, void* C, void* bias_grad,
+                             int M, int N, long long ldc, int accumulate, int splitk, void* workspace,
+                             long long workspace_bytes, float* sumsq, void* stream) {
+  if (sumsq == nullptr) return TN_EINVAL;
+  return wgrad(A, B, lda, ldb, K, C, bias_grad, M, N, ldc, accumulate, 0, splitk, workspace, workspace_bytes, stream, sumsq);
 }
 
 long long tn_gemm_grouped_workspace_bytes(const int* M, const int* N, const int* K, int ngrp) {
@@ -932,18 +908,24 @@
   return S > 1 ? slab_floats(S, r) * (long long)sizeof(float) : 0;
 }
 
-int tn_gemm_bf16_grouped(const void* const* A, const void* const* B, const long long* lda, const long long* ldb,
-                         const int* K, void* const* C, const long long* ldc, const int* M, const int* N, int ngrp,
-                         int a_kmaj, int b_kmaj, int accumulate, int c_f32, void* workspace, long long workspace_bytes,
-                         void* stream) {
+static int grouped(const void* const* A, const void* const* B, const long long* lda, const long long* ldb,
+                   const int* K, void* const* C, const long long* ldc, const int* M, const int* N, int ngrp,
+                   int a_kmaj, int b_kmaj, int accumulate, int c_f32, void* workspace, long long workspace_bytes,
+                   float* const* sumsq, void* stream) {
   if (ngrp < 1 || ngrp > MAXSEG) return TN_EINVAL;
   if (!(a_kmaj && b_kmaj)) return TN_EINVAL;
   Params p;
   clear_params(p);
   int total = 0, min_stages = 0x7fffffff;
+  bool slots = false;
   for (int g = 0; g < ngrp; ++g) {
     if (!grouped_product(A[g], B[g], lda[g], ldb[g], K[g], C[g], ldc[g], M[g], N[g], c_f32, total, p.seg[g], p.grp[g]))
       return TN_EINVAL;
+    if (sumsq != nullptr && sumsq[g] != nullptr) {
+      if (c_f32 || !aligned(15, sumsq[g])) return TN_EINVAL;
+      p.grp_sumsq[g] = sumsq[g];
+      slots = true;
+    }
     min_stages = min(min_stages, p.grp[g].stages);
     total += p.grp[g].nbm * p.grp[g].nbn;
   }
@@ -965,6 +947,8 @@
   p.ntiles = main_tiles;
   if (c_f32)
     hipLaunchKernelGGL((gemm_kernel<true, true, false, false, true, EPI_GROUPED>), grid_for(main_tiles), dim3(NT), 0, st, p);
+  else if (slots)
+    launch_sumsq(EPI_GROUPED, grid_for(main_tiles), st, p);
   else
     hipLaunchKernelGGL((gemm_kernel<true, true, false, false, false, EPI_GROUPED>), grid_for(main_tiles), dim3(NT), 0, st, p);
   if (S > 1) {
@@ -992,14 +976,33 @@
       q.ntiles = hi - lo;
       q.c_f32 = c_f32;
       hipLaunchKernelGGL((gemm_kernel<true, true, false, true>), grid_for(q.ntiles * S), dim3(NT), 0, st, q);
-      hipLaunchKernelGGL(splitk_reduce_kernel, dim3((unsigned)q.ntiles * 32u), dim3(256), 0, st, q.ws, q.splitk, q.M, q.N,
-                         q.nbm, q.nbn, q.tile0, q.ntiles, q.C, q.ldc, (const bf16_t*)nullptr, q.accumulate, q.c_f32,
-                         (const float*)nullptr, (bf16_t*)nullptr);
+      if (p.grp_sumsq[g] != nullptr)
+        launch_splitk_reduce_sumsq(st, q, nullptr, nullptr, p.grp_sumsq[g]);
+      else
+        hipLaunchKernelGGL(splitk_reduce_kernel, dim3((unsigned)q.ntiles * 32u), dim3(256), 0, st, q.ws, q.splitk, q.M, q.N,
+                           q.nbm, q.nbn, q.tile0, q.ntiles, q.C, q.ldc, (const bf16_t*)nullptr, q.accumulate, q.c_f32,
+                           (const float*)nullptr, (bf16_t*)nullptr);
       ws += slab_floats(S, q.ntiles);
     }
   }
   TN_LAUNCH_CHECK();
   return TN_OK;
+}
+
+int tn_gemm_bf16_grouped(const void* const* A, const void* const* B, const long long* lda, const long long* ldb,
+                         const int* K, void* const* C, const long long* ldc, const int* M, const int* N, int ngrp,
+                         int a_kmaj, int b_kmaj, int accumulate, int c_f32, void* workspace, long long workspace_bytes,
+                         void* stream) {
+  return grouped(A, B, lda, ldb, K, C, ldc, M, N, ngrp, a_kmaj, b_kmaj, accumulate, c_f32, workspace, workspace_bytes,
+                 nullptr, stream);
+}
+
+int tn_gemm_bf16_grouped_sumsq(const void* const* A, const void* const* B, const long long* lda, const long long* ldb,
+                               const int* K, void* const* C, const long long* ldc, const int* M, const int* N, int ngrp,
+                               int accumulate, void* workspace, long long workspace_bytes, float* const* sumsq,
+                               void* stream) {
+  if (sumsq == nullptr) return TN_EINVAL;
+  return grouped(A, B, lda, ldb, K, C, ldc, M, N, ngrp, 1, 1, accumulate, 0, workspace, workspace_bytes, sumsq, stream);
 }
 int tn_gemm_bf16_swiglu_fwd(const void* x, const void* wg, const void* wu, void* gate, void* up, void* act, int M, int I,
                             int K, long long ldx, long long ldw, long long ldc, void* stream) {
diff --git a/touchnet_amd/csrc/gemm_host.h b/touchnet_amd/csrc/gemm_host.h
--- a/touchnet_amd/csrc/gemm_host.h
+++ b/touchnet_amd/csrc/gemm_host.h
@@ -6,6 +6,13 @@
 using tn::bf16_t;
 
 extern "C" int tn_gemm_get_persistent(void);
+
+namespace tn {
+namespace gemm {
+void launch_sumsq(int epi, dim3 grid, hipStream_t st, const Params& p);
+void launch_splitk_reduce_sumsq(hipStream_t st, const Params& p, const float* bias_ws, bf16_t* bias_out, float* sumsq);
+}
+}
 
 namespace {
 
diff --git a/touchnet_amd/csrc/gemm_kernel.h b/touchnet_amd/csrc/gemm_kernel.h
--- a/touchnet_amd/csrc/gemm_kernel.h
+++ b/touchnet_amd/csrc/gemm_kernel.h
@@ -41,6 +41,7 @@
   Seg seg;
   Grp grp;
   bf16_t* bias_out;
+  float* sumsq;
 };
 typedef const __attribute__((address_space(4))) Rec* rec_ptr_t;
 constexpr int MAXTAB = 1024;
@@ -79,7 +80,22 @@
   const bf16_t* rope_sin;
   int rope_d;
   const Rec* table;
+  float* sumsq;
+  float* grp_sumsq[MAXSEG];
 };
+constexpr int SUMSQ_SLOTS = 32;
+
+__device__ __forceinline__ float sumsq8(const uint4& v) {
+#pragma clang fp contract(off)
+  const uint32_t w[4] = {v.x, v.y, v.z, v.w};
+  float s[4];
+#pragma unroll
+  for (int i = 0; i < 4; ++i) {
+    const float lo = __uint_as_float(w[i] << 16), hi = __uint_as_float(w[i] & 0xffff0000u);
+    s[i] = __builtin_fmaf(hi, hi, lo * lo);
+  }
+  return (s[0] + s[1]) + (s[2] + s[3]);
+}
 
 __device__ __forceinline__ int xcd_chunk(int bid, int total) {
   const int xcd = bid & 7, local = bid >> 3;
@@ -181,7 +197,7 @@
   return r;
 }
 
-template <bool AK, bool BK, bool HAS_CT, bool SPLITK = false, bool OUT_F32 = false, int EPI = EPI_PLAIN>
+template <bool AK, bool BK, bool HAS_CT, bool SPLITK = false, bool OUT_F32 = false, int EPI = EPI_PLAIN, bool SUMSQ = false>
 struct Kernel {
   static_assert(EPI == EPI_PLAIN || EPI == EPI_GROUPED || EPI == EPI_BIASG || EPI == EPI_TABLE,
                 "Kernel: plain / grouped / bias-gradient epilogues (the fused ones are Kernel16's)");
@@ -189,6 +205,7 @@
   static constexpr bool BIASG = EPI == EPI_BIASG || EPI == EPI_TABLE;
   static_assert(!MULTI || (!HAS_CT && !SPLITK), "grouped launch: whole tiles, no transposed copy");
   static_assert(!BIASG || (AK && BK && !HAS_CT), "bias gradient: weight-gradient mode");
+  static_assert(!SUMSQ || (AK && BK && !HAS_CT && !SPLITK && !OUT_F32), "sum of squares: unsplit bf16 weight gradients");
   struct Out {
     bf16_t* C;
     long long ldc;
@@ -615,10 +632,19 @@
       } else if constexpr (MULTI) {
         const Grp r = grp_of(grp);
         const Out o = {r.C, r.ldc, r.M, r.N};
-        epilogue(p, o, acc, smem + (wave < 4 ? pb : pa) * SLOT + (wave & 3) * 8192, m0 + wr * 128, n0 + wc * 64, lane);
+        const float ssq =
+            epilogue(p, o, acc, smem + (wave < 4 ? pb : pa) * SLOT + (wave & 3) * 8192, m0 + wr * 128, n0 + wc * 64, lane);
+        if constexpr (SUMSQ) {
+          float* slots;
+          if constexpr (EPI == EPI_TABLE) slots = tab[grp].sumsq;
+          else slots = grp == 0 ? p.grp_sumsq[0] : grp == 1 ? p.grp_sumsq[1] : p.grp_sumsq[2];
+          store_sumsq(slots, ssq, (m0 >> 8) * r.nbn + (n0 >> 8), wave, lane);
+        }
       } else {
         const Out o = {p.C, p.ldc, p.M, p.N};
-        epilogue(p, o, acc, smem + (wave < 4 ? pb : pa) * SLOT + (wave & 3) * 8192, m0 + wr * 128, n0 + wc * 64, lane);
+        const float ssq =
+            epilogue(p, o, acc, smem + (wave < 4 ? pb : pa) * SLOT + (wave & 3) * 8192, m0 + wr * 128, n0 + wc * 64, lane);
+        if constexpr (SUMSQ) store_sumsq(p.sumsq, ssq, (m0 >> 8) * p.nbn + (n0 >> 8), wave, lane);
       }
       zero_acc();
       __builtin_amdgcn_s_waitcnt(0xc07f);
@@ -671,9 +697,19 @@
     }
   }
 
-  static __device__ __forceinline__ void epilogue(const Params& p, const Out& o, Acc& acc, char* park, int wm0, int wn0,
-                                                  int lane) {
+  static __device__ __forceinline__ void store_sumsq(float* slots, float ssq, int tile, int wave, int lane) {
+    if (slots == nullptr) return;
+    const float tot = wave_sum(ssq);
+    if (lane == 0) {
+      const f32x4_t v = {tot, 0.f, 0.f, 0.f};
+      *reinterpret_cast<f32x4_t*>(slots + (long long)tile * SUMSQ_SLOTS + wave * 4) = v;
+    }
+  }
+
+  static __device__ __forceinline__ float epilogue(const Params& p, const Out& o, Acc& acc, char* park, int wm0, int wn0,
+                                                   int lane) {
     const int l31 = lane & 31, hi = lane >> 5;
+    float ssq = 0.f;
     float bias_v[2][4][4];
     if (p.bias != nullptr) {
 #pragma unroll
@@ -729,6 +765,7 @@
             v = nw.raw;
           }
           *reinterpret_cast<uint4*>(dst) = v;
+          if constexpr (SUMSQ) ssq += sumsq8(v);
         }
       }
       if constexpr (HAS_CT) {
@@ -755,6 +792,7 @@
         }
       }
     }
+    return ssq;
   }
 };
 
@@ -764,5 +802,70 @@
   Kernel<AK, BK, HAS_CT, SPLITK, OUT_F32, EPI>::run(p, smem);
 }
 
-}
-}
+template <int EPI>
+__global__ __launch_bounds__(NT, 2) void gemm_sumsq_kernel(const Params p) {
+  __shared__ __attribute__((aligned(1024))) char smem[LDS_BYTES];
+  Kernel<true, true, false, false, false, EPI, true>::run(p, smem);
+}
+
+
+__device__ __forceinline__ float splitk_reduce_thread(const float* __restrict__ ws, int S, int M, int N, int nbm, int tm,
+                                                      int tn, int t, int part, int ntiles, bf16_t* __restrict__ C,
+                                                      long long ldc, const bf16_t* __restrict__ bias, int accumulate,
+                                                      int out_f32, const float* __restrict__ bias_ws,
+                                                      bf16_t* __restrict__ bias_out) {
+  const int idx = part * 256 + threadIdx.x;
+  const int lm = idx >> 5, ln = (idx & 31) * 8;
+  const int m = tm * BM + lm, n = tn * BN + ln;
+  if (m >= M || n >= N) return 0.f;
+  if (bias_out != nullptr && tn == 0 && ln == 0) {
+    float b = 0.f;
+    for (int sp = 0; sp < S; ++sp) b += bias_ws[(long long)sp * (nbm * BM) + m];
+    bias_out[m] = f2bf(b);
+  }
+  float a[8] = {0.f, 0.f, 0.f, 0.f, 0.f, 0.f, 0.f, 0.f};
+  const float* src = ws + (long long)t * (BM * BN) + lm * BN + ln;
+  const long long slab = (long long)ntiles * (BM * BN);
+  for (int sp = 0; sp < S; ++sp) {
+    const float4 x = *reinterpret_cast<const float4*>(src + sp * slab);
+    const float4 y = *reinterpret_cast<const float4*>(src + sp * slab + 4);
+    a[0] += x.x; a[1] += x.y; a[2] += x.z; a[3] += x.w;
+    a[4] += y.x; a[5] += y.y; a[6] += y.z; a[7] += y.w;
+  }
+  if (out_f32) {
+    float* d = reinterpret_cast<float*>(C) + (long long)m * ldc + n;
+    float4 x = make_float4(a[0], a[1], a[2], a[3]), y = make_float4(a[4], a[5], a[6], a[7]);
+    if (accumulate) {
+      const float4 ox = *reinterpret_cast<const float4*>(d), oy = *reinterpret_cast<const float4*>(d + 4);
+      x.x += ox.x; x.y += ox.y; x.z += ox.z; x.w += ox.w;
+      y.x += oy.x; y.y += oy.y; y.z += oy.z; y.w += oy.w;
+    }
+    *reinterpret_cast<float4*>(d) = x;
+    *reinterpret_cast<float4*>(d + 4) = y;
+    return 0.f;
+  }
+  bf16_t* dst = C + (long long)m * ldc + n;
+  if (bias != nullptr) {
+    Vec16<bf16_t> b;
+    float fb[8];
+    b.load(bias + n);
+    b.unpack(fb);
+#pragma unroll
+    for (int e = 0; e < 8; ++e) a[e] += fb[e];
+  }
+  if (accumulate) {
+    Vec16<bf16_t> o;
+    float fo[8];
+    o.load(dst);
+    o.unpack(fo);
+#pragma unroll
+    for (int e = 0; e < 8; ++e) a[e] += fo[e];
+  }
+  Vec16<bf16_t> out;
+  out.pack(a);
+  out.store(dst);
+  return sumsq8(out.raw);
+}
+
+}
+}
diff --git a/touchnet_amd/csrc/gemm_sumsq.hip b/touchnet_amd/csrc/gemm_sumsq.hip
--- /dev/null
+++ b/touchnet_amd/csrc/gemm_sumsq.hip
@@ -0,0 +1,34 @@
+#include "gemm_host.h"
+
+namespace tn {
+namespace gemm {
+
+__global__ __launch_bounds__(256) void splitk_reduce_sumsq_kernel(const float* __restrict__ ws, int S, int M, int N, int nbm,
+                                                                  int nbn, int tile0, int ntiles, bf16_t* __restrict__ C,
+                                                                  long long ldc, const bf16_t* __restrict__ bias,
+                                                                  int accumulate, const float* __restrict__ bias_ws,
+                                                                  bf16_t* __restrict__ bias_out, float* __restrict__ sumsq) {
+  static_assert(SUMSQ_SLOTS == 32, "one slot per reduce block of a tile");
+  __shared__ float sm[4];
+  const int t = blockIdx.x >> 5, part = blockIdx.x & 31;
+  int tm, tn;
+  tile_of_block(tile0 + t, nbm, nbn, tm, tn);
+  const float ssq =
+      splitk_reduce_thread(ws, S, M, N, nbm, tm, tn, t, part, ntiles, C, ldc, bias, accumulate, 0, bias_ws, bias_out);
+  const float tot = block_sum(ssq, sm);
+  if (threadIdx.x == 0) sumsq[((long long)tm * nbn + tn) * SUMSQ_SLOTS + part] = tot;
+}
+
+void launch_sumsq(int epi, dim3 grid, hipStream_t st, const Params& p) {
+  if (epi == EPI_BIASG) hipLaunchKernelGGL((gemm_sumsq_kernel<EPI_BIASG>), grid, dim3(NT), 0, st, p);
+  else if (epi == EPI_GROUPED) hipLaunchKernelGGL((gemm_sumsq_kernel<EPI_GROUPED>), grid, dim3(NT), 0, st, p);
+  else hipLaunchKernelGGL((gemm_sumsq_kernel<EPI_PLAIN>), grid, dim3(NT), 0, st, p);
+}
+
+void launch_splitk_reduce_sumsq(hipStream_t st, const Params& p, const float* bias_ws, bf16_t* bias_out, float* sumsq) {
+  hipLaunchKernelGGL(splitk_reduce_sumsq_kernel, dim3((unsigned)p.ntiles * 32u), dim3(256), 0, st, p.ws, p.splitk, p.M, p.N,
+                     p.nbm, p.nbn, p.tile0, p.ntiles, p.C, p.ldc, p.bias, p.accumulate, bias_ws, bias_out, sumsq);
+}
+
+}
+}
diff --git a/touchnet_amd/csrc/gemm_table.hip b/touchnet_amd/csrc/gemm_table.hip
--- a/touchnet_amd/csrc/gemm_table.hip
+++ b/touchnet_amd/csrc/gemm_table.hip
@@ -22,14 +22,15 @@
 
 long long tn_gemm_grouped_table_bytes(int n) { return n < 1 || n > MAXTAB ? -1 : (long long)n * (long long)sizeof(Rec); }
 
-int tn_gemm_bf16_grouped_table(const void* const* A, const void* const* B, const long long* lda, const long long* ldb,
-                               const int* K, void* const* C, const long long* ldc, const int* M, const int* N,
-                               void* const* bias_grad, int n, int accumulate, int c_f32, void* table, long long table_bytes,
-                               void* stream) {
+static int grouped_table(const void* const* A, const void* const* B, const long long* lda, const long long* ldb,
+                         const int* K, void* const* C, const long long* ldc, const int* M, const int* N,
+                         void* const* bias_grad, int n, int accumulate, int c_f32, void* table, long long table_bytes,
+                         float* const* sumsq, void* stream) {
   if (n < 1 || n > MAXTAB) return TN_EINVAL;
   if (table == nullptr || !aligned(15, table) || table_bytes < tn_gemm_grouped_table_bytes(n)) return TN_EINVAL;
   std::vector<RecChunk> chunks((n + TABCHUNK - 1) / TABCHUNK);
   long long total = 0;
+  bool slots = false;
   for (int g = 0; g < n; ++g) {
     Rec& r = chunks[g / TABCHUNK].r[g % TABCHUNK];
     if (total > 0x7fffffff) return TN_EINVAL;
@@ -37,6 +38,11 @@
       return TN_EINVAL;
     r.bias_out = bias_grad != nullptr ? (bf16_t*)bias_grad[g] : nullptr;
     if (!aligned(1, r.bias_out)) return TN_EINVAL;
+    if (sumsq != nullptr && sumsq[g] != nullptr) {
+      if (c_f32 || !aligned(15, sumsq[g])) return TN_EINVAL;
+      r.sumsq = sumsq[g];
+      slots = true;
+    }
     total += (long long)r.grp.nbm * r.grp.nbn;
   }
   if (total > 0x7fffffff) return TN_EINVAL;
@@ -53,10 +59,27 @@
   p.ntiles = (int)total;
   if (c_f32)
     hipLaunchKernelGGL((gemm_kernel<true, true, false, false, true, EPI_TABLE>), grid_for(p.ntiles), dim3(NT), 0, st, p);
+  else if (slots)
+    hipLaunchKernelGGL((gemm_sumsq_kernel<EPI_TABLE>), grid_for(p.ntiles), dim3(NT), 0, st, p);
   else
     hipLaunchKernelGGL((gemm_kernel<true, true, false, false, false, EPI_TABLE>), grid_for(p.ntiles), dim3(NT), 0, st, p);
   TN_LAUNCH_CHECK();
   return TN_OK;
 }
 
+int tn_gemm_bf16_grouped_table(const void* const* A, const void* const* B, const long long* lda, const long long* ldb,
+                               const int* K, void* const* C, const long long* ldc, const int* M, const int* N,
+                               void* const* bias_grad, int n, int accumulate, int c_f32, void* table, long long table_bytes,
+                               void* stream) {
+  return grouped_table(A, B, lda, ldb, K, C, ldc, M, N, bias_grad, n, accumulate, c_f32, table, table_bytes, nullptr, stream);
 }
+
+int tn_gemm_bf16_grouped_table_sumsq(const void* const* A, const void* const* B, const long long* lda, const long long* ldb,
+                                     const int* K, void* const* C, const long long* ldc, const int* M, const int* N,
+                                     void* const* bias_grad, int n, int accumulate, void* table, long long table_bytes,
+                                     float* const* sumsq, void* stream) {
+  if (sumsq == nullptr) return TN_EINVAL;
+  return grouped_table(A, B, lda, ldb, K, C, ldc, M, N, bias_grad, n, accumulate, 0, table, table_bytes, sumsq, stream);
+}
+
+}
diff --git a/touchnet_amd/csrc/optim.hip b/touchnet_amd/csrc/optim.hip
--- a/touchnet_amd/csrc/optim.hip
+++ b/touchnet_amd/csrc/optim.hip
@@ -76,6 +76,37 @@
       acc += f * f;
     }
   }
+  acc = block_sum(acc, sm);
+  if (threadIdx.x == 0) partial[c] = acc;
+}
+
+constexpr long long kSumChunk = 8192;
+
+__global__ __launch_bounds__(256) void sum_ranges_kernel(const void* const* __restrict__ ptrs,
+                                                         const long long* __restrict__ sizes,
+                                                         const long long* __restrict__ first_chunk, int nranges,
+                                                         float* __restrict__ partial) {
+  __shared__ float sm[4];
+  const long long c = blockIdx.x;
+  int lo = 0, hi = nranges - 1;
+  while (lo < hi) {
+    const int mid = (lo + hi + 1) >> 1;
+    if (first_chunk[mid] <= c) lo = mid; else hi = mid - 1;
+  }
+  const float* g = static_cast<const float*>(ptrs[lo]);
+  const long long beg = (c - first_chunk[lo]) * kSumChunk;
+  const long long end = min(beg + kSumChunk, sizes[lo]);
+  float acc = 0.f;
+  long long done = beg;
+  if ((reinterpret_cast<uintptr_t>(g) & 15) == 0) {
+    const long long nvec = (end - beg) / 4;
+    for (long long v = threadIdx.x; v < nvec; v += 256) {
+      const float4 a = *reinterpret_cast<const float4*>(g + beg + v * 4);
+      acc += (a.x + a.y) + (a.z + a.w);
+    }
+    done = beg + nvec * 4;
+  }
+  for (long long i = done + threadIdx.x; i < end; i += 256) acc += g[i];
   acc = block_sum(acc, sm);
   if (threadIdx.x == 0) partial[c] = acc;
 }
@@ -282,6 +313,20 @@
   return TN_OK;
 }
 
+long long tn_sum_ranges_chunk(void) { return kSumChunk; }
+
+int tn_sum_ranges(const void* const* ptrs, const long long* sizes, const long long* first_chunk, int nranges,
+                  long long nchunks, float* partial, float* norm_sq, void* stream) {
+  if (nranges <= 0 || nchunks <= 0 || nchunks > 0x7fffffffLL) return TN_EINVAL;
+  hipStream_t st = (hipStream_t)stream;
+  hipLaunchKernelGGL(sum_ranges_kernel, dim3((unsigned)nchunks), dim3(256), 0, st, ptrs, sizes, first_chunk, nranges,
+                     partial);
+  TN_LAUNCH_CHECK();
+  hipLaunchKernelGGL(sumsq_final_kernel, dim3(1), dim3(1024), 0, st, partial, norm_sq, (int)nchunks);
+  TN_LAUNCH_CHECK();
+  return TN_OK;
+}
+
 int tn_adamw_step(float* p, float* m, float* v, const void* g, void* p_shadow_bf16, const float* norm_sq,
                   long long n, float lr, float beta1, float beta2, float eps, float weight_decay, float max_norm,
                   float bias_corr1, float bias_corr2, int g_dtype, void* stream) {
diff --git a/touchnet_amd/functional.py b/touchnet_amd/functional.py
--- a/touchnet_amd/functional.py
+++ b/touchnet_amd/functional.py
@@ -357,7 +357,7 @@
 def gemm(segs, a_kmaj: bool = False, b_kmaj: bool = False, bias: Optional[torch.Tensor] = None,
          out: Optional[torch.Tensor] = None, accumulate: bool = False,
          out_t: Optional[torch.Tensor] = None, bias_grad: Optional[torch.Tensor] = None,
-         addend: Optional[torch.Tensor] = None) -> torch.Tensor:
+         addend: Optional[torch.Tensor] = None, sumsq: Optional[int] = None) -> torch.Tensor:
     if not 1 <= len(segs) <= 3:
         raise _C.KernelError("gemm: 1..3 segments")
     for a, b in segs:
@@ -400,16 +400,23 @@
                      "tn_gemm_bf16_addend")
             return out
     lib = _C.lib()
-    if f32 or bias_grad is not None:
+    if sumsq is not None and (f32 or not wgrad_mode or addend is not None):
+        raise _C.KernelError("gemm: sumsq exists for the single-segment weight-gradient mode with a bf16 output only")
+    if f32 or bias_grad is not None or sumsq is not None:
         if not wgrad_mode:
             raise _C.KernelError("gemm: bias_grad exists for the single-segment weight-gradient mode only")
         split = split_k(M, N, Ks[0], True, True) if SPLIT_K else 1
         ws, ws_bytes = _splitk_workspace(M, N, split, bias_grad is not None, a0.device)
-        if bias_grad is None:
+        if bias_grad is not None:
+            _check_bias_grad(bias_grad, M, a0)
+        if sumsq is not None:
+            _C.check(lib.tn_gemm_bf16_wgrad_sumsq(_p(a0), _p(b0), a0.stride(0), b0.stride(0), Ks[0], _p(out), _p(bias_grad), M,
+                                                  N, out.stride(0), int(accumulate), split, _p(ws), ws_bytes,
+                                                  ctypes.c_void_p(sumsq), _cur()), "tn_gemm_bf16_wgrad_sumsq")
+        elif bias_grad is None:
             _C.check(lib.tn_gemm_bf16_wgrad_f32(_p(a0), _p(b0), a0.stride(0), b0.stride(0), Ks[0], _p(out), M, N, out.stride(0),
                                                 int(accumulate), split, _p(ws), ws_bytes, _cur()), "tn_gemm_bf16_wgrad_f32")
         else:
-            _check_bias_grad(bias_grad, M, a0)
             _C.check(lib.tn_gemm_bf16_wgrad_bias(_p(a0), _p(b0), a0.stride(0), b0.stride(0), Ks[0], _p(out), _p(bias_grad), M, N,
                                                  out.stride(0), int(accumulate), int(f32), split, _p(ws), ws_bytes, _cur()),
                      "tn_gemm_bf16_wgrad_bias")
@@ -463,7 +470,17 @@
     return outs
 
 
-def gemm_grouped_wgrad(pairs, outs=None, accumulate: bool = False):
+def wgrad_sumsq_floats(M: int, N: int) -> int:
+    return int(_C.lib().tn_gemm_wgrad_sumsq_floats(int(M), int(N)))
+
+
+def _slot_array(sumsq, n, outs, name):
+    if len(sumsq) != n or outs[0].dtype != torch.bfloat16:
+        raise _C.KernelError(f"{name}: sumsq needs one entry per product and bf16 outputs")
+    return _carr(ctypes.c_void_p, list(sumsq))
+
+
+def gemm_grouped_wgrad(pairs, outs=None, accumulate: bool = False, sumsq=None):
     n = len(pairs)
     if not 1 <= n <= 3:
         raise _C.KernelError("gemm_grouped_wgrad: 1..3 products")
@@ -475,6 +492,12 @@
     need = int(_C.lib().tn_gemm_grouped_workspace_bytes(Ms, Ns, Ks, n))
     ws = torch.empty(need // 4, dtype=torch.float32, device=outs[0].device) if need > 0 else None
     Ap, Bp, la, lb = _operand_arrays(pairs)
+    if sumsq is not None and any(s is not None for s in sumsq):
+        _C.check(_C.lib().tn_gemm_bf16_grouped_sumsq(
+            Ap, Bp, la, lb, Ks, _carr(ctypes.c_void_p, [o.data_ptr() for o in outs]),
+            _carr(ctypes.c_longlong, [o.stride(0) for o in outs]), Ms, Ns, n, int(accumulate), _p(ws), need,
+            _slot_array(sumsq, n, outs, "gemm_grouped_wgrad"), _cur()), "tn_gemm_bf16_grouped_sumsq")
+        return list(outs)
     _C.check(_C.lib().tn_gemm_bf16_grouped(Ap, Bp, la, lb, Ks, _carr(ctypes.c_void_p, [o.data_ptr() for o in outs]),
                                            _carr(ctypes.c_longlong, [o.stride(0) for o in outs]), Ms, Ns, n, 1, 1,
                                            int(accumulate), int(f32), _p(ws), need, _cur()), "tn_gemm_bf16_grouped")
@@ -484,7 +507,7 @@
 GROUPED_TABLE_MAX = 1024
 
 
-def gemm_grouped_table_wgrad(pairs, outs=None, accumulate: bool = False, bias_grads=None):
+def gemm_grouped_table_wgrad(pairs, outs=None, accumulate: bool = False, bias_grads=None, sumsq=None):
     n = len(pairs)
     if not 1 <= n <= GROUPED_TABLE_MAX:
         raise _C.KernelError(f"gemm_grouped_table_wgrad: 1..{GROUPED_TABLE_MAX} products")
@@ -498,6 +521,15 @@
     need = int(lib.tn_gemm_grouped_table_bytes(n))
     table = torch.empty(need, dtype=torch.uint8, device=outs[0].device)
     Ap, Bp, la, lb = _operand_arrays(pairs)
+    if sumsq is not None and any(s is not None for s in sumsq):
+        _C.check(lib.tn_gemm_bf16_grouped_table_sumsq(
+            Ap, Bp, la, lb, _carr(ctypes.c_int, [a.shape[0] for a, _ in pairs]),
+            _carr(ctypes.c_void_p, [o.data_ptr() for o in outs]), _carr(ctypes.c_longlong, [o.stride(0) for o in outs]),
+            _carr(ctypes.c_int, [a.shape[1] for a, _ in pairs]), _carr(ctypes.c_int, [b.shape[1] for _, b in pairs]),
+            _carr(ctypes.c_void_p, [bg.data_ptr() if bg is not None else None for bg in bias_grads]), n, int(accumulate),
+            _p(table), need, _slot_array(sumsq, n, outs, "gemm_grouped_table_wgrad"), _cur()),
+            "tn_gemm_bf16_grouped_table_sumsq")
+        return list(outs)
     _C.check(lib.tn_gemm_bf16_grouped_table(
         Ap, Bp, la, lb, _carr(ctypes.c_int, [a.shape[0] for a, _ in pairs]),
         _carr(ctypes.c_void_p, [o.data_ptr() for o in outs]), _carr(ctypes.c_longlong, [o.stride(0) for o in outs]),
@@ -754,6 +786,78 @@
     return sink if sink is not None and sink.owns(w) else None
 
 
+WGRAD_SUMSQ = True
+SUMSQ_LEDGERS = {}
+
+
+class GradNormLedger:
+
+    def __init__(self, weights):
+        self._range = {}
+        total = 0
+        for w in weights:
+            if id(w) in self._range or w.dim() != 2 or w.dtype != torch.bfloat16:
+                continue
+            n = wgrad_sumsq_floats(*w.shape)
+            self._range[id(w)] = (w, total, n)
+            total += n
+            SUMSQ_LEDGERS[id(w)] = weakref.ref(self)
+        dev = next((w.device for w, _, _ in self._range.values()), None)
+        self.arena = torch.empty(total, dtype=torch.float32, device=dev) if total else None
+        self._wrote = {}
+
+    def __len__(self):
+        return len(self._range)
+
+    def close(self):
+        for k in self._range:
+            ref = SUMSQ_LEDGERS.get(k)
+            if ref is not None and ref() is self:
+                del SUMSQ_LEDGERS[k]
+        self._range, self._wrote = {}, {}
+
+    def slots(self, w) -> Optional[int]:
+        own = self._range.get(id(w))
+        if own is None or own[0] is not w:
+            return None
+        self._wrote.pop(id(w), None)
+        return self.arena.data_ptr() + 4 * own[1]
+
+    def wrote(self, w, out) -> None:
+        if id(w) in self._range:
+            self._wrote[id(w)] = (out.data_ptr(), out._version)
+
+    def covered(self, w, grad) -> bool:
+        rec = self._wrote.get(id(w))
+        own = self._range.get(id(w))
+        return (rec is not None and own is not None and own[0] is w and grad.dtype == torch.bfloat16
+                and tuple(grad.shape) == tuple(w.shape) and grad.is_contiguous()
+                and rec == (grad.data_ptr(), grad._version))
+
+    def take(self, pairs):
+        hit, ranges = [], []
+        for i, (w, g) in enumerate(pairs):
+            if self.covered(w, g):
+                _, first, n = self._range[id(w)]
+                hit.append(i)
+                ranges.append((self.arena.data_ptr() + 4 * first, n))
+        self._wrote = {}
+        return hit, ranges
+
+
+def _slots_of(w) -> Optional[int]:
+    if not WGRAD_SUMSQ:
+        return None
+    led = _live(SUMSQ_LEDGERS, w)
+    return led.slots(w) if led is not None and _sink_of(w) is None else None
+
+
+def _slots_wrote(w, out) -> None:
+    led = _live(SUMSQ_LEDGERS, w)
+    if led is not None:
+        led.wrote(w, out)
+
+
 DEFERRED_WGRAD = True
 DEFERRED_WGRAD_FLUSH_LAYERS = 11
 WGRAD_QUEUES = {}
@@ -835,10 +939,14 @@
                         for w, dy, _, _, _ in chunk]
                 bgs = [torch.empty(dy.shape[1], dtype=torch.bfloat16, device=dy.device) if b is not None else None
                        for _, dy, _, b, _ in chunk]
-                self.launch([(dy, x2) for _, dy, x2, _, _ in chunk], outs=outs, accumulate=acc, bias_grads=bgs)
-                for (w, _, _, b, _), o, bg in zip(chunk, outs, bgs):
+                slots = [_slots_of(w) for w, _, _, _, _ in chunk]
+                extra = {"sumsq": slots} if any(s is not None for s in slots) else {}
+                self.launch([(dy, x2) for _, dy, x2, _, _ in chunk], outs=outs, accumulate=acc, bias_grads=bgs, **extra)
+                for (w, _, _, b, _), o, bg, s in zip(chunk, outs, bgs, slots):
                     if not acc:
                         w.grad = o
+                    if s is not None:
+                        _slots_wrote(w, o)
                     if b is not None:
                         if b.grad is None:
                             b.grad = bg
@@ -864,7 +972,11 @@
 
     def launch():
         if sink is None:
-            return gemm([(dy, x2)], True, True, bias_grad=db)
+            slots = _slots_of(w)
+            dw = gemm([(dy, x2)], True, True, bias_grad=db, sumsq=slots)
+            if slots is not None:
+                _slots_wrote(w, dw)
+            return dw
         view, acc = sink.take(w)
         gemm([(dy, x2)], True, True, out=view, accumulate=acc, bias_grad=db)
         sink.done(w)
@@ -932,7 +1044,12 @@
 
     def launch():
         if not owned:
-            return gemm_grouped_wgrad(pairs)
+            slots = [_slots_of(w) for w, _, _ in items]
+            dws = gemm_grouped_wgrad(pairs, sumsq=slots)
+            for (w, _, _), dw, s in zip(items, dws, slots):
+                if s is not None:
+                    _slots_wrote(w, dw)
+            return dws
         taken = [sk.take(w) for sk, (w, _, _) in zip(sinks, items)]
         if len({(v.dtype, bool(acc)) for v, acc in taken}) == 1:
             gemm_grouped_wgrad(pairs, outs=[v for v, _ in taken], accumulate=bool(taken[0][1]))
diff --git a/touchnet_amd/utils/optimizer.py b/touchnet_amd/utils/optimizer.py
--- a/touchnet_amd/utils/optimizer.py
+++ b/touchnet_amd/utils/optimizer.py
@@ -10,6 +10,13 @@
 
 def _local(t: torch.Tensor) -> torch.Tensor:
     return t._local_tensor if hasattr(t, "_local_tensor") else t
+
+
+def ledger_weights(params, groups, tp_group) -> List[Any]:
+    if groups or tp_group is not None or any(hasattr(p, "_local_tensor") for p in params):
+        return []
+    return [p for p in params if p.dim() == 2 and p.dtype == torch.bfloat16 and (p.is_cuda or p.is_meta)
+            and p.shape[0] % 8 == 0 and p.shape[1] % 8 == 0]
 
 
 def _shard_groups(params) -> List[Any]:
@@ -51,6 +58,14 @@
         self.norm_sq = torch.zeros(1, dtype=torch.float32, device=dev)
         self.step_state = torch.zeros(8, dtype=torch.float32, device=dev)
         self._partial, self._keep = None, None
+        ws = ledger_weights(self.params, self.groups, tp_group)
+        if ws:
+            from touchnet_amd.functional import GradNormLedger
+            self.ledger = GradNormLedger(ws)
+        else:
+            self.ledger = None
+        self._ranges = None
+        self.last_covered = []
         self._pipe = None
         self._pipe_delay_cycles = 0
         self.side_workgroups = int(os.environ.get("TN_ADAMW_SIDE_WORKGROUPS", "128"))
@@ -101,6 +116,22 @@
                                         p_(self.norm_sq), _C.dcode(gs[0]), st()), "tn_sumsq_multi")
             keep.append((table, gs))
         return keep
+
+    def _sum_ranges(self, ranges, device):
+        if not ranges:
+            return
+        lib, p_, st = _C.lib(), _C.ptr, _C.stream
+        if self._ranges is None or self._ranges[0] != ranges:
+            chunk = int(lib.tn_sum_ranges_chunk())
+            first, tot = [], 0
+            for _, n in ranges:
+                first.append(tot)
+                tot += (n + chunk - 1) // chunk
+            table = self._table([[a for a, _ in ranges], [n for _, n in ranges], first], device)
+            self._ranges = (list(ranges), table, tot, torch.empty(tot, dtype=torch.float32, device=device))
+        _, table, tot, partial = self._ranges
+        _C.check(lib.tn_sum_ranges(p_(table[0]), p_(table[1]), p_(table[2]), len(ranges), tot, p_(partial),
+                                   p_(self.norm_sq), st()), "tn_sum_ranges")
 
     def zero_grad(self, set_to_none: bool = True):
         for p in self.params:
@@ -132,7 +163,20 @@
             tp_all_reduce(self.norm_sq, self.tp_group)
             keep += self._sumsq(drop_empty(pick(False)))
         else:
-            keep = self._sumsq(by_dtype)
+            listed, ranges, self.last_covered = by_dtype, [], []
+            if self.ledger is not None:
+                items = by_dtype.get(torch.bfloat16, [])
+                hit, ranges = self.ledger.take([(self.params[i], g) for i, g in items])
+                if hit:
+                    gone = set(hit)
+                    self.last_covered = [items[k][0] for k in hit]
+                    rest = [it for k, it in enumerate(items) if k not in gone]
+                    listed = {dt: (rest if dt == torch.bfloat16 else v) for dt, v in by_dtype.items()}
+                    listed = {dt: v for dt, v in listed.items() if v}
+            keep = self._sumsq(listed)
+            self._sum_ranges(ranges, self.norm_sq.device)
+            if ranges:
+                keep.append([g for _, g in by_dtype[torch.bfloat16]])
         for grp in self.groups:
             torch.distributed.all_reduce(self.norm_sq, group=grp)
         _C.check(lib.tn_adamw_prepare(p_(self.norm_sq), p_(self.step_state), b1, b2, float(self.max_norm), st()),
```

New measurement: 22090. 3.9% lower.
